# MinghanLi/MDQE_CVPR2023

Measured on AMD Instinct MI355X. Metric: frames/sec (eval-only) R50 OVIS 360p 4-frame clip, higher is better.
Workload: dtype f32; 1 GPU; R50_ovis_360 eval-only, H2D included: 120 synthetic 360x640 u8 frames/GPU/step from pinned host memory, 4-frame clips stride 1, 30-frame windows, one model(inputs) call per video; random-init weights, calibrated class logits (DESIGN.md §5); frames_per_gpu=120, instances_out=10, tracked_instances=7, gemm=exact fp32 MFMA, hw_queues=4, ranks_seen=1, parallelism=single GPU

## Files before the change

### include/mdqe_hip.h

```cpp
#ifndef MDQE_HIP_H
#define MDQE_HIP_H
#include <stdint.h>

#ifdef __cplusplus
extern "C" {
#endif

#define MDQE_OK 0
#define MDQE_EINVAL 1
#define MDQE_ELAUNCH 2
#define MDQE_ENULL 3
#define MDQE_ESTATE 4

#define MDQE_ACT_NONE 0
#define MDQE_ACT_RELU 1
#define MDQE_ACT_GELU 2
#define MDQE_ACT_SIGMOID 3
#define MDQE_ACT_TANH 4

#define MDQE_ABI_VERSION 6
int mdqe_abi_version(void);
int mdqe_version(void);
const char* mdqe_strerror(int code);

int mdqe_msda_forward_f32(const float* value, const int64_t* shapes, const int64_t* level_start,
                          const float* loc, const float* attn,
                          int B, int S, int M, int D, int L, int Q, int P,
                          float* out, void* stream);

int mdqe_msda_backward_f32(const float* value, const int64_t* shapes, const int64_t* level_start, const float* loc,
                           const float* attn, const float* grad_out, int B, int S, int M, int D, int L, int Q, int P,
                           float* grad_value, float* grad_loc, float* grad_attn, void* stream);

int mdqe_msda_forward_f64(const double* value, const int64_t* shapes, const int64_t* level_start, const double* loc,
                          const double* attn, int B, int S, int M, int D, int L, int Q, int P, double* out, void* stream);
int mdqe_msda_backward_f64(const double* value, const int64_t* shapes, const int64_t* level_start, const double* loc,
                           const double* attn, const double* grad_out, int B, int S, int M, int D, int L, int Q, int P,
                           double* grad_value, double* grad_loc, double* grad_attn, void* stream);

int mdqe_msda_forward_grouped_f32(const float* value, const int64_t* shapes, const int64_t* level_start,
                                  const float* loc, const float* attn,
                                  int B, int S, int M, int D, int G, int L, int Q, int P,
                                  float scale, float* out, void* stream);

int mdqe_msda_fused_f32(const float* value, long ldv, long v_brows, const int* vidx, const float* offs, long ldo,
                        const float* logits, long ldl, const float* ref, long ref_bstride, int ref_dim,
                        int mode, const float* grid, const int* lvH_host, const int* lvW_host,
                        const int* lvStart_host, int B, int M, int D, int G, int L, int Q, int P, float scale,
                        float* out, long ldout, long value_rows, void* stream);

int mdqe_gemm_nt_f32(const float* A, long lda, const float* W, const float* bias, float* C, long ldc,
                     int M, int N, int K, int act, int act_cols, const float* residual, long ldr, int res_mod,
                     int res_first, const unsigned char* rowmask, int mask_cols, int tile, int ksplit,
                     float* splitk_ws, const void* w_split, void* stream);

int mdqe_gemm_nt_cat2_f32(const float* A1, long lda1, int K1, const float* A2, long lda2, int K2, int NI, int OH, int OW,
                          int H2, int W2, int stride, const float* W, const float* bias, float* C, long ldc, int N, int act,
                          void* stream);

int mdqe_gemm_nt_pix_f32(const float* A, long lda, int K, int NI, int H, int W, int OH, int OW, int stride, const float* Wt,
                         const float* bias, float* C, long ldc, int N, int act, void* stream);

int mdqe_gemm_ln_f32(const float* A, long lda, const float* W, const float* bias, float* C, long ldc, int M, int N, int K,
                     const float* residual, long ldr, const float* gamma, const float* beta, float eps, void* stream);
int mdqe_gemm_ln2_f32(const float* A, long lda, const float* W, const float* bias, float* C, long ldc, int M, int N, int K,
                      const float* residual, long ldr, const float* gamma, const float* beta, const float* gamma2, const float* beta2,
                      float* C2, long ldc2, float eps, void* stream);

int mdqe_gemm_nt_side_f32(const float* A, long lda, const float* W, const float* bias, float* C, long ldc, int M, int N, int K,
                          const float* side, const float* side_w, int side_cols, const void* w_split, void* stream);

int mdqe_set_gemm_precision(int mode);
int mdqe_get_gemm_precision(void);
int mdqe_set_gemm_precision_thread(int mode);

int mdqe_f16x3_split_f32(const float* w, long n, void* planes, void* stream);

int mdqe_debug_gemm_stamps(void* buf);
int mdqe_debug_gemm_variant(int v);
int mdqe_debug_gemm_tile_rule(int v);
int mdqe_debug_gemm_rows_dot(int v);
int mdqe_debug_gemm_fast_epilogue(int v);
int mdqe_debug_gemm_stagger(int v);
int mdqe_debug_gemm_stages(int v);
int mdqe_debug_msda_dec_stage_kb(int kb);
int mdqe_debug_trk_fast(int on);
int mdqe_debug_trk_spin_us(int us);
int mdqe_debug_trk_times(double* out5, int on);
int mdqe_debug_trk_siou_blocks(int blocks);
int mdqe_debug_gemm_lds_pad(int bytes);
int mdqe_debug_window_attn_variant(int v);
int mdqe_debug_msda_xcd_order(int v);
int mdqe_debug_msda_dec_staged(int v);
int mdqe_debug_msda_dec_wpe8(int v);
int mdqe_debug_msda_patch(int v);
int mdqe_debug_msda_stage_kb(int v);
int mdqe_debug_msda_tp_staged(int v);
int mdqe_debug_msda_op_staged(int v);
int mdqe_debug_msda_variant(int v);
int mdqe_debug_mha_variant(int v);

int mdqe_conv2d_nhwc_f32(const float* X, long x_img_stride, const float* Wt, const float* bias, float* Y, long ldy,
                         int NI, int H, int W, int Cin, int Cout, int KH, int KW, int stride, int pad,
                         int act, const float* residual, long ldr, int res_first, int tile, const void* w_split,
                         int ksplit, float* splitk_ws, void* stream);

int mdqe_winograd_weight_f32(const float* Wt, int Cout, int Cin, float* U, void* stream);
long mdqe_winograd_workspace_bytes(int NI, int H, int W, int Cin, int Cout);
int mdqe_conv3x3_winograd_f32(const float* X, long x_img_stride, const float* U, const float* bias, float* Y, long ldy,
                              int NI, int H, int W, int Cin, int Cout, int act, void* workspace, long ws_bytes, void* stream);
int mdqe_debug_winograd_tile(int tile);

int mdqe_resize_pil_bilinear_u8(const unsigned char* in, long in_img_stride, int NI, int C, int H, int W, int oh, int ow,
                                const int* xmin, const int* xcnt, const int* xk, int kxs, const int* ymin, const int* ycnt,
                                const int* yk, int kys, unsigned char* out, void* stream);

#define MDQE_YUV_COEFFS { \
  {16, 128, 76309, 104597, -25675, -53279, 132201},  \
  {0, 128, 65536, 91881, -22553, -46802, 116130},    \
  {16, 128, 76309, 117489, -13975, -34925, 138438},  \
  {0, 128, 65536, 103206, -12276, -30679, 121609},   \
  {64, 512, 19077, 26149, -6419, -13320, 33050},     \
  {0, 512, 16336, 22903, -5622, -11666, 28947},      \
  {64, 512, 19077, 29372, -3494, -8731, 34610},      \
  {0, 512, 16336, 25726, -3060, -7647, 30313}        }
int mdqe_yuv420sp_to_rgb_u8(const void* y, long y_pitch, long y_stride, const void* uv, long uv_pitch, long uv_stride,
                            int NI, int H, int W, int fmt , int matrix , int full_range,
                            int bgr, unsigned char* out , void* stream);

int mdqe_layernorm_f32(const float* x, const float* res, const float* gamma, const float* beta, float* y,
                       long rows, int C, float eps, void* stream);

long mdqe_groupnorm_workspace_bytes(int NI, int G);
int mdqe_groupnorm_nhwc_f32(const float* x, long ldx, long x_img_stride, float* y, long ldy, long y_img_stride,
                            int NI, int HW, int C, int G,
                            const float* gamma, const float* beta, float eps, int act, void* workspace, void* stream);

int mdqe_stem_im2col_f32(const void* frames, int is_u8, long frame_stride, int NI, int h, int w, int Hp, int Wp,
                         const float* mean3_host, const float* std3_host, float* out, void* stream);

int mdqe_stem_conv_f32(const void* frames, int is_u8, long frame_stride, int NI, int h, int w, int Hp, int Wp,
                       const float* mean3_host, const float* std3_host, const float* wk, const float* bias, float* out,
                       void* stream);

int mdqe_maxpool3x3s2_nhwc_f32(const float* x, float* y, int NI, int H, int W, int C, void* stream);

int mdqe_upsample_nearest_add_nhwc_f32(const float* a, const float* b, float* y, int NI, int H, int W, int Hb, int Wb,
                                       int C, void* stream);

int mdqe_dwconv5x5_nhwc_f32(const float* x, const float* wt, const float* bias, float* y, int NI, int H, int W, int C,
                            int up2, const float* tw, const float* tb, void* stream);

int mdqe_dwconv5x5_c256_f32(const float* x, const float* wt, const float* bias, float* y, int NI, int H, int W, void* stream);
int mdqe_dwconv5x5_up2_c256_f32(const float* x, const float* wt, const float* bias, const float* tw, const float* tb, float* y,
                                int NI, int Hs, int Ws, void* stream);

int mdqe_dwconv5x5_up2_pw_c256_f32(const float* x, const float* wt, const float* bias, const float* tw, const float* tb,
                                   const float* pw, const float* pb, float* out, long ldo, int NI, int Hs, int Ws, void* stream);

int mdqe_trk_siou_f32(const float* saved, long saved_stride, int n_saved, const float* inp, long inp_stride,
                      int n_in, long n, float* out3, void* stream);
int mdqe_trk_accumulate_f32(float* sum, long sum_stride, float* cnt, long cnt_stride, const float* src,
                            long src_stride, long n, int nf, const int* r_host, const int* c_host, int count,
                            void* stream);
int mdqe_trk_siou_host_f32(const float* saved, long saved_stride, int n_saved, const float* inp, long inp_stride,
                           int n_in, long n, float* acc, unsigned* ticket, unsigned long long* out_host,
                           unsigned seq, void* stream);
int mdqe_trk_wait_counts(const unsigned long long* out_host, int n_out, unsigned seq, int spin_us, float* counts, void* stream);

int mdqe_trk_window_mean_f32(const float* sum, const float* cnt, long hw, int mem_len, int n, int nf, long f0,
                             float* out, void* stream);
int mdqe_trk_carry_f32(float* sum, float* cnt, long hw, int mem_len, int n, int k, long src0, float* carry, void* stream);

int mdqe_lsap_f64(const double* cost, int nr, int nc, int maximize, int* rows_out, int* cols_out, int* n_out);
int mdqe_tracker_create(int max_inst, int T, int win, int stride, int K, int E, float thr, void** handle);
int mdqe_tracker_destroy(void* handle);
int mdqe_tracker_state(void* handle, int* num_inst, int* num_clip, int* start_frame);
int mdqe_tracker_overlap(void* handle, int f0, int n_frames, int* ni, int* s0, int* a, int* nf);
int mdqe_tracker_decide(void* handle, int f0, int n_frames, int n_in, const float* scores, const float* cls_probs,
                        const float* embeds, const float* counts3, int* r_idx, int* c_idx, int* n_pairs,
                        int* s0, int* a, int* nf);
int mdqe_tracker_result(void* handle, int is_last, float* out_cls, int* n, int* ln, unsigned char* carry_valid);
int mdqe_tracker_update(void* handle, float* bank_sum, float* bank_cnt, long hw, int f0, int n_frames, int n_in,
                        const float* scores, const float* cls_probs, const float* embeds, const float* masks,
                        long inst_stride, float* counts_dev, float* counts_host, void* stream);
int mdqe_tracker_update_many(void* handle, float* bank_sum, float* bank_cnt, long hw, int n_clips, const int* f0,
                             const int* n_frames, const int* n_in, const int* row0, const float* scores,
                             const float* cls_probs, const float* embeds, const float* const* masks,
                             const long* inst_stride, float* counts_dev, float* counts_host, void* stream);
int mdqe_tracker_get_result(void* handle, int is_last, float* bank_sum, float* bank_cnt, long hw, float* out_masks,
                            float* carry, float* out_cls, int* n, int* ln, void* stream);

int mdqe_clip_assoc_f32(const float* emb, int Q, int E, const int* fidx, int Bc, int T, int ct, float wdw, int nb,
                        int* idx_out, void* stream);
int mdqe_clip_gather_init_f32(const float* content, const float* coords, const int* fidx, const int* idx, int Bc, int T,
                              int Q, int C, int ct, float* x, float* ref, float* xinst, void* stream);
int mdqe_box_refine_f32(const float* delta, const float* prev, int Bc, int T, int Q, int t0, int t1, float* boxes,
                        float* ibox, void* stream);
int mdqe_add_rows_f32(const float* a, long lda, const float* b, long ldb, float* out, long ldo, long rows, int C, void* stream);
int mdqe_time_fuse_f32(const float* w, const float* x, int Bc, int T, int Q, int C, float* out, const float* pos,
                       float* out_plus_pos, void* stream);
int mdqe_box_head_refine_f32(const float* h, long ldh, const float* W, const float* bias, const float* prev, int Bc, int T, int Q, int K,
                             int t0, int t1, float* boxes, float* ibox, void* stream);
int mdqe_time_fuse_dot_f32(const float* xw, const float* wt, const float* bt, const float* src, int Bc, int T, int Q, int C, float* out,
                           void* stream);

int mdqe_clip_select_f32(const float* cls, const float* emb, int B, int Q, int K, int C, float thr, int max_keep,
                         int* order_ws, int* n_thr_ws, float* inv_norm_ws, float* sim_ws, int* kept, int* n_keep, void* stream);
long mdqe_dyn_mask_workspace_floats(int n_rows, int T, int H, int W);
int mdqe_dyn_mask_nms_f32(const float* coef, const int* kept, const float* feats, int B, int Q, int M, int T, int H, int W,
                          const int* row0_host, const int* n_host, const int* f0_host, float* logits, float* soft_h,
                          float* hard_h, float* part, float* gram, float* stats, float* mi, void* stream);
long mdqe_nms_workspace_floats(int n_max);
int mdqe_clip_finalize_f32(const float* cls, const float* emb, const int* kept, const float* stats, const float* mi, int B,
                           int Q, int K, int C, float thr, const int* row0_host, const int* n_host, int* sel, int* n_sel,
                           float* out, void* stream);
int mdqe_rows_gather_f32(const float* src, const int* idx_dev, int n, long len, float* out, void* stream);

int mdqe_mask_row_stats_f32(const float* logits, int n, int T, int H, int W, int t_step, float* stats5,
                            float* soft_h, float* hard_h, void* stream);

int mdqe_mha_small_f32(const float* qk, long ldqk, const float* v, long ldv, float* o, long ldo, int B, int Q,
                       int C, int nh, void* stream);

int mdqe_query_select_f32(const float* conf, int NI, int H, int W, int K, int nb, float* score_ws, float* coords,
                          void* stream);

int mdqe_sample_levels_mean_f32(const float* tokens, int NI, long N, int C, const float* coords, int Qn,
                                const int* lvH_host, const int* lvW_host, const int* lvStart_host, int n_levels,
                                float* out, void* stream);

int mdqe_final_masks_u8(const float* logits, int n_sel, const int* inst_idx_dev, int Fw, int Hm, int Wm, int factor,
                        int h, int w, int Ho, int Wo, unsigned char* out, long out_inst_stride, int f_off,
                        void* stream);

int mdqe_final_masks_rle(const float* logits, int n_sel, const int* inst_idx_dev, int Fw, int Hm, int Wm, int factor,
                         int h, int w, int Ho, int Wo, int cap, int* pos, int* n_pos, void* stream);

int mdqe_final_masks_u8_geom(const float* logits, int n_sel, const int* inst_idx_dev, int Fw, int Hm, int Wm, int factor,
                             int h, int w, int Ho, int Wo, unsigned char* out, long out_inst_stride, int f_off,
                             int* geom, void* stream);
int mdqe_final_masks_rle_geom(const float* logits, int n_sel, const int* inst_idx_dev, int Fw, int Hm, int Wm, int factor,
                              int h, int w, int Ho, int Wo, int cap, int* pos, int* n_pos, int* geom, void* stream);

int mdqe_final_label_map_u8(const float* logits, int n_sel, const int* inst_idx_dev, int Fw, int Hm, int Wm, int factor,
                            int h, int w, int Ho, int Wo, unsigned char* out, int f_off, int* geom, void* stream);

int mdqe_final_matte_u8(const float* logits, int n_sel, const int* inst_idx_dev, int Fw, int Hm, int Wm, int factor,
                        int h, int w, int Ho, int Wo, const unsigned char* take, float gain, unsigned char* out, int f_off,
                        void* stream);

int mdqe_final_masks_overlap(const float* logits, int n_sel, const int* inst_idx_dev, int Fw, int Hm, int Wm, int factor,
                             int h, int w, int Ho, int Wo,
                             const uint32_t* gt_bits, int G, int f_off,
                             unsigned long long* inter, long inter_row_stride, int* area, void* stream);

int mdqe_render_overlay_u8(const void* frames, int is_u8, long frame_stride, int h0, int w0,
                           const unsigned char* labels, int F, int Ho, int Wo,
                           const unsigned char* palette, int a256, int contour,
                           unsigned char* out, int f_off, void* stream);

int mdqe_render_overlay_yuv420sp(const void* y, long y_pitch, long y_stride, const void* uv, long uv_pitch, long uv_stride,
                                 int F, int H, int W, int fmt , const unsigned char* labels,
                                 const unsigned short* palette_yuv, int a256, int contour,
                                 void* out_y, long out_y_pitch, long out_y_stride,
                                 void* out_uv, long out_uv_pitch, long out_uv_stride, int f_off, void* stream);

int mdqe_render_mosaic_u8(const void* frames, int is_u8, long frame_stride, int h0, int w0,
                          const unsigned char* labels, int F, int Ho, int Wo,
                          const unsigned char* palette, const unsigned char* action, int a256, int contour, int cell,
                          unsigned char* out, int f_off, void* stream);
int mdqe_render_mosaic_yuv420sp(const void* y, long y_pitch, long y_stride, const void* uv, long uv_pitch, long uv_stride,
                                int F, int H, int W, int fmt , const unsigned char* labels,
                                const unsigned short* palette_yuv, const unsigned char* action, int a256, int contour, int cell,
                                void* out_y, long out_y_pitch, long out_y_stride,
                                void* out_uv, long out_uv_pitch, long out_uv_stride, int f_off, void* stream);

int mdqe_render_blur_u8(const void* frames, int is_u8, long frame_stride, int h0, int w0,
                        const unsigned char* labels, int F, int Ho, int Wo,
                        const unsigned char* palette, const unsigned char* action, int a256, int contour,
                        const unsigned short* taps, int radius, unsigned char* out, int f_off, void* stream);
int mdqe_render_blur_yuv420sp(const void* y, long y_pitch, long y_stride, const void* uv, long uv_pitch, long uv_stride,
                              int F, int H, int W, int fmt , const unsigned char* labels,
                              const unsigned short* palette_yuv, const unsigned char* action, int a256, int contour,
                              const unsigned short* taps, int radius, const unsigned short* taps_c, int radius_c,
                              void* out_y, long out_y_pitch, long out_y_stride,
                              void* out_uv, long out_uv_pitch, long out_uv_stride, int f_off, void* stream);

int mdqe_render_replace_u8(const void* frames, int is_u8, long frame_stride, int h0, int w0,
                           const unsigned char* labels, int F, int Ho, int Wo,
                           const unsigned char* palette, const unsigned char* action, int a256, int contour,
                           const unsigned char* matte, const unsigned char* backdrop, int backdrop_picture, int mode,
                           unsigned char* out, int f_off, void* stream);
int mdqe_render_replace_yuv420sp(const void* y, long y_pitch, long y_stride, const void* uv, long uv_pitch, long uv_stride,
                                 int F, int H, int W, int fmt , const unsigned char* labels,
                                 const unsigned short* palette_yuv, const unsigned char* action, int a256, int contour,
                                 const unsigned char* matte, const unsigned short* backdrop_yuv,
                                 const void* by, long by_pitch, const void* buv, long buv_pitch, int mode,
                                 void* out_y, long out_y_pitch, long out_y_stride,
                                 void* out_uv, long out_uv_pitch, long out_uv_stride, int f_off, void* stream);

int mdqe_annotate_u8(unsigned char* pic , int F, int Ho, int Wo, int f_off,
                     const int* geom , int n,
                     const unsigned char* palette , const unsigned char* ink ,
                     const unsigned char* captions , int cap_len,
                     const unsigned char* font , int box, int scale, int min_area, void* stream);
int mdqe_annotate_yuv420sp(void* y, long y_pitch, long y_stride, void* uv, long uv_pitch, long uv_stride,
                           int F, int H, int W, int fmt , int f_off, const int* geom, int n,
                           const unsigned short* palette_yuv, const unsigned short* ink_yuv,
                           const unsigned char* captions, int cap_len, const unsigned char* font,
                           int box, int scale, int min_area, void* stream);

int mdqe_track_crops_u8(const void* frames, int is_u8, long frame_stride, int h0, int w0,
                        const unsigned char* labels, int F, int Ho, int Wo, const int* geom, int n,
                        int f_first, int f_step, int Sh, int Sw, int pad256, int min_area, int cutout, int fill,
                        unsigned char* out, long out_row_stride, int c_off, int* rects, long rect_row_stride, void* stream);
int mdqe_track_crops_yuv420sp(const void* y, long y_pitch, long y_stride, const void* uv, long uv_pitch, long uv_stride,
                              int H, int W, int fmt , int matrix , int full_range, int bgr,
                              const unsigned char* labels, int F, int Ho, int Wo, const int* geom, int n,
                              int f_first, int f_step, int Sh, int Sw, int pad256, int min_area, int cutout, int fill,
                              unsigned char* out, long out_row_stride, int c_off, int* rects, long rect_row_stride, void* stream);

int mdqe_label_centroids_u8(const unsigned char* labels, int F, int Ho, int Wo, int n, int min_area, long long* mom ,
                            int* pts , long pts_row_stride, int p_off, void* stream);
int mdqe_render_trails_u8(unsigned char* pic , int F, int Ho, int Wo, int f_off,
                          const int* pts, long pts_row_stride, int p_off, int n, int trail, int width,
                          const unsigned char* palette , void* stream);
int mdqe_render_trails_yuv420sp(void* y, long y_pitch, long y_stride, void* uv, long uv_pitch, long uv_stride,
                                int F, int H, int W, int fmt , int f_off,
                                const int* pts, long pts_row_stride, int p_off, int n, int trail, int width,
                                const unsigned short* palette_yuv, void* stream);

int mdqe_label_polygons_u8(const unsigned char* labels, int F, int Ho, int Wo, int n, int min_area,
                           int cap_vertices, int cap_rings,
                           int* xy,
                           int* rings,
                           int* totals,
                           void* workspace, long workspace_bytes, void* stream);
long mdqe_label_polygons_workspace(int F, int Ho, int Wo, int cap_vertices);

int mdqe_grow_labels_u8(const unsigned char* labels, int F, int Ho, int Wo,
                        const unsigned char* grow , int radius,
                        unsigned char* out , void* stream);

int mdqe_image_mask_stats_f32(const float* logits, int n, int Hm, int Wm, int factor, int h, int w, float* stats, void* stream);
int mdqe_image_final_masks_u8(const float* logits, int n_sel, const int* idx_dev, int Hm, int Wm, int factor, int h, int w,
                              int Ho, int Wo, unsigned char* out, void* stream);

int mdqe_layernorm_post_f32(const float* x, const float* gamma, const float* beta, const float* post, float* y,
                            long rows, int C, float eps, void* stream);
int mdqe_gemm_nt_swin_f32(const float* X, long lda, const float* W, const float* bias, float* C, long ldc, int B, int H, int Wd,
                          int ws, int shift, int N, int K, void* stream);
int mdqe_layernorm_swin_scatter_f32(const float* rows, const float* gamma, const float* beta, const float* shortcut, float* out,
                                    int B, int H, int W, int C, int ws, int shift, float eps, void* stream);
int mdqe_patch4_im2col_f32(const void* frames, int is_u8, long frame_stride, int NI, int h, int w, int Hp, int Wp,
                           const float* mean3_host, const float* std3_host, float* out, void* stream);
int mdqe_swin_window_f32(const float* src, const float* shortcut, float* dst, int B, int H, int W, int C, int ws,
                         int shift, int mode, void* stream);
int mdqe_window_attn_f32(const float* qkv, long ld, float* o, long ldo, int n_windows, int N, int C, int nh,
                         const float* scale, const float* bias, const float* mask, int nW, void* stream);
int mdqe_patch_merge_gather_f32(const float* x, float* out, int B, int H, int W, int C, void* stream);

#ifdef __cplusplus
}
#endif
#endif
```

### mdqe_cvpr2023_amd/_lib.py

```python
import ctypes
import os
from ctypes import c_char_p, c_float, c_int, c_void_p

_HERE = os.path.dirname(os.path.abspath(__file__))
LIB_PATH = os.environ.get("MDQE_HIP_LIB") or os.path.join(_HERE, "csrc", "libmdqe_hip.so")

from ctypes import c_long
i, f, p, l = c_int, c_float, c_void_p, c_long

SIGNATURES = {
    "mdqe_msda_forward_f32": [p, p, p, p, p, i, i, i, i, i, i, i, p, p],
    "mdqe_msda_backward_f32": [p, p, p, p, p, p, i, i, i, i, i, i, i, p, p, p, p],
    "mdqe_msda_forward_f64": [p, p, p, p, p, i, i, i, i, i, i, i, p, p],
    "mdqe_msda_backward_f64": [p, p, p, p, p, p, i, i, i, i, i, i, i, p, p, p, p],
    "mdqe_msda_forward_grouped_f32": [p, p, p, p, p, i, i, i, i, i, i, i, i, f, p, p],
    "mdqe_msda_fused_f32": [p, l, l, p, p, l, p, l, p, l, i, i, p, p, p, p, i, i, i, i, i, i, i, f, p, l, l, p],
    "mdqe_trk_siou_f32": [p, l, i, p, l, i, l, p, p],
    "mdqe_trk_accumulate_f32": [p, l, p, l, p, l, l, i, p, p, i, p],
    "mdqe_trk_window_mean_f32": [p, p, l, i, i, i, l, p, p],
    "mdqe_trk_carry_f32": [p, p, l, i, i, i, l, p, p],
    "mdqe_lsap_f64": [p, i, i, i, p, p, p],
    "mdqe_tracker_create": [i, i, i, i, i, i, f, p],
    "mdqe_tracker_destroy": [p],
    "mdqe_tracker_state": [p, p, p, p],
    "mdqe_tracker_overlap": [p, i, i, p, p, p, p],
    "mdqe_tracker_decide": [p, i, i, i, p, p, p, p, p, p, p, p, p, p],
    "mdqe_tracker_result": [p, i, p, p, p, p],
    "mdqe_tracker_update": [p, p, p, l, i, i, i, p, p, p, p, l, p, p, p],
    "mdqe_tracker_update_many": [p, p, p, l, i, p, p, p, p, p, p, p, p, p, p, p, p],
    "mdqe_tracker_get_result": [p, i, p, p, l, p, p, p, p, p, p],
    "mdqe_clip_assoc_f32": [p, i, i, p, i, i, i, f, i, p, p],
    "mdqe_clip_gather_init_f32": [p, p, p, p, i, i, i, i, i, p, p, p, p],
    "mdqe_box_refine_f32": [p, p, i, i, i, i, i, p, p, p],
    "mdqe_add_rows_f32": [p, l, p, l, p, l, l, i, p],
    "mdqe_time_fuse_f32": [p, p, i, i, i, i, p, p, p, p],
    "mdqe_box_head_refine_f32": [p, l, p, p, p, i, i, i, i, i, i, p, p, p],
    "mdqe_time_fuse_dot_f32": [p, p, p, p, i, i, i, i, p, p],
    "mdqe_clip_select_f32": [p, p, i, i, i, i, f, i, p, p, p, p, p, p, p],
    "mdqe_dyn_mask_nms_f32": [p, p, p, i, i, i, i, i, i, p, p, p, p, p, p, p, p, p, p, p],
    "mdqe_clip_finalize_f32": [p, p, p, p, p, i, i, i, i, f, p, p, p, p, p, p],
    "mdqe_rows_gather_f32": [p, p, i, l, p, p],
    "mdqe_mha_small_f32": [p, l, p, l, p, l, i, i, i, i, p],
    "mdqe_query_select_f32": [p, i, i, i, i, i, p, p, p],
    "mdqe_sample_levels_mean_f32": [p, i, l, i, p, i, p, p, p, i, p, p],
    "mdqe_image_mask_stats_f32": [p, i, i, i, i, i, i, p, p],
    "mdqe_image_final_masks_u8": [p, i, p, i, i, i, i, i, i, i, p, p],
    "mdqe_final_masks_rle": [p, i, p, i, i, i, i, i, i, i, i, i, p, p, p],
    "mdqe_final_masks_u8": [p, i, p, i, i, i, i, i, i, i, i, p, l, i, p],
    "mdqe_final_masks_rle_geom": [p, i, p, i, i, i, i, i, i, i, i, i, p, p, p, p],
    "mdqe_final_masks_u8_geom": [p, i, p, i, i, i, i, i, i, i, i, p, l, i, p, p],
    "mdqe_final_label_map_u8": [p, i, p, i, i, i, i, i, i, i, i, p, i, p, p],
    "mdqe_final_matte_u8": [p, i, p, i, i, i, i, i, i, i, i, p, f, p, i, p],
    "mdqe_render_replace_u8": [p, i, l, i, i, p, i, i, i, p, p, i, i, p, p, i, i, p, i, p],
    "mdqe_render_replace_yuv420sp": [p, l, l, p, l, l, i, i, i, i, p, p, p, i, i, p, p, p, l, p, l, i, p, l, l, p, l, l, i, p],
    "mdqe_render_overlay_u8": [p, i, l, i, i, p, i, i, i, p, i, i, p, i, p],
    "mdqe_render_overlay_yuv420sp": [p, l, l, p, l, l, i, i, i, i, p, p, i, i, p, l, l, p, l, l, i, p],
    "mdqe_render_mosaic_u8": [p, i, l, i, i, p, i, i, i, p, p, i, i, i, p, i, p],
    "mdqe_render_mosaic_yuv420sp": [p, l, l, p, l, l, i, i, i, i, p, p, p, i, i, i, p, l, l, p, l, l, i, p],
    "mdqe_render_blur_u8": [p, i, l, i, i, p, i, i, i, p, p, i, i, p, i, p, i, p],
    "mdqe_render_blur_yuv420sp": [p, l, l, p, l, l, i, i, i, i, p, p, p, i, i, p, i, p, i, p, l, l, p, l, l, i, p],
    "mdqe_annotate_u8": [p, i, i, i, i, p, i, p, p, p, i, p, i, i, i, p],
    "mdqe_annotate_yuv420sp": [p, l, l, p, l, l, i, i, i, i, i, p, i, p, p, p, i, p, i, i, i, p],
    "mdqe_track_crops_u8": [p, i, l, i, i, p, i, i, i, p, i, i, i, i, i, i, i, i, i, p, l, i, p, l, p],
    "mdqe_track_crops_yuv420sp": [p, l, l, p, l, l, i, i, i, i, i, i, p, i, i, i, p, i, i, i, i, i, i, i, i, i, p, l, i, p, l, p],
    "mdqe_label_centroids_u8": [p, i, i, i, i, i, p, p, l, i, p],
    "mdqe_label_polygons_u8": [p, i, i, i, i, i, i, i, p, p, p, p, l, p],
    "mdqe_grow_labels_u8": [p, i, i, i, p, i, p, p],
    "mdqe_render_trails_u8": [p, i, i, i, i, p, l, i, i, i, i, p, p],
    "mdqe_render_trails_yuv420sp": [p, l, l, p, l, l, i, i, i, i, i, p, l, i, i, i, i, p, p],
    "mdqe_final_masks_overlap": [p, i, p, i, i, i, i, i, i, i, i, p, i, i, p, l, p, p],
    "mdqe_set_gemm_precision": [i],
    "mdqe_set_gemm_precision_thread": [i],
    "mdqe_layernorm_post_f32": [p, p, p, p, p, l, i, f, p],
    "mdqe_gemm_nt_swin_f32": [p, l, p, p, p, l, i, i, i, i, i, i, i, p],
    "mdqe_layernorm_swin_scatter_f32": [p, p, p, p, p, i, i, i, i, i, i, f, p],
    "mdqe_patch4_im2col_f32": [p, i, l, i, i, i, i, i, p, p, p, p],
    "mdqe_swin_window_f32": [p, p, p, i, i, i, i, i, i, i, p],
    "mdqe_window_attn_f32": [p, l, p, l, i, i, i, i, p, p, p, i, p],
    "mdqe_patch_merge_gather_f32": [p, p, i, i, i, i, p],
    "mdqe_gemm_nt_f32": [p, l, p, p, p, l, i, i, i, i, i, p, l, i, i, p, i, i, i, p, p, p],
    "mdqe_f16x3_split_f32": [p, l, p, p],
    "mdqe_debug_gemm_stamps": [p],
    "mdqe_debug_gemm_variant": [i],
    "mdqe_debug_gemm_tile_rule": [i],
    "mdqe_debug_gemm_rows_dot": [i],
    "mdqe_debug_gemm_stagger": [i],
    "mdqe_debug_gemm_fast_epilogue": [i],
    "mdqe_debug_gemm_stages": [i],
    "mdqe_debug_gemm_lds_pad": [i],
    "mdqe_debug_trk_siou_blocks": [i],
    "mdqe_trk_siou_host_f32": [p, l, i, p, l, i, l, p, p, p, i, p],
    "mdqe_trk_wait_counts": [p, i, i, i, p, p],
    "mdqe_debug_trk_times": [p, i],
    "mdqe_debug_trk_fast": [i],
    "mdqe_debug_trk_spin_us": [i],
    "mdqe_debug_msda_dec_stage_kb": [i],
    "mdqe_debug_window_attn_variant": [i],
    "mdqe_debug_mha_variant": [i],
    "mdqe_debug_msda_xcd_order": [i],
    "mdqe_debug_msda_dec_staged": [i],
    "mdqe_debug_msda_patch": [i],
    "mdqe_debug_msda_dec_wpe8": [i],
    "mdqe_debug_msda_op_staged": [i],
    "mdqe_debug_msda_tp_staged": [i],
    "mdqe_debug_msda_stage_kb": [i],
    "mdqe_debug_msda_variant": [i],
    "mdqe_mask_row_stats_f32": [p, i, i, i, i, i, p, p, p, p],
    "mdqe_conv2d_nhwc_f32": [p, l, p, p, p, l, i, i, i, i, i, i, i, i, i, i, p, l, i, i, p, i, p, p],
    "mdqe_winograd_weight_f32": [p, i, i, p, p],
    "mdqe_conv3x3_winograd_f32": [p, l, p, p, p, l, i, i, i, i, i, i, p, l, p],
    "mdqe_debug_winograd_tile": [i],
    "mdqe_layernorm_f32": [p, p, p, p, p, l, i, f, p],
    "mdqe_gemm_ln_f32": [p, l, p, p, p, l, i, i, i, p, l, p, p, f, p],
    "mdqe_gemm_ln2_f32": [p, l, p, p, p, l, i, i, i, p, l, p, p, p, p, p, l, f, p],
    "mdqe_gemm_nt_side_f32": [p, l, p, p, p, l, i, i, i, p, p, i, p, p],
    "mdqe_gemm_nt_cat2_f32": [p, l, i, p, l, i, i, i, i, i, i, i, p, p, p, l, i, i, p],
    "mdqe_gemm_nt_pix_f32": [p, l, i, i, i, i, i, i, i, p, p, p, l, i, i, p],
    "mdqe_groupnorm_nhwc_f32": [p, l, l, p, l, l, i, i, i, i, p, p, f, i, p, p],
    "mdqe_resize_pil_bilinear_u8": [p, l, i, i, i, i, i, i, p, p, p, i, p, p, p, i, p, p],
    "mdqe_yuv420sp_to_rgb_u8": [p, l, l, p, l, l, i, i, i, i, i, i, i, p, p],
    "mdqe_stem_im2col_f32": [p, i, l, i, i, i, i, i, p, p, p, p],
    "mdqe_stem_conv_f32": [p, i, l, i, i, i, i, i, p, p, p, p, p, p],
    "mdqe_maxpool3x3s2_nhwc_f32": [p, p, i, i, i, i, p],
    "mdqe_upsample_nearest_add_nhwc_f32": [p, p, p, i, i, i, i, i, i, p],
    "mdqe_dwconv5x5_nhwc_f32": [p, p, p, p, i, i, i, i, i, p, p, p],
    "mdqe_dwconv5x5_c256_f32": [p, p, p, p, i, i, i, p],
    "mdqe_dwconv5x5_up2_c256_f32": [p, p, p, p, p, p, i, i, i, p],
    "mdqe_dwconv5x5_up2_pw_c256_f32": [p, p, p, p, p, p, p, p, l, i, i, i, p],
}


ABI_VERSION = 6


class LibraryMissing(RuntimeError):
    pass


class MdqeError(RuntimeError):
    pass


_lib = None


def load_library(path=None):
    global _lib
    if _lib is not None and path is None:
        return _lib
    path = path or LIB_PATH
    if not os.path.exists(path):
        raise LibraryMissing(
            f"{path} not found: build it with `make -C mdqe_cvpr2023_amd/csrc` (or "
            f"`python -c 'import __graft_entry__ as g; g.build()'`).  There is no CPU/PyTorch fallback.")
    import torch
    h = ctypes.CDLL(path)
    h.mdqe_version.restype = c_int
    h.mdqe_abi_version.restype = c_int
    h.mdqe_abi_version.argtypes = []
    if h.mdqe_abi_version() != ABI_VERSION:
        raise MdqeError(f"{path} implements ABI {h.mdqe_abi_version()}, this binding was written against ABI {ABI_VERSION} "
                        f"(include/mdqe_hip.h MDQE_ABI_VERSION): rebuild with `make -C mdqe_cvpr2023_amd/csrc`")
    h.mdqe_strerror.restype = c_char_p
    h.mdqe_strerror.argtypes = [c_int]
    h.mdqe_get_gemm_precision.restype = c_int
    h.mdqe_get_gemm_precision.argtypes = []
    h.mdqe_nms_workspace_floats.restype = c_long
    h.mdqe_nms_workspace_floats.argtypes = [c_int]
    h.mdqe_dyn_mask_workspace_floats.restype = c_long
    h.mdqe_dyn_mask_workspace_floats.argtypes = [c_int, c_int, c_int, c_int]
    h.mdqe_groupnorm_workspace_bytes.restype = c_long
    h.mdqe_groupnorm_workspace_bytes.argtypes = [c_int, c_int]
    h.mdqe_winograd_workspace_bytes.restype = c_long
    h.mdqe_winograd_workspace_bytes.argtypes = [c_int, c_int, c_int, c_int, c_int]
    h.mdqe_label_polygons_workspace.restype = c_long
    h.mdqe_label_polygons_workspace.argtypes = [c_int, c_int, c_int, c_int]
    for name, args in SIGNATURES.items():
        fn = getattr(h, name)
        fn.argtypes = args
        fn.restype = c_int
    if path == LIB_PATH:
        _lib = h
    return h


class _Lazy:
    def __getattr__(self, name):
        return getattr(load_library(), name)


lib = _Lazy()


def check(code, what=""):
    if code != 0:
        raise MdqeError(f"{what}: {load_library().mdqe_strerror(code).decode()} (code {code})")


def ptr(t):
    return None if t is None else t.data_ptr()


def raw_stream(device=None):
    import torch
    if device is None:
        idx = torch._C._cuda_getDevice()
    else:
        idx = device if isinstance(device, int) else torch.device(device).index
        if idx is None:
            idx = torch._C._cuda_getDevice()
    return torch._C._cuda_getCurrentRawStream(idx)


def cur_stream(device=None):
    return raw_stream(device)
```

### mdqe_cvpr2023_amd/csrc/common.h

```cpp
#pragma once
#include <hip/hip_runtime.h>
#include <stdint.h>
#include "../../include/mdqe_hip.h"

#define MDQE_CHECK_PTR(p) do { if ((p) == nullptr) return MDQE_ENULL; } while (0)
#define MDQE_REQUIRE(c) do { if (!(c)) return MDQE_EINVAL; } while (0)

static inline void mdqe_clear_error() { (void)hipGetLastError(); }
static inline int mdqe_launch_status() {
  return hipGetLastError() == hipSuccess ? MDQE_OK : MDQE_ELAUNCH;
}

#include <mutex>
static inline hipError_t mdqe_allow_lds(const void* kern, int bytes) {
  static std::mutex mu;
  static const void* fn[64];
  static int cap[64];
  static int n = 0;
  std::lock_guard<std::mutex> g(mu);
  int i = 0;
  for (; i < n; ++i) if (fn[i] == kern) break;
  if (i < n && cap[i] >= bytes) return hipSuccess;
  const hipError_t e = hipFuncSetAttribute(kern, hipFuncAttributeMaxDynamicSharedMemorySize, bytes);
  if (e == hipSuccess && i < 64) { fn[i] = kern; cap[i] = bytes; if (i == n) ++n; }
  return e;
}

typedef float f32x4 __attribute__((ext_vector_type(4)));
typedef float f32x2 __attribute__((ext_vector_type(2)));
typedef float f32x16 __attribute__((ext_vector_type(16)));

__device__ __forceinline__ float mdqe_gelu(float x) {
#pragma clang fp contract(off)
  const float z = __builtin_fabsf(x) * 0.70710678118654752440f;
  const float t = __builtin_amdgcn_rcpf(__builtin_fmaf(0.3275911f, z, 1.0f));
  float q = __builtin_fmaf(t, 0.5307027145f, -0.7265760135f);
  q = __builtin_fmaf(t, q, 0.7107068705f);
  q = __builtin_fmaf(t, q, -0.142248368f);
  q = __builtin_fmaf(t, q, 0.127414796f);
  const float h = q * t * __builtin_amdgcn_exp2f(z * z * -1.4426950408889634f);
  const float xh = x * h;
  return x >= 0.f ? x - xh : xh;
}

__device__ __forceinline__ float mdqe_act(float x, int act) {
  switch (act) {
    case MDQE_ACT_RELU: return x > 0.f ? x : 0.f;
    case MDQE_ACT_GELU: return mdqe_gelu(x);
    case MDQE_ACT_SIGMOID: return 1.0f / (1.0f + __expf(-x));
    case MDQE_ACT_TANH: return tanhf(x);
    default: return x;
  }
}

template <typename V4, typename ColOk>
__device__ __forceinline__ void mdqe_act4(V4& v, int act, ColOk col_ok) {
  if (act == MDQE_ACT_RELU) {
#pragma unroll
    for (int e = 0; e < 4; ++e)
      if (col_ok(e)) v[e] = v[e] > 0.f ? v[e] : 0.f;
  } else if (act == MDQE_ACT_GELU) {
#pragma unroll
    for (int e = 0; e < 4; ++e)
      if (col_ok(e)) v[e] = mdqe_gelu(v[e]);
  } else if (act != MDQE_ACT_NONE) {
#pragma unroll 1
    for (int e = 0; e < 4; ++e) {
      float x = v[0];
      if (col_ok(e)) x = mdqe_act(x, act);
      v = V4{v[1], v[2], v[3], x};
    }
  }
}
```

### mdqe_cvpr2023_amd/csrc/dwconv.hip

```cpp
#include "common.h"

namespace {
__device__ __forceinline__ f32x4 ld4(const float* p) { return *reinterpret_cast<const f32x4*>(p); }
}

__global__ void __launch_bounds__(256, 2)
dw5_c256_kernel(const float* __restrict__ x, const float* __restrict__ wt, const float* __restrict__ bias, float* __restrict__ y,
                int NI, int H, int W) {
  constexpr int C = 256;
  const int lane = threadIdx.x & 63;
  const long wid = (long)blockIdx.x * 4 + (threadIdx.x >> 6), nw = (long)gridDim.x * 4;
  f32x4 w[25];
#pragma unroll
  for (int t = 0; t < 25; ++t) w[t] = ld4(wt + t * C + lane * 4);
  const f32x4 bv = ld4(bias + lane * 4);
  const int Wp = (W + 1) / 2;
  const long total = (long)NI * H * Wp;
  for (long i = wid; i < total; i += nw) {
    const int pw_ = (int)(i % Wp); const long t = i / Wp;
    const int hh = (int)(t % H), img = (int)(t / H);
    const int w0 = pw_ * 2;
    f32x4 a0 = bv, a1 = bv;
#pragma unroll
    for (int kh = 0; kh < 5; ++kh) {
      const int ih = hh - 2 + kh;
      if (ih < 0 || ih >= H) continue;
      const float* row = x + (((long)img * H + ih) * W) * C + lane * 4;
      f32x4 X[6];
#pragma unroll
      for (int c = 0; c < 6; ++c) {
        const int iw = w0 - 2 + c;
        X[c] = (iw >= 0 && iw < W) ? ld4(row + (long)iw * C) : f32x4{0.f, 0.f, 0.f, 0.f};
      }
#pragma unroll
      for (int kw = 0; kw < 5; ++kw) { a0 += X[kw] * w[kh * 5 + kw]; a1 += X[kw + 1] * w[kh * 5 + kw]; }
    }
    float* o = y + (((long)img * H + hh) * W + w0) * C + lane * 4;
    *reinterpret_cast<f32x4*>(o) = a0;
    if (w0 + 1 < W) *reinterpret_cast<f32x4*>(o + C) = a1;
  }
}

__global__ void __launch_bounds__(256, 2)
dw5_up2_c256_kernel(const float* __restrict__ x, const float* __restrict__ wt, const float* __restrict__ bias,
                    const float* __restrict__ tw, const float* __restrict__ tb, float* __restrict__ y, int NI, int Hs, int Ws) {
  constexpr int C = 256;
  const int lane = threadIdx.x & 63;
  const long wid = (long)blockIdx.x * 4 + (threadIdx.x >> 6), nw = (long)gridDim.x * 4;
  const int H = 2 * Hs, W = 2 * Ws;
  f32x4 w[25];
#pragma unroll
  for (int t = 0; t < 25; ++t) w[t] = ld4(wt + t * C + lane * 4);
  const f32x4 bv = ld4(bias + lane * 4), twv = ld4(tw + lane * 4), tbv = ld4(tb + lane * 4);
  f32x4 wall = {0.f, 0.f, 0.f, 0.f};
#pragma unroll
  for (int t = 0; t < 25; ++t) wall += w[t];
  const f32x4 cin = bv + tbv * wall;

  const long total = (long)NI * Hs * Ws;
  for (long i = wid; i < total; i += nw) {
    const int b = (int)(i % Ws); const long t = i / Ws;
    const int a = (int)(t % Hs), img = (int)(t / Hs);
    f32x4 o00 = {0.f, 0.f, 0.f, 0.f}, o01 = o00, o10 = o00, o11 = o00;
#pragma unroll
    for (int r = 0; r < 3; ++r) {
      const int ia = a - 1 + r;
      if (ia < 0 || ia >= Hs) continue;
      const float* row = x + (((long)img * Hs + ia) * Ws) * C + lane * 4;
      f32x4 X[3];
#pragma unroll
      for (int c = 0; c < 3; ++c) {
        const int ib = b - 1 + c;
        X[c] = (ib >= 0 && ib < Ws) ? ld4(row + (long)ib * C) : f32x4{0.f, 0.f, 0.f, 0.f};
      }
#pragma unroll
      for (int c = 0; c < 3; ++c) o00 += X[c] * w[(2 * r) * 5 + 2 * c];
#pragma unroll
      for (int c = 1; c < 3; ++c) o01 += X[c] * w[(2 * r) * 5 + 2 * c - 1];
      if (r >= 1) {
#pragma unroll
        for (int c = 0; c < 3; ++c) o10 += X[c] * w[(2 * r - 1) * 5 + 2 * c];
#pragma unroll
        for (int c = 1; c < 3; ++c) o11 += X[c] * w[(2 * r - 1) * 5 + 2 * c - 1];
      }
    }
    f32x4 c00 = cin, c01 = cin, c10 = cin, c11 = cin;
    if (a == 0 || a == Hs - 1 || b == 0 || b == Ws - 1) {
      auto cst = [&](int hh, int ww) {
        f32x4 s = {0.f, 0.f, 0.f, 0.f};
#pragma unroll
        for (int kh = 0; kh < 5; ++kh) {
          const int ih = hh - 2 + kh;
          if (ih < 0 || ih >= H) continue;
#pragma unroll
          for (int kw = 0; kw < 5; ++kw) {
            const int iw = ww - 2 + kw;
            if (iw >= 0 && iw < W) s += w[kh * 5 + kw];
          }
        }
        return bv + tbv * s;
      };
      c00 = cst(2 * a, 2 * b); c01 = cst(2 * a, 2 * b + 1); c10 = cst(2 * a + 1, 2 * b); c11 = cst(2 * a + 1, 2 * b + 1);
    }
    float* o = y + (((long)img * H + 2 * a) * W + 2 * b) * C + lane * 4;
    *reinterpret_cast<f32x4*>(o) = c00 + twv * o00;
    *reinterpret_cast<f32x4*>(o + C) = c01 + twv * o01;
    *reinterpret_cast<f32x4*>(o + (long)W * C) = c10 + twv * o10;
    *reinterpret_cast<f32x4*>(o + (long)W * C + C) = c11 + twv * o11;
  }
}

__global__ void __launch_bounds__(256, 1)
dw5_up2_pw_c256_kernel(const float* __restrict__ x, const float* __restrict__ wt, const float* __restrict__ bias,
                       const float* __restrict__ tw, const float* __restrict__ tb, const float* __restrict__ pw,
                       const float* __restrict__ pb, float* __restrict__ out, long ldo, int NI, int Hs, int Ws) {
  constexpr int C = 256, QT = 8;
  extern __shared__ __attribute__((aligned(16))) float dwpw_lds[];
  const int lane = threadIdx.x & 63;
  const int wave = __builtin_amdgcn_readfirstlane(threadIdx.x >> 6);
  float* const tile = dwpw_lds + wave * (32 * C);
  const long wid = (long)blockIdx.x * 4 + wave, nw = (long)gridDim.x * 4;
  const int H = 2 * Hs, W = 2 * Ws;
  const int lr = lane & 31, lh = lane >> 5;
  f32x4 w[25];
#pragma unroll
  for (int t = 0; t < 25; ++t) w[t] = ld4(wt + t * C + lane * 4);
  const f32x4 bv = ld4(bias + lane * 4), twv = ld4(tw + lane * 4), tbv = ld4(tb + lane * 4);
  f32x4 wall = {0.f, 0.f, 0.f, 0.f};
#pragma unroll
  for (int t = 0; t < 25; ++t) wall += w[t];
  const f32x4 cin = bv + tbv * wall;
  f32x4 B0[16], B1[16];
#pragma unroll
  for (int kt = 0; kt < 16; ++kt) {
    B0[kt] = ld4(pw + lr * C + kt * 16 + lh * 4);
    B1[kt] = ld4(pw + lr * C + kt * 16 + 8 + lh * 4);
  }
  const f32x4 pbv = ld4(pb + (lane & 7) * 4);

  const int Wt = (Ws + QT - 1) / QT;
  const long total = (long)NI * Hs * Wt;
  f32x4 X[3][QT + 2];
  auto load_strip = [&](long i) __attribute__((always_inline)) {
    const int b0 = (int)(i % Wt) * QT; const long t = i / Wt;
    const int a = (int)(t % Hs), img = (int)(t / Hs);
#pragma unroll
    for (int r = 0; r < 3; ++r) {
      const int ia = a - 1 + r;
      const bool rok = ia >= 0 && ia < Hs;
      const float* row = x + (((long)img * Hs + (rok ? ia : a)) * Ws) * C + lane * 4;
#pragma unroll
      for (int c = 0; c < QT + 2; ++c) {
        const int ib = b0 - 1 + c;
        X[r][c] = (rok && ib >= 0 && ib < Ws) ? ld4(row + (long)ib * C) : f32x4{0.f, 0.f, 0.f, 0.f};
      }
    }
  };
  long i = wid;
  if (i < total) load_strip(i);
  while (i < total) {
    const int b0 = (int)(i % Wt) * QT; const long ti = i / Wt;
    const int a = (int)(ti % Hs), img = (int)(ti / Hs);
    const int nq = min(QT, Ws - b0);
#pragma unroll
    for (int q = 0; q < QT; ++q) {
      if (q >= nq) continue;
      const int b = b0 + q;
      f32x4 o00 = {0.f, 0.f, 0.f, 0.f}, o01 = o00, o10 = o00, o11 = o00;
#pragma unroll
      for (int r = 0; r < 3; ++r) {
        const int ia = a - 1 + r;
        if (ia < 0 || ia >= Hs) continue;
#pragma unroll
        for (int c = 0; c < 3; ++c) o00 += X[r][q + c] * w[(2 * r) * 5 + 2 * c];
#pragma unroll
        for (int c = 1; c < 3; ++c) o01 += X[r][q + c] * w[(2 * r) * 5 + 2 * c - 1];
        if (r >= 1) {
#pragma unroll
          for (int c = 0; c < 3; ++c) o10 += X[r][q + c] * w[(2 * r - 1) * 5 + 2 * c];
#pragma unroll
          for (int c = 1; c < 3; ++c) o11 += X[r][q + c] * w[(2 * r - 1) * 5 + 2 * c - 1];
        }
      }
      f32x4 c00 = cin, c01 = cin, c10 = cin, c11 = cin;
      if (a == 0 || a == Hs - 1 || b == 0 || b == Ws - 1) {
        auto cst = [&](int hh, int ww) {
          f32x4 s = {0.f, 0.f, 0.f, 0.f};
#pragma unroll
          for (int kh = 0; kh < 5; ++kh) {
            const int ih = hh - 2 + kh;
            if (ih < 0 || ih >= H) continue;
#pragma unroll
            for (int kw = 0; kw < 5; ++kw) {
              const int iw = ww - 2 + kw;
              if (iw >= 0 && iw < W) s += w[kh * 5 + kw];
            }
          }
          return bv + tbv * s;
        };
        c00 = cst(2 * a, 2 * b); c01 = cst(2 * a, 2 * b + 1); c10 = cst(2 * a + 1, 2 * b); c11 = cst(2 * a + 1, 2 * b + 1);
      }
      *reinterpret_cast<f32x4*>(tile + (4 * q + 0) * C + ((lane ^ ((4 * q + 0) & 15)) << 2)) = c00 + twv * o00;
      *reinterpret_cast<f32x4*>(tile + (4 * q + 1) * C + ((lane ^ ((4 * q + 1) & 15)) << 2)) = c01 + twv * o01;
      *reinterpret_cast<f32x4*>(tile + (4 * q + 2) * C + ((lane ^ ((4 * q + 2) & 15)) << 2)) = c10 + twv * o10;
      *reinterpret_cast<f32x4*>(tile + (4 * q + 3) * C + ((lane ^ ((4 * q + 3) & 15)) << 2)) = c11 + twv * o11;
    }
    asm volatile("s_waitcnt lgkmcnt(0)" ::: "memory");
    __builtin_amdgcn_wave_barrier();
    const long inext = i + nw;
    if (inext < total) load_strip(inext);

    f32x16 acc;
#pragma unroll
    for (int r = 0; r < 16; ++r) acc[r] = 0.f;
    const float* const arow = tile + lr * C;
#pragma unroll
    for (int kt = 0; kt < 16; ++kt) {
      const f32x4 a0 = *reinterpret_cast<const f32x4*>(arow + (((4 * kt + lh) ^ (lr & 15)) << 2));
      const f32x4 a1 = *reinterpret_cast<const f32x4*>(arow + (((4 * kt + 2 + lh) ^ (lr & 15)) << 2));
#pragma unroll
      for (int s = 0; s < 4; ++s) acc = __builtin_amdgcn_mfma_f32_32x32x2f32(a0[s], B0[kt][s], acc, 0, 0, 0);
#pragma unroll
      for (int s = 0; s < 4; ++s) acc = __builtin_amdgcn_mfma_f32_32x32x2f32(a1[s], B1[kt][s], acc, 0, 0, 0);
    }
    asm volatile("s_waitcnt lgkmcnt(0)" ::: "memory");
    __builtin_amdgcn_wave_barrier();
#pragma unroll
    for (int r = 0; r < 16; ++r) tile[((r & 3) + 8 * (r >> 2) + 4 * lh) * 32 + lr] = acc[r];
    asm volatile("s_waitcnt lgkmcnt(0)" ::: "memory");
    __builtin_amdgcn_wave_barrier();
#pragma unroll
    for (int it = 0; it < 4; ++it) {
      const int row = it * 8 + (lane >> 3), c4 = lane & 7;
      const int q = row >> 2, dy = (row >> 1) & 1, dx = row & 1;
      const f32x4 v = *reinterpret_cast<const f32x4*>(tile + row * 32 + c4 * 4) + pbv;
      if (q < nq) {
        const long pix = ((long)img * H + 2 * a + dy) * W + 2 * (b0 + q) + dx;
        *reinterpret_cast<f32x4*>(out + pix * ldo + c4 * 4) = v;
      }
    }
    asm volatile("s_waitcnt lgkmcnt(0)" ::: "memory");
    __builtin_amdgcn_wave_barrier();
    i = inext;
  }
}

extern "C" int mdqe_dwconv5x5_c256_f32(const float* x, const float* wt, const float* bias, float* y, int NI, int H, int W,
                                       void* stream) {
  MDQE_REQUIRE(NI >= 0 && H > 0 && W > 0);
  if (NI == 0) return MDQE_OK;
  MDQE_CHECK_PTR(x); MDQE_CHECK_PTR(wt); MDQE_CHECK_PTR(bias); MDQE_CHECK_PTR(y);
  mdqe_clear_error();
  const long total = (long)NI * H * ((W + 1) / 2);
  long nb = (total + 3) / 4; if (nb > 256 * 8) nb = 256 * 8;
  hipLaunchKernelGGL(dw5_c256_kernel, dim3((unsigned)nb), dim3(256), 0, (hipStream_t)stream, x, wt, bias, y, NI, H, W);
  return mdqe_launch_status();
}

extern "C" int mdqe_dwconv5x5_up2_c256_f32(const float* x, const float* wt, const float* bias, const float* tw, const float* tb,
                                           float* y, int NI, int Hs, int Ws, void* stream) {
  MDQE_REQUIRE(NI >= 0 && Hs > 0 && Ws > 0);
  if (NI == 0) return MDQE_OK;
  MDQE_CHECK_PTR(x); MDQE_CHECK_PTR(wt); MDQE_CHECK_PTR(bias); MDQE_CHECK_PTR(tw); MDQE_CHECK_PTR(tb); MDQE_CHECK_PTR(y);
  mdqe_clear_error();
  const long total = (long)NI * Hs * Ws;
  long nb = (total + 3) / 4; if (nb > 256 * 8) nb = 256 * 8;
  hipLaunchKernelGGL(dw5_up2_c256_kernel, dim3((unsigned)nb), dim3(256), 0, (hipStream_t)stream, x, wt, bias, tw, tb, y, NI, Hs, Ws);
  return mdqe_launch_status();
}

extern "C" int mdqe_dwconv5x5_up2_pw_c256_f32(const float* x, const float* wt, const float* bias, const float* tw, const float* tb,
                                              const float* pw, const float* pb, float* out, long ldo, int NI, int Hs, int Ws,
                                              void* stream) {
  MDQE_REQUIRE(NI >= 0 && Hs > 0 && Ws > 0 && ldo >= 32 && ldo % 4 == 0);
  if (NI == 0) return MDQE_OK;
  MDQE_CHECK_PTR(x); MDQE_CHECK_PTR(wt); MDQE_CHECK_PTR(bias); MDQE_CHECK_PTR(tw); MDQE_CHECK_PTR(tb);
  MDQE_CHECK_PTR(pw); MDQE_CHECK_PTR(pb); MDQE_CHECK_PTR(out);
  MDQE_REQUIRE((((uintptr_t)x | (uintptr_t)wt | (uintptr_t)bias | (uintptr_t)tw | (uintptr_t)tb | (uintptr_t)pw | (uintptr_t)pb |
                 (uintptr_t)out) & 15) == 0);
  mdqe_clear_error();
  static int num_cus = 0;
  if (num_cus == 0) {
    int dev = 0, n = 0;
    (void)hipGetDevice(&dev);
    if (hipDeviceGetAttribute(&n, hipDeviceAttributeMultiprocessorCount, dev) != hipSuccess || n <= 0) n = 256;
    num_cus = n;
  }
  const int smem = 4 * 32 * 256 * (int)sizeof(float);
  if (mdqe_allow_lds(reinterpret_cast<const void*>(dw5_up2_pw_c256_kernel), smem) != hipSuccess) return MDQE_ELAUNCH;
  const long total = (long)NI * Hs * ((Ws + 7) / 8);
  long nb = (total + 3) / 4; if (nb > num_cus) nb = num_cus;
  hipLaunchKernelGGL(dw5_up2_pw_c256_kernel, dim3((unsigned)nb), dim3(256), (size_t)smem, (hipStream_t)stream, x, wt, bias, tw, tb, pw,
                     pb, out, ldo, NI, Hs, Ws);
  return mdqe_launch_status();
}
```

### mdqe_cvpr2023_amd/csrc/norm.hip

```cpp
#include "common.h"

__device__ __forceinline__ float wave_sum(float v) {
#pragma unroll
  for (int o = 32; o > 0; o >>= 1) v += __shfl_xor(v, o, 64);
  return v;
}

__device__ __forceinline__ float wave_sum_c256(float v) {
  v += __shfl_xor(v, 8, 64);
  v += __shfl_xor(v, 1, 64); v += __shfl_xor(v, 2, 64); v += __shfl_xor(v, 4, 64);
  v += __shfl_xor(v, 16, 64); v += __shfl_xor(v, 32, 64);
  return v;
}

struct SwinMap { int ws, shift, H, W; };

template <int NCH>
__global__ void __launch_bounds__(256)
layernorm_kernel(const float* __restrict__ x, const float* __restrict__ res, const float* __restrict__ gamma,
                 const float* __restrict__ beta, const float* __restrict__ post, float* __restrict__ y, long rows, int C, float eps,
                 SwinMap sm) {
  const int lane = threadIdx.x & 63;
  const long wid = (long)blockIdx.x * (blockDim.x >> 6) + (threadIdx.x >> 6);
  const long nw = (long)gridDim.x * (blockDim.x >> 6);
  for (long r = wid; r < rows; r += nw) {
    long ro = r;
    if (sm.ws > 0) {
      const int ws = sm.ws, nWx = (sm.W + ws - 1) / ws, nWy = (sm.H + ws - 1) / ws;
      const int ix = (int)(r % ws); long t = r / ws;
      const int iy = (int)(t % ws); t /= ws;
      const int wx = (int)(t % nWx); t /= nWx;
      const int wy = (int)(t % nWy); const long b = t / nWy;
      const int yy = (wy * ws + iy + sm.shift) % (nWy * ws), xx = (wx * ws + ix + sm.shift) % (nWx * ws);
      if (yy >= sm.H || xx >= sm.W) continue;
      ro = (b * sm.H + yy) * sm.W + xx;
    }
    f32x4 v[NCH];
    float s = 0.f;
#pragma unroll
    for (int i = 0; i < NCH; ++i) {
      const int c = lane * 4 + i * 256;
      if (c < C) {
        v[i] = *reinterpret_cast<const f32x4*>(x + r * C + c);
        if (res != nullptr) v[i] += *reinterpret_cast<const f32x4*>(res + r * C + c);
        s += (v[i][0] + v[i][1]) + (v[i][2] + v[i][3]);
      } else {
        v[i] = f32x4{0.f, 0.f, 0.f, 0.f};
      }
    }
    const bool tree256 = NCH == 1 && C == 256;
    const float mean = (tree256 ? wave_sum_c256(s) : wave_sum(s)) / C;
    float q = 0.f;
#pragma unroll
    for (int i = 0; i < NCH; ++i) {
      const int c = lane * 4 + i * 256;
      if (c < C) {
        const f32x4 d = v[i] - mean;
        q += (d[0] * d[0] + d[1] * d[1]) + (d[2] * d[2] + d[3] * d[3]);
      }
    }
    const float rstd = rsqrtf((tree256 ? wave_sum_c256(q) : wave_sum(q)) / C + eps);
#pragma unroll
    for (int i = 0; i < NCH; ++i) {
      const int c = lane * 4 + i * 256;
      if (c < C) {
        const f32x4 g = *reinterpret_cast<const f32x4*>(gamma + c);
        const f32x4 b = *reinterpret_cast<const f32x4*>(beta + c);
        f32x4 o = (v[i] - mean) * rstd * g + b;
        if (post != nullptr) o += *reinterpret_cast<const f32x4*>(post + ro * C + c);
        *reinterpret_cast<f32x4*>(y + ro * C + c) = o;
      }
    }
  }
}

static int layernorm_impl(const float* x, const float* res, const float* gamma, const float* beta, const float* post, float* y,
                          long rows, int C, float eps, void* stream, SwinMap sm = SwinMap{0, 0, 0, 0}) {
  MDQE_REQUIRE(rows >= 0 && C > 0 && C % 4 == 0 && C <= 2048);
  if (rows == 0) return MDQE_OK;
  MDQE_CHECK_PTR(x); MDQE_CHECK_PTR(gamma); MDQE_CHECK_PTR(beta); MDQE_CHECK_PTR(y);
  mdqe_clear_error();
  long nb = (rows + 3) / 4;
  if (nb > 256 * 32) nb = 256 * 32;
  hipStream_t st = (hipStream_t)stream;
  if (C <= 256) hipLaunchKernelGGL((layernorm_kernel<1>), dim3((unsigned)nb), dim3(256), 0, st, x, res, gamma, beta, post, y, rows, C, eps, sm);
  else if (C <= 512) hipLaunchKernelGGL((layernorm_kernel<2>), dim3((unsigned)nb), dim3(256), 0, st, x, res, gamma, beta, post, y, rows, C, eps, sm);
  else if (C <= 1024) hipLaunchKernelGGL((layernorm_kernel<4>), dim3((unsigned)nb), dim3(256), 0, st, x, res, gamma, beta, post, y, rows, C, eps, sm);
  else hipLaunchKernelGGL((layernorm_kernel<8>), dim3((unsigned)nb), dim3(256), 0, st, x, res, gamma, beta, post, y, rows, C, eps, sm);
  return mdqe_launch_status();
}

extern "C" int mdqe_layernorm_f32(const float* x, const float* res, const float* gamma, const float* beta, float* y,
                                  long rows, int C, float eps, void* stream) {
  return layernorm_impl(x, res, gamma, beta, nullptr, y, rows, C, eps, stream);
}

extern "C" int mdqe_layernorm_post_f32(const float* x, const float* gamma, const float* beta, const float* post, float* y,
                                       long rows, int C, float eps, void* stream) {
  MDQE_CHECK_PTR(post);
  return layernorm_impl(x, nullptr, gamma, beta, post, y, rows, C, eps, stream);
}

extern "C" int mdqe_layernorm_swin_scatter_f32(const float* rows_, const float* gamma, const float* beta, const float* shortcut, float* out,
                                               int B, int H, int W, int C, int ws, int shift, float eps, void* stream) {
  MDQE_REQUIRE(B >= 0 && H > 0 && W > 0 && ws > 0 && shift >= 0 && shift < ws);
  MDQE_CHECK_PTR(shortcut);
  const long Hp = (H + ws - 1) / ws * ws, Wp = (W + ws - 1) / ws * ws;
  return layernorm_impl(rows_, nullptr, gamma, beta, shortcut, out, (long)B * Hp * Wp, C, eps, stream, SwinMap{ws, shift, H, W});
}

#define GN_MAX_CHUNKS 64

__global__ void __launch_bounds__(256)
gn_partial_kernel(const float* __restrict__ x, long ldx, long xis, int HW, int C, int G, int nchunks, double* __restrict__ part) {
  __shared__ float sh_s[1024], sh_q[1024];
  __shared__ double ch_s[1024], ch_q[1024];
  const int img = blockIdx.y, chunk = blockIdx.x;
  const int c4n = C / 4;
  const int tpr = 256 / c4n;
  const int col = threadIdx.x % c4n, rsub = threadIdx.x / c4n;
  const int per = (HW + nchunks - 1) / nchunks;
  const int p0 = chunk * per, p1 = min(HW, p0 + per);
  float s[4] = {0, 0, 0, 0}, q[4] = {0, 0, 0, 0};
  if (rsub < tpr) {
    const float* base = x + (long)img * xis + col * 4;
    for (int p = p0 + rsub; p < p1; p += tpr) {
      const f32x4 v = *reinterpret_cast<const f32x4*>(base + (long)p * ldx);
#pragma unroll
      for (int k = 0; k < 4; ++k) { s[k] += v[k]; q[k] += v[k] * v[k]; }
    }
#pragma unroll
    for (int k = 0; k < 4; ++k) { sh_s[rsub * C + col * 4 + k] = s[k]; sh_q[rsub * C + col * 4 + k] = q[k]; }
  }
  __syncthreads();
  for (int c = threadIdx.x; c < C; c += 256) {
    double a = 0.0, b = 0.0;
    for (int r = 0; r < tpr; ++r) { a += (double)sh_s[r * C + c]; b += (double)sh_q[r * C + c]; }
    ch_s[c] = a; ch_q[c] = b;
  }
  __syncthreads();
  const int cpg = C / G;
  if (threadIdx.x < G) {
    double a = 0.0, b = 0.0;
    for (int c = threadIdx.x * cpg; c < (threadIdx.x + 1) * cpg; ++c) { a += ch_s[c]; b += ch_q[c]; }
    double* o = part + (((long)img * nchunks + chunk) * G + threadIdx.x) * 2;
    o[0] = a; o[1] = b;
  }
}

__global__ void __launch_bounds__(256)
gn_apply_kernel(const float* __restrict__ x, long ldx, long xis, float* __restrict__ y, long ldy, long yis, int HW, int C, int G, int nchunks,
                const double* __restrict__ part, const float* __restrict__ gamma, const float* __restrict__ beta,
                float eps, int act) {
  __shared__ float s_mean[64], s_rstd[64];
  const int img = blockIdx.y;
  if (threadIdx.x < G) {
    double s = 0.0, q = 0.0;
    for (int c = 0; c < nchunks; ++c) {
      const double* o = part + (((long)img * nchunks + c) * G + threadIdx.x) * 2;
      s += o[0]; q += o[1];
    }
    const double n = (double)HW * (C / G);
    const double mean = s / n;
    double var = q / n - mean * mean;
    if (var < 0) var = 0;
    s_mean[threadIdx.x] = (float)mean;
    s_rstd[threadIdx.x] = (float)(1.0 / sqrt(var + (double)eps));
  }
  __syncthreads();
  const int c4n = C / 4, cpg = C / G;
  const long total = (long)HW * c4n;
  for (long i = (long)blockIdx.x * blockDim.x + threadIdx.x; i < total; i += (long)gridDim.x * blockDim.x) {
    const int col = (int)(i % c4n);
    const long p = i / c4n;
    const f32x4 v = *reinterpret_cast<const f32x4*>(x + (long)img * xis + p * ldx + col * 4);
    const f32x4 g = *reinterpret_cast<const f32x4*>(gamma + col * 4);
    const f32x4 b = *reinterpret_cast<const f32x4*>(beta + col * 4);
    f32x4 o;
#pragma unroll
    for (int k = 0; k < 4; ++k) {
      const int gi = (col * 4 + k) / cpg;
      o[k] = mdqe_act((v[k] - s_mean[gi]) * s_rstd[gi] * g[k] + b[k], act);
    }
    *reinterpret_cast<f32x4*>(y + (long)img * yis + p * ldy + col * 4) = o;
  }
}

extern "C" long mdqe_groupnorm_workspace_bytes(int NI, int G) { return (long)NI * GN_MAX_CHUNKS * G * 2 * sizeof(double); }

extern "C" int mdqe_groupnorm_nhwc_f32(const float* x, long ldx, long x_img_stride, float* y, long ldy, long y_img_stride,
                                       int NI, int HW, int C, int G,
                                       const float* gamma, const float* beta, float eps, int act, void* workspace,
                                       void* stream) {
  MDQE_REQUIRE(NI >= 0 && HW > 0 && C > 0 && G > 0 && G <= 64 && C % G == 0 && C % 4 == 0 && C <= 1024);
  MDQE_REQUIRE(ldx >= C && ldy >= C && ldx % 4 == 0 && ldy % 4 == 0);
  if (x_img_stride <= 0) x_img_stride = (long)HW * ldx;
  if (y_img_stride <= 0) y_img_stride = (long)HW * ldy;
  MDQE_REQUIRE(x_img_stride % 4 == 0 && y_img_stride % 4 == 0);
  if (NI == 0) return MDQE_OK;
  MDQE_CHECK_PTR(x); MDQE_CHECK_PTR(y); MDQE_CHECK_PTR(gamma); MDQE_CHECK_PTR(beta); MDQE_CHECK_PTR(workspace);
  mdqe_clear_error();
  hipStream_t st = (hipStream_t)stream;
  int nchunks = (HW + 255) / 256;
  if (nchunks > GN_MAX_CHUNKS) nchunks = GN_MAX_CHUNKS;
  if (nchunks < 1) nchunks = 1;
  hipLaunchKernelGGL(gn_partial_kernel, dim3(nchunks, NI), dim3(256), 0, st, x, ldx, x_img_stride, HW, C, G, nchunks, (double*)workspace);
  int rc = mdqe_launch_status();
  if (rc) return rc;
  long blocks = ((long)HW * (C / 4) + 255) / 256;
  if (blocks > 512) blocks = 512;
  hipLaunchKernelGGL(gn_apply_kernel, dim3((unsigned)blocks, NI), dim3(256), 0, st, x, ldx, x_img_stride, y, ldy, y_img_stride, HW, C, G, nchunks,
                     (const double*)workspace, gamma, beta, eps, act);
  return mdqe_launch_status();
}
```

### mdqe_cvpr2023_amd/csrc/spatial.hip

```cpp
#include "common.h"

template <typename T>
__global__ void __launch_bounds__(256)
stem_im2col_kernel(const T* __restrict__ frames, long frame_stride, int NI, int h, int w, int Hp, int Wp,
                   float m0, float m1, float m2, float s0, float s1, float s2, float* __restrict__ out, int OH, int OW) {
  const long total = (long)NI * OH * OW * 40;
  for (long i = (long)blockIdx.x * blockDim.x + threadIdx.x; i < total; i += (long)gridDim.x * blockDim.x) {
    const int q4 = (int)(i % 40);
    const long m = i / 40;
    const int ow = (int)(m % OW); const long t = m / OW; const int oh = (int)(t % OH); const int img = (int)(t / OH);
    f32x4 v;
#pragma unroll
    for (int e = 0; e < 4; ++e) {
      const int k = q4 * 4 + e;
      float val = 0.f;
      if (k < 147) {
        const int c = k % 3, tap = k / 3, kw = tap % 7, kh = tap / 7;
        const int ih = oh * 2 - 3 + kh, iw = ow * 2 - 3 + kw;
        if (ih >= 0 && ih < h && iw >= 0 && iw < w) {
          const float raw = (float)frames[(long)img * frame_stride + ((long)c * h + ih) * w + iw];
          const float mean = c == 0 ? m0 : (c == 1 ? m1 : m2);
          const float sd = c == 0 ? s0 : (c == 1 ? s1 : s2);
          val = (raw - mean) / sd;
        }
      }
      v[e] = val;
    }
    *reinterpret_cast<f32x4*>(out + m * 160 + q4 * 4) = v;
  }
}

extern "C" int mdqe_stem_im2col_f32(const void* frames, int is_u8, long frame_stride, int NI, int h, int w, int Hp, int Wp,
                                    const float* mean3_host, const float* std3_host, float* out, void* stream) {
  MDQE_REQUIRE(NI >= 0 && h > 0 && w > 0 && Hp >= h && Wp >= w && Hp % 2 == 0 && Wp % 2 == 0);
  if (NI == 0) return MDQE_OK;
  MDQE_CHECK_PTR(frames); MDQE_CHECK_PTR(out); MDQE_CHECK_PTR(mean3_host); MDQE_CHECK_PTR(std3_host);
  mdqe_clear_error();
  const int OH = Hp / 2, OW = Wp / 2;
  const long total = (long)NI * OH * OW * 40;
  long nb = (total + 255) / 256; if (nb > 256 * 16) nb = 256 * 16;
  hipStream_t st = (hipStream_t)stream;
  if (is_u8)
    hipLaunchKernelGGL((stem_im2col_kernel<unsigned char>), dim3((unsigned)nb), dim3(256), 0, st, (const unsigned char*)frames,
                       frame_stride, NI, h, w, Hp, Wp, mean3_host[0], mean3_host[1], mean3_host[2], std3_host[0], std3_host[1],
                       std3_host[2], out, OH, OW);
  else
    hipLaunchKernelGGL((stem_im2col_kernel<float>), dim3((unsigned)nb), dim3(256), 0, st, (const float*)frames, frame_stride, NI,
                       h, w, Hp, Wp, mean3_host[0], mean3_host[1], mean3_host[2], std3_host[0], std3_host[1], std3_host[2], out,
                       OH, OW);
  return mdqe_launch_status();
}

__global__ void __launch_bounds__(256)
maxpool3x3s2_kernel(const float* __restrict__ x, float* __restrict__ y, int NI, int H, int W, int C, int OH, int OW) {
  const int c4n = C / 4;
  const long total = (long)NI * OH * OW * c4n;
  for (long i = (long)blockIdx.x * blockDim.x + threadIdx.x; i < total; i += (long)gridDim.x * blockDim.x) {
    const int c4 = (int)(i % c4n); long t = i / c4n;
    const int ow = (int)(t % OW); t /= OW; const int oh = (int)(t % OH); const int img = (int)(t / OH);
    f32x4 m = {-INFINITY, -INFINITY, -INFINITY, -INFINITY};
#pragma unroll
    for (int kh = 0; kh < 3; ++kh) {
      const int ih = oh * 2 - 1 + kh;
      if (ih < 0 || ih >= H) continue;
#pragma unroll
      for (int kw = 0; kw < 3; ++kw) {
        const int iw = ow * 2 - 1 + kw;
        if (iw < 0 || iw >= W) continue;
        const f32x4 v = *reinterpret_cast<const f32x4*>(x + (((long)img * H + ih) * W + iw) * C + c4 * 4);
#pragma unroll
        for (int e = 0; e < 4; ++e) m[e] = fmaxf(m[e], v[e]);
      }
    }
    *reinterpret_cast<f32x4*>(y + (((long)img * OH + oh) * OW + ow) * C + c4 * 4) = m;
  }
}

extern "C" int mdqe_maxpool3x3s2_nhwc_f32(const float* x, float* y, int NI, int H, int W, int C, void* stream) {
  MDQE_REQUIRE(NI >= 0 && H > 0 && W > 0 && C > 0 && C % 4 == 0);
  if (NI == 0) return MDQE_OK;
  MDQE_CHECK_PTR(x); MDQE_CHECK_PTR(y);
  mdqe_clear_error();
  const int OH = (H + 2 - 3) / 2 + 1, OW = (W + 2 - 3) / 2 + 1;
  const long total = (long)NI * OH * OW * (C / 4);
  long nb = (total + 255) / 256; if (nb > 256 * 16) nb = 256 * 16;
  hipLaunchKernelGGL(maxpool3x3s2_kernel, dim3((unsigned)nb), dim3(256), 0, (hipStream_t)stream, x, y, NI, H, W, C, OH, OW);
  return mdqe_launch_status();
}

__global__ void __launch_bounds__(256)
upsample_add_kernel(const float* __restrict__ a, const float* __restrict__ b, float* __restrict__ y, int NI, int H, int W,
                    int Hb, int Wb, int C) {
  const int c4n = C / 4;
  const float sh = (float)Hb / (float)H, sw = (float)Wb / (float)W;
  const long total = (long)NI * H * W * c4n;
  for (long i = (long)blockIdx.x * blockDim.x + threadIdx.x; i < total; i += (long)gridDim.x * blockDim.x) {
    const int c4 = (int)(i % c4n); long t = i / c4n;
    const int ww = (int)(t % W); t /= W; const int hh = (int)(t % H); const int img = (int)(t / H);
    const int hb = min((int)floorf(hh * sh), Hb - 1), wb = min((int)floorf(ww * sw), Wb - 1);
    const f32x4 va = *reinterpret_cast<const f32x4*>(a + (((long)img * H + hh) * W + ww) * C + c4 * 4);
    const f32x4 vb = *reinterpret_cast<const f32x4*>(b + (((long)img * Hb + hb) * Wb + wb) * C + c4 * 4);
    *reinterpret_cast<f32x4*>(y + (((long)img * H + hh) * W + ww) * C + c4 * 4) = va + vb;
  }
}

extern "C" int mdqe_upsample_nearest_add_nhwc_f32(const float* a, const float* b, float* y, int NI, int H, int W, int Hb,
                                                  int Wb, int C, void* stream) {
  MDQE_REQUIRE(NI >= 0 && H > 0 && W > 0 && Hb > 0 && Wb > 0 && C > 0 && C % 4 == 0);
  if (NI == 0) return MDQE_OK;
  MDQE_CHECK_PTR(a); MDQE_CHECK_PTR(b); MDQE_CHECK_PTR(y);
  mdqe_clear_error();
  const long total = (long)NI * H * W * (C / 4);
  long nb = (total + 255) / 256; if (nb > 256 * 16) nb = 256 * 16;
  hipLaunchKernelGGL(upsample_add_kernel, dim3((unsigned)nb), dim3(256), 0, (hipStream_t)stream, a, b, y, NI, H, W, Hb, Wb, C);
  return mdqe_launch_status();
}

template <int K>
__global__ void __launch_bounds__(256)
dwconv_kernel(const float* __restrict__ x, const float* __restrict__ wt, const float* __restrict__ bias, float* __restrict__ y,
              int NI, int H, int W, int C, int up2, const float* __restrict__ tw, const float* __restrict__ tb) {
  const int c4n = C / 4;
  const long total = (long)NI * H * W * c4n;
  const int Hs = up2 ? H / 2 : H, Ws = up2 ? W / 2 : W;
  for (long i = (long)blockIdx.x * blockDim.x + threadIdx.x; i < total; i += (long)gridDim.x * blockDim.x) {
    const int c4 = (int)(i % c4n); long t = i / c4n;
    const int ww = (int)(t % W); t /= W; const int hh = (int)(t % H); const int img = (int)(t / H);
    f32x4 acc = *reinterpret_cast<const f32x4*>(bias + c4 * 4);
    f32x4 twv = {0, 0, 0, 0}, tbv = {0, 0, 0, 0};
    if (up2) { twv = *reinterpret_cast<const f32x4*>(tw + c4 * 4); tbv = *reinterpret_cast<const f32x4*>(tb + c4 * 4); }
#pragma unroll
    for (int kh = 0; kh < K; ++kh) {
      const int ih = hh - K / 2 + kh;
      if (ih < 0 || ih >= H) continue;
#pragma unroll
      for (int kw = 0; kw < K; ++kw) {
        const int iw = ww - K / 2 + kw;
        if (iw < 0 || iw >= W) continue;
        const f32x4 wv = *reinterpret_cast<const f32x4*>(wt + (long)(kh * K + kw) * C + c4 * 4);
        f32x4 v;
        if (up2) {
          if (((ih | iw) & 1) == 0)
            v = *reinterpret_cast<const f32x4*>(x + (((long)img * Hs + (ih >> 1)) * Ws + (iw >> 1)) * C + c4 * 4) * twv + tbv;
          else
            v = tbv;
        } else {
          v = *reinterpret_cast<const f32x4*>(x + (((long)img * Hs + ih) * Ws + iw) * C + c4 * 4);
        }
        acc += v * wv;
      }
    }
    *reinterpret_cast<f32x4*>(y + (((long)img * H + hh) * W + ww) * C + c4 * 4) = acc;
  }
}

extern "C" int mdqe_dwconv5x5_nhwc_f32(const float* x, const float* wt, const float* bias, float* y, int NI, int H, int W,
                                       int C, int up2, const float* tw, const float* tb, void* stream) {
  MDQE_REQUIRE(NI >= 0 && H > 0 && W > 0 && C > 0 && C % 4 == 0);
  MDQE_REQUIRE(!up2 || (H % 2 == 0 && W % 2 == 0));
  if (NI == 0) return MDQE_OK;
  MDQE_CHECK_PTR(x); MDQE_CHECK_PTR(wt); MDQE_CHECK_PTR(bias); MDQE_CHECK_PTR(y);
  if (up2) { MDQE_CHECK_PTR(tw); MDQE_CHECK_PTR(tb); }
  mdqe_clear_error();
  const long total = (long)NI * H * W * (C / 4);
  long nb = (total + 255) / 256; if (nb > 256 * 32) nb = 256 * 32;
  hipLaunchKernelGGL((dwconv_kernel<5>), dim3((unsigned)nb), dim3(256), 0, (hipStream_t)stream, x, wt, bias, y, NI, H, W, C, up2,
                     tw, tb);
  return mdqe_launch_status();
}

__global__ void __launch_bounds__(256)
resize_pil_bilinear_kernel(const unsigned char* __restrict__ in, long in_img_stride, int C, int H, int W, int oh, int ow,
                           const int* __restrict__ xmin, const int* __restrict__ xcnt, const int* __restrict__ xk, int kxs,
                           const int* __restrict__ ymin, const int* __restrict__ ycnt, const int* __restrict__ yk, int kys,
                           unsigned char* __restrict__ out, long total) {
  for (long i = (long)blockIdx.x * blockDim.x + threadIdx.x; i < total; i += (long)gridDim.x * blockDim.x) {
    const int X = (int)(i % ow); long t = i / ow;
    const int Y = (int)(t % oh); t /= oh;
    const int c = (int)(t % C); const long img = t / C;
    const unsigned char* src = in + img * in_img_stride + (long)c * H * W;
    const int x0 = xmin[X], nx = xcnt[X], y0 = ymin[Y], ny = ycnt[Y];
    const int* kx = xk + (long)X * kxs;
    const int* ky = yk + (long)Y * kys;
    int acc = 1 << 21;
    for (int ty = 0; ty < ny; ++ty) {
      const unsigned char* row = src + (long)(y0 + ty) * W + x0;
      int hv;
      if (ow == W) {
        hv = row[X - x0];
      } else {
        int hs = 1 << 21;
        for (int tx = 0; tx < nx; ++tx) hs += (int)row[tx] * kx[tx];
        hv = min(max(hs >> 22, 0), 255);
      }
      if (oh == H) { acc = hv; break; }
      acc += hv * ky[ty];
    }
    out[i] = (unsigned char)(oh == H ? acc : min(max(acc >> 22, 0), 255));
  }
}

extern "C" int mdqe_resize_pil_bilinear_u8(const unsigned char* in, long in_img_stride, int NI, int C, int H, int W, int oh, int ow,
                                           const int* xmin, const int* xcnt, const int* xk, int kxs, const int* ymin,
                                           const int* ycnt, const int* yk, int kys, unsigned char* out, void* stream) {
  MDQE_REQUIRE(NI >= 0 && C > 0 && H > 0 && W > 0 && oh > 0 && ow > 0 && kxs > 0 && kys > 0);
  if (NI == 0) return MDQE_OK;
  MDQE_CHECK_PTR(in); MDQE_CHECK_PTR(out); MDQE_CHECK_PTR(xmin); MDQE_CHECK_PTR(xcnt); MDQE_CHECK_PTR(xk);
  MDQE_CHECK_PTR(ymin); MDQE_CHECK_PTR(ycnt); MDQE_CHECK_PTR(yk);
  mdqe_clear_error();
  const long total = (long)NI * C * oh * ow;
  long nb = (total + 255) / 256; if (nb > 256 * 64) nb = 256 * 64;
  hipLaunchKernelGGL(resize_pil_bilinear_kernel, dim3((unsigned)nb), dim3(256), 0, (hipStream_t)stream, in, in_img_stride, C, H, W, oh,
                     ow, xmin, xcnt, xk, kxs, ymin, ycnt, yk, kys, out, total);
  return mdqe_launch_status();
}
```

### mdqe_cvpr2023_amd/engine.py

```python
import contextlib
import math
import os
from types import SimpleNamespace as NS

import numpy as np
import torch
import torch.nn.functional as F

from . import ops
from .config import MDQEConfig
from .params import ALIASES, RESNET_BLOCKS, msda_dir_grid


def _fold_bn(sd, p, eps=1e-5):
    scale = sd[p + ".norm.weight"] * (sd[p + ".norm.running_var"] + eps).rsqrt()
    shift = sd[p + ".norm.bias"] - sd[p + ".norm.running_mean"] * scale
    return sd[p + ".weight"] * scale.view(-1, 1, 1, 1), shift


GEO_CACHE = max(1, int(os.environ.get("MDQE_GEO_CACHE", "16")))
STEM_FUSED = os.environ.get("MDQE_STEM_FUSED", "1") != "0"
SWIN_FUSED = os.environ.get("MDQE_SWIN_FUSED", "1") != "0"
RESNET_CAT = os.environ.get("MDQE_RESNET_CAT", "1") != "0"

# ... 173 lines not shown
                Wi, bi = sd[f"{q}.{mod}.in_proj_weight"], sd[f"{q}.{mod}.in_proj_bias"]
                setattr(L, tag, NS(wqk=up(Wi[:2 * C]), bqk=up(bi[:2 * C]), wv=up(Wi[2 * C:]), bv=up(bi[2 * C:]),
                                   wo=up(sd[f"{q}.{mod}.out_proj.weight"]), bo=up(sd[f"{q}.{mod}.out_proj.bias"])))
            for tag, mod in (("ca", "cross_attn"), ("ta", "temp_attn_inst")):
                if not (q + f".{mod}.value_proj.weight") in sd:
                    setattr(L, tag, None)
                    continue
                wq = torch.cat([sd[f"{q}.{mod}.sampling_grid_offsets.weight"], sd[f"{q}.{mod}.attention_weights.weight"]], 0)
                bq = torch.cat([sd[f"{q}.{mod}.sampling_grid_offsets.bias"], sd[f"{q}.{mod}.attention_weights.bias"]])
                setattr(L, tag, NS(wq=up(wq), bq=up(bq), n_off=sd[f"{q}.{mod}.sampling_grid_offsets.weight"].shape[0],
                                   wo=up(sd[f"{q}.{mod}.output_proj.weight"]), bo=up(sd[f"{q}.{mod}.output_proj.bias"])))
                vw.append(sd[f"{q}.{mod}.value_proj.weight"])
                vb.append(sd[f"{q}.{mod}.value_proj.bias"])
            P64, bp64 = w.double().cpu(), sd[d + ".point2pos_proj.bias"].double().cpu()
            for tag, mod in (("sa", "self_attn"), ("sai", "self_attn_inst")):
                m = getattr(L, tag)
                Wi, bi = sd[f"{q}.{mod}.in_proj_weight"].double().cpu(), sd[f"{q}.{mod}.in_proj_bias"].double().cpu()
                sw = torch.zeros(3 * C, 4, dtype=torch.float64)
                sw[:2 * C] = Wi[:2 * C] @ P64
                bb = bi.clone()
                bb[:2 * C] += Wi[:2 * C] @ bp64
                m.wqkv, m.bqkv_pos, m.side_w = up(Wi.float()), up(bb.float()), up(sw.float())
            for tag in ("ca", "ta"):
                m = getattr(L, tag)
                if m is None:
                    continue
                m.side_w = up((m.wq.double().cpu() @ P64).float())
                m.bq_pos = up((m.bq.double().cpu() + m.wq.double().cpu() @ bp64).float())
            for nm in ("norm1", "norm2", "norm3", "norm1_inst", "norm2_inst", "norm3_inst"):
                setattr(L, nm, (up(sd[f"{q}.{nm}.weight"]), up(sd[f"{q}.{nm}.bias"])))
            for nm in ("linear1", "linear2", "linear1_inst", "linear2_inst", "time_weights"):
                setattr(L, nm, (up(sd[f"{q}.{nm}.weight"]), up(sd[f"{q}.{nm}.bias"])))
            self.dec.append(L)
        self.dec_vw, self.dec_vb = up(torch.cat(vw, 0)), up(torch.cat(vb))
        self.n_val = len(vw)
        self.grid_sp = up(msda_dir_grid(nh, cfg.n_levels, cfg.dec_points))
        self.grid_tp = up(msda_dir_grid(nh, cfg.n_frames, cfg.dec_points))
        nb = cfg.n_bins
        ii, jj = torch.meshgrid(torch.arange(nb), torch.arange(nb), indexing="ij")
        ind = torch.stack([jj, ii], -1).view(-1, 2)
        self.relpos = (ind[:, None] - ind[None]).abs().to(dev)


def _pos_sine(mask, npf, temperature=10000.0):
    nm = ~mask[None]
    y = nm.cumsum(1, dtype=torch.float32)
    x = nm.cumsum(2, dtype=torch.float32)
    y = y / (y[:, -1:, :] + 1e-6) * (2 * math.pi)
    x = x / (x[:, :, -1:] + 1e-6) * (2 * math.pi)
    d = torch.arange(npf, dtype=torch.float32)
    d = temperature ** (2 * torch.div(d, 2, rounding_mode="trunc") / npf)
    px, py = x[..., None] / d, y[..., None] / d
    px = torch.stack((px[..., 0::2].sin(), px[..., 1::2].cos()), 4).flatten(3)
    py = torch.stack((py[..., 0::2].sin(), py[..., 1::2].cos()), 4).flatten(3)
    return torch.cat((py, px), 3)[0].reshape(-1, 2 * npf)


class Geometry:

    def __init__(self, P: Packed, h, w):
        cfg, dev = P.cfg, P.dev
        d = cfg.size_divisibility
        self.h, self.w = h, w
        self.Hp, self.Wp = (h + d - 1) // d * d, (w + d - 1) // d * d
        shapes, masks = [], []
        for s in cfg.backbone_strides:
            H, W = self.Hp // s, self.Wp // s
            m = torch.ones(H, W, dtype=torch.bool)
            m[: int(np.ceil(float(h) / s)), : int(np.ceil(float(w) / s))] = False
            shapes.append((H, W))
            masks.append(m)
        for l in range(len(shapes), cfg.n_levels):
            H, W = (shapes[-1][0] + 2 - 3) // 2 + 1, (shapes[-1][1] + 2 - 3) // 2 + 1
            m = F.interpolate(masks[len(cfg.backbone_strides) - 1][None, None].float(), size=(H, W)).to(torch.bool)[0, 0]
            shapes.append((H, W))
            masks.append(m)
        self.shapes = shapes
        self.hw = [a * b for a, b in shapes]
        self.starts = [0] + list(np.cumsum(self.hw)[:-1])
        self.N = int(sum(self.hw))
        self.mask_flat = torch.cat([m.flatten() for m in masks]).to(dev)
        self.any_pad = bool(self.mask_flat.any())
        npf = cfg.hidden_dim // 2
        self.pos_tables = []
        if P.level_embed is not None:
            pos = torch.cat([_pos_sine(m, npf) + P.level_embed[l].view(1, -1) for l, m in enumerate(masks)], 0)
            ref = torch.cat([self._ref_points(H, W) for H, W in shapes], 0)
            self.ref = ref.contiguous().to(dev)
            pos_d = pos.contiguous().to(dev)
            nq = P.enc[0].wq.shape[0] if P.enc else 0
            C = cfg.hidden_dim
            for lyr in P.enc:
                t = torch.zeros(self.N, C + nq, device=dev)
                ops.linear(pos_d, lyr.wq, None, out=t[:, C:], ldc=C + nq)
                self.pos_tables.append(t)
        self._masks_rep = {}
        self.swin_masks = None
        if P.swin is not None:
            H, W = self.Hp // 4, self.Wp // 4
            self.swin_masks = []
            for stg in P.swin.stages:
                self.swin_masks.append((H, W, _swin_shift_mask(H, W, stg.ws).to(dev)))
                H, W = (H + 1) // 2, (W + 1) // 2

    @staticmethod
    def _ref_points(H, W):
        ry, rx = torch.meshgrid(torch.linspace(0.5, H - 0.5, H), torch.linspace(0.5, W - 0.5, W), indexing="ij")
        return torch.stack((rx.reshape(-1) / max(W, 1), ry.reshape(-1) / max(H, 1)), -1)

    def rowmask(self, n):
        if not self.any_pad:
            return None
        if n not in self._masks_rep:
            m = self.mask_flat.view(torch.uint8).repeat(n).contiguous()
            if m.is_cuda:
                torch.cuda.current_stream(m.device).synchronize()
            self._masks_rep[n] = m
        return self._masks_rep[n]


def inverse_sigmoid(x, eps=1e-5):
    x = x.clamp(0, 1)
    return torch.log(x.clamp(min=eps) / (1 - x).clamp(min=eps))


def box_cxcywh_to_xyxy(b):
    cx, cy, w, h = b.unbind(-1)
    return torch.stack([cx - 0.5 * w, cy - 0.5 * h, cx + 0.5 * w, cy + 0.5 * h], -1)


def box_xyxy_to_cxcywh(b):
    x0, y0, x1, y1 = b.unbind(-1)
    return torch.stack([(x0 + x1) / 2, (y0 + y1) / 2, x1 - x0, y1 - y0], -1)


INST_STREAMS = {}
DEC_TWO_STREAMS = os.environ.get("MDQE_DEC_TWO_STREAMS", "1") != "0"
DEC_FUSED = os.environ.get("MDQE_DEC_FUSED", "1") != "0"


class Engine:
    def __init__(self, cfg: MDQEConfig, state_dict, device="cuda", backbone_fn=None, only_backbone=False):
        self.cfg = cfg
        self.P = Packed(state_dict, cfg, device, only_backbone=only_backbone)
        self.dev = self.P.dev
        self.backbone_fn = backbone_fn
        self._geo = {}
        self.precision_map = os.environ.get("MDQE_PRECISION_MAP", "")
        if self.precision_map not in ("", "reference", "autocast_f16"):
            raise ValueError("MDQE_PRECISION_MAP: '' (exact fp32 everywhere), 'reference' or 'autocast_f16', not %r" % self.precision_map)

    def amp(self):
        if self.precision_map == "reference" and self.dev.type == "cuda":
            return ops.gemm_precision("f16x3")
        if self.precision_map == "autocast_f16" and self.dev.type == "cuda":
            return ops.gemm_precision("f16")
        return contextlib.nullcontext()

    def geometry(self, h, w) -> Geometry:
        k = (h, w)
        g = self._geo.pop(k, None)
        if g is None:
            g = Geometry(self.P, h, w)
            while len(self._geo) >= GEO_CACHE:
                self._geo.pop(next(iter(self._geo)))
        self._geo[k] = g
        return g

    def backbone(self, frames, geo):
        if self.backbone_fn is not None:
            return self.backbone_fn(frames, geo)
        with self.amp():
            return self.backbone_swin(frames, geo) if self.P.swin is not None else self._backbone_r50(frames, geo)

    def _backbone_r50(self, frames, geo):
        bb, cfg = self.P.bb, self.cfg
        NI = frames.shape[0]
        if STEM_FUSED:
            x = ops.stem_conv(frames, geo.Hp, geo.Wp, cfg.pixel_mean, cfg.pixel_std, bb.stem_wk, bb.stem_b)
        else:
            col = ops.stem_im2col(frames, geo.Hp, geo.Wp, cfg.pixel_mean, cfg.pixel_std)
            x = ops.linear(col, bb.stem_w, bb.stem_b, act="relu").view(NI, geo.Hp // 2, geo.Wp // 2, 64)
            del col
        x = ops.maxpool3x3s2(x)
        outs = []
        for si, blocks in enumerate(bb.stages):
            for blk in blocks:
                s, s1, s3 = blk.stride, blk.s1, blk.s3
                if blk.cat is not None and RESNET_CAT and ops.get_gemm_precision() == "f32" and x.is_contiguous():
                    if s1 == 1:
                        y = self._conv(x, blk.conv1, 1, 1, 0, "relu")
                    else:
                        y = ops.linear_pix(x, s1, blk.conv1[0].view(blk.conv1[0].shape[0], -1), blk.conv1[1], act="relu")
                    y = self._conv(y, blk.conv2, 3, s3, 1, "relu")
                    x = ops.linear_cat2(y, x, s, *blk.cat, act="relu")
                    continue
                sc = x if blk.shortcut is None else self._conv(x, blk.shortcut, 1, s, 0, None)
                y = self._conv(x, blk.conv1, 1, s1, 0, "relu")
                y = self._conv(y, blk.conv2, 3, s3, 1, "relu")
                x = self._conv(y, blk.conv3, 1, 1, 0, "relu", residual=sc)
            if si >= 1:
                outs.append(x)
        return outs

    def backbone_swin(self, frames, geo):
        sw, cfg = self.P.swin, self.cfg
        NI = frames.shape[0]
        col = ops.patch4_im2col(frames, geo.Hp, geo.Wp, cfg.pixel_mean, cfg.pixel_std)
        x = ops.layernorm(ops.linear(col, sw.pe_w, sw.pe_b), *sw.pe_n)
        del col
        outs = []
        for si, stg in enumerate(sw.stages):
            H, W, mask = geo.swin_masks[si]
            C, ws, nh = stg.dim, stg.ws, stg.nh
            N = ws * ws
            nWy, nWx = (H + ws - 1) // ws, (W + ws - 1) // ws
            x4 = x.view(NI, H, W, C)
            fuse = SWIN_FUSED and ops.get_gemm_precision() == "f32" and x4.is_contiguous()
            own = False
            for blk in stg.blocks:
                if fuse:
                    qkv = ops.linear_swin(x4, blk.wqkv, blk.bqkv, ws, blk.shift)
                else:
                    qkv = ops.linear(ops.swin_window_gather(x4, ws, blk.shift), blk.wqkv, blk.bqkv)
                a = ops.window_attn(qkv, NI * nWy * nWx, N, C, nh, blk.scale, blk.bias, mask if blk.shift > 0 else None, nWy * nWx)
                if fuse:
                    x4 = ops.layernorm_swin_scatter(ops.linear(a, blk.wproj, blk.bproj), *blk.n1, x4, ws, blk.shift,
                                                    out=x4 if own else torch.empty_like(x4))
                else:
                    pr = ops.layernorm(ops.linear(a, blk.wproj, blk.bproj), *blk.n1)
                    x4 = ops.swin_window_scatter_add(pr, x4, ws, blk.shift)
                own = True
                x2 = x4.view(-1, C)
                h = ops.linear(x2, *blk.fc1, act="gelu")
                x4 = ops.layernorm_post(ops.linear(h, *blk.fc2), *blk.n2, post=x2).view(NI, H, W, C)
            if stg.out_norm is not None:
                outs.append(ops.layernorm(x4, *stg.out_norm).view(NI, H, W, C))
            if stg.down is not None:
                g = ops.patch_merge_gather(x4)
                x = ops.layernorm(ops.linear(g, stg.down.w, None), *stg.down.n)
        return outs

    @staticmethod
    def _conv(x, wb, k, stride, pad, act, residual=None):
        w, b = wb
        if k == 1 and stride == 1 and x.is_contiguous():
            NI, H, W, Cin = x.shape
            r = residual.view(-1, residual.shape[-1]) if residual is not None else None
            return ops.linear(x.view(-1, Cin), w.view(w.shape[0], Cin), b, act=act, residual=r, res_first=True).view(NI, H, W, -1)
        return ops.conv2d_nhwc(x, w, b, stride, pad, act=act, residual=residual, res_first=True)

    def encode(self, feats, geo):
        P, cfg = self.P, self.cfg
        NI, C, N = feats[0].shape[0], cfg.hidden_dim, geo.N
        x = torch.empty(NI, N, C, device=self.dev)
        src = None
        for l in range(cfg.n_levels):
            ip = P.inproj[l]
            with self.amp():
                if l < len(feats):
                    f = feats[l]
                    y = ops.linear(f.reshape(-1, f.shape[-1]), ip.w.view(C, -1), ip.b)
                else:
                    src = feats[-1] if l == len(feats) else src
                    y = ops.conv2d_nhwc(src, ip.w, ip.b, 2, 1)
                    src = None
            s0, hw = geo.starts[l], geo.hw[l]
            ops.groupnorm_nhwc(y.view(NI, hw, C), 32, ip.g, ip.beta, out=x[:, s0:s0 + hw])
        M, nh = NI * N, cfg.nheads
        D = C // nh
        LP = cfg.n_levels * cfg.enc_points
        levels = ([s[0] for s in geo.shapes], [s[1] for s in geo.shapes], geo.starts)
        rowmask = geo.rowmask(NI)
        x2 = x.view(M, C)
        nq = 3 * nh * LP
        proj = torch.empty(M, C + nq, device=self.dev)
        attn = torch.empty(M, C, device=self.dev)
        hid = torch.empty(M, cfg.d_ffn, device=self.dev)
        y = torch.empty(M, C, device=self.dev)
        for li, lyr in enumerate(P.enc):
            ops.linear(x2, lyr.wcat, lyr.bcat, residual=geo.pos_tables[li], res_mod=N, rowmask=rowmask, mask_cols=C, out=proj)
            ops.msda_fused(proj[:, :C], proj[:, C:C + 2 * nh * LP], proj[:, C + 2 * nh * LP:], geo.ref, levels, NI, N, nh, D,
                           cfg.n_levels, cfg.enc_points, mode=0, v_brows=N, out=attn)
            ops.linear_ln(attn, lyr.wo, lyr.bo, x2, *lyr.n1, out=x2, scratch=y)
            ops.linear(x2, lyr.w1, lyr.b1, act="gelu", out=hid)
            if li == len(P.enc) - 1:
                _, out = ops.linear_ln(hid, lyr.w2, lyr.b2, x2, *lyr.n2, out=x2, scratch=y, second=P.enc_norm)
                return out.view(NI, N, C)
            ops.linear_ln(hid, lyr.w2, lyr.b2, x2, *lyr.n2, out=x2, scratch=y)
        return ops.layernorm(x2, *P.enc_norm).view(NI, N, C)

    def mask_features(self, enc, geo, out=None):
        with self.amp():
            return self._mask_features(enc, geo, out)

    def mask_feature_shape(self, geo):
        H, W = geo.shapes[0]
        return 2 * H, 2 * W, int(self.P.mh.out_lay2.pw.shape[0])

    def _mask_features(self, enc, geo, out=None):
        mh, cfg = self.P.mh, self.cfg
        NI, N, C = enc.shape
        lv = [enc[:, geo.starts[l]:geo.starts[l] + geo.hw[l]].view(NI, geo.shapes[l][0], geo.shapes[l][1], C) for l in range(3)]
        x = ops.conv2d_nhwc(lv[2], *mh.lay1, 1, 1)
        x = ops.groupnorm_nhwc(x, 8, *mh.gn1, act="gelu", out=x).view(x.shape)
        for i, f in ((2, lv[1]), (3, lv[0])):
            cur = ops.conv2d_nhwc(f, *getattr(mh, f"ad{i - 1}"), 1, 0)
            x = ops.upsample_nearest_add(cur, x, out=cur)
            x = ops.conv2d_nhwc(x, *getattr(mh, f"lay{i}"), 1, 1)
            x = ops.groupnorm_nhwc(x, 8, *getattr(mh, f"gn{i}"), act="gelu", out=x).view(x.shape)
        o1, o2 = mh.out_lay1, mh.out_lay2
        y = ops.dwconv5x5(x, o1.dw, o1.db)
        y = ops.linear(y.view(-1, C), o1.pw, o1.pb).view(x.shape)
        y = ops.groupnorm_nhwc(y, 32, o1.g, o1.beta, act="relu", out=y).view(x.shape)
        Md = o2.pw.shape[0]
        Hm, Wm = 2 * y.shape[1], 2 * y.shape[2]
        if out is not None and (tuple(out.shape) != (NI, Hm, Wm, Md) or not out.is_contiguous()):
            raise RuntimeError("mask_features: out must be a contiguous [NI, Hm, Wm, M] tensor")
        z2 = ops.dwconv5x5_up2_pw(y, o2.dw, o2.db, mh.tw, mh.tb, o2.pw, o2.pb, out=None if out is None else out.view(-1, Md)).view(NI, Hm, Wm, Md)
        return ops.groupnorm_nhwc(z2, 32 if Md % 32 == 0 else 24, o2.g, o2.beta, act="relu", out=z2).view(z2.shape)

    def _mlp(self, x, layers, last_act=None, out=None):
        n = len(layers)
        for i, (w, b) in enumerate(layers):
            x = ops.linear(x, w, b, act="gelu" if i < n - 1 else last_act, out=out if i == n - 1 else None)
        return x

    def frame_queries(self, enc, geo, out=None):
        cfg = self.cfg
        NI, N, C = enc.shape
        H, W = geo.shapes[0]
        nb = cfg.n_bins
        o_coords, o_content, o_emb = out if out is not None else (None, None, None)
        with self.amp():
            conf = self._mlp(enc[:, :H * W].reshape(-1, C), self.P.rpn_cls).view(NI, H, W, -1)
        coords = ops.query_select(conf, nb, out=o_coords)
        content = ops.sample_levels_mean(enc, coords, geo.shapes, geo.starts, out=o_content)
        with self.amp():
            emb = self._mlp(content.view(-1, C), self.P.track_embed, out=None if o_emb is None else o_emb.view(NI * nb * nb, -1)).view(NI, nb * nb, -1)
        return coords, content, emb

    def cache_shapes(self, geo, keep_enc=False):
        cfg, P = self.cfg, self.P
        C, Q = cfg.hidden_dim, cfg.n_bins * cfg.n_bins
        sh = {"vals": (geo.N, int(P.dec_vw.shape[0])), "coords": (Q, 2), "content": (Q, C), "emb": (Q, int(P.track_embed[-1][0].shape[0])),
              "mf": self.mask_feature_shape(geo)}
        if keep_enc:
            sh["enc"] = (geo.N, C)
        return sh

    def dec_values(self, enc, geo, out=None):
        NI, N, C = enc.shape
        if out is not None:
            out = out.view(NI * N, -1)
        return ops.linear(enc.view(-1, C), self.P.dec_vw, self.P.dec_vb, rowmask=geo.rowmask(NI),
                          mask_cols=self.P.dec_vw.shape[0], out=out).view(NI, N, -1)

    def _to_dev_i32(self, arr):
        h = torch.from_numpy(np.ascontiguousarray(arr, dtype=np.int32))
        if self.dev.type != "cuda":
            return h.to(self.dev)
        return h.pin_memory().to(self.dev, non_blocking=True)

    def decode_clip(self, coords, content, emb, values, geo):
        T = content.shape[0]
        out = self.decode_clips({"coords": coords, "content": content, "emb": emb, "vals": values}, [0], T, geo)
        return {k: v[0] for k, v in out.items()}

    def decode_clips(self, cache, starts, T, geo, two_streams=True):
        P, cfg = self.P, self.cfg
        Bc = len(starts)
        fidx_h = np.asarray([[a + t for t in range(T)] for a in starts], dtype=np.int32).reshape(Bc, T)
        lo, hi = int(fidx_h.min()), int(fidx_h.max()) + 1
        if lo > 0 or hi < cache["content"].shape[0]:
            cache = {k: v[lo:hi] for k, v in cache.items() if k in ("coords", "content", "emb", "vals")}
            fidx_h = fidx_h - lo
        fidx = self._to_dev_i32(fidx_h)
        content, vals = cache["content"], cache["vals"]
        Q, C = content.shape[1], content.shape[2]
        nh, N = cfg.nheads, geo.N
        D, Tc = C // nh, cfg.n_frames
        ct = int((T - 1) / 2)
        idx = ops.clip_assoc(cache["emb"], fidx, ct, cfg.window_inter_frame_asso / 2, cfg.n_bins) if T > 1 else None
        x, ref, x_inst = ops.clip_gather_init(content, cache["coords"], fidx, idx, ct)
        BT = Bc * T
        fused = DEC_FUSED
        small = fused and C == 256

        def refine(z, prev, zn=None):
            z = ops.layernorm(z, *P.dec_norm) if zn is None else zn
            if small:
                h = ops.linear(ops.linear(z, *P.bbox_embed[0], act="gelu"), *P.bbox_embed[1], act="gelu")
                return ops.box_head_refine(h, *P.bbox_embed[2], prev, Bc, T, Q, t0, t1)
            return ops.box_refine(self._mlp(z, P.bbox_embed), prev, Bc, T, Q, t0, t1)

        def qkv(sa, z, box, B_):
            if fused:
                o = ops.linear_side(z, sa.wqkv, sa.bqkv_pos, box, sa.side_w, 2 * C)
                return ops.mha_small(o[:, :2 * C], o[:, 2 * C:], B_, Q, C, nh)
            zp = ops.add_rows(z, ops.linear(box, *P.p2p))
            return ops.mha_small(ops.linear(zp, sa.wqk, sa.bqk), ops.linear(z, sa.wv, sa.bv), B_, Q, C, nh)

        def qproj(m, z, box):
            if fused:
                return ops.linear_side(z, m.wq, m.bq_pos, box, m.side_w, m.wq.shape[0])
            return ops.linear(ops.add_rows(z, ops.linear(box, *P.p2p)), m.wq, m.bq)

        t0, t1 = max(ct - int((Tc - 1) / 2), 0), ct + Tc
        boxes, ibox = refine(x, ref)
        itv = max(int(T / Tc), 1)
        ts = max(ct - int((Tc - 1) / 2) * itv, 0)
        tca = list(range(ts, T, itv))[:Tc]
        tca = tca + [tca[-1]] * (Tc - len(tca))
        lv_sp = ([s[0] for s in geo.shapes], [s[1] for s in geo.shapes], geo.starts)
        lv_tp = ([s[0] for s in geo.shapes for _ in range(Tc)], [s[1] for s in geo.shapes for _ in range(Tc)],
                 [f * N + geo.starts[g] for g in range(len(geo.shapes)) for f in tca])
        LP = cfg.n_levels * cfg.dec_points
        TP = Tc * cfg.dec_points
        vals2 = vals.view(-1, vals.shape[-1])
        vidx_sp = fidx.view(-1)
        vidx_tp = self._to_dev_i32(fidx_h[:, 0])
        vi = 0
        main = torch.cuda.current_stream(self.dev) if self.dev.type == "cuda" else None
        two = DEC_TWO_STREAMS and two_streams and main is not None and len(P.dec) > 1
        if two:
            pool = INST_STREAMS
            side = pool.get(main.cuda_stream)
            if side is None:
                side = pool[main.cuda_stream] = torch.cuda.Stream(self.dev, priority=-1)
            side.wait_stream(main)
            hold = [x_inst]

        def inst_level(L, x, sx, x_inst, ibox, vi):
            if small:
                fq = ops.time_fuse_dot(x, *L.time_weights, sx, Bc, T, Q)
            else:
                fq = ops.time_fuse(ops.linear(x, *L.time_weights), sx, Bc, T, Q)
            if L.ta is not None:
                pr = qproj(L.ta, fq, ibox)
                a = ops.msda_fused(vals2[:, vi * C:(vi + 1) * C], pr[:, :2 * nh * TP], pr[:, 2 * nh * TP:], ibox.view(Bc, Q, 4), lv_tp,
                                   Bc, Q, nh, D, Tc, cfg.dec_points, mode=1, grid=P.grid_tp, groups=len(geo.shapes),
                                   scale=1.0 / len(geo.shapes), v_brows=N, vidx=vidx_tp)
                x_inst = ops.linear_ln(a, L.ta.wo, L.ta.bo, x_inst, *L.norm2_inst)
            else:
                x_inst = ops.layernorm(x_inst, *L.norm2_inst, res=fq)
            x_inst = ops.linear_ln(qkv(L.sai, x_inst, ibox, Bc), L.sai.wo, L.sai.bo, x_inst, *L.norm1_inst)
            hdn = ops.linear(x_inst, *L.linear1_inst, act="gelu")
            return ops.linear_ln(hdn, *L.linear2_inst, x_inst, *L.norm3_inst)

        for L in P.dec:
            pr = qproj(L.ca, x, boxes)
            a = ops.msda_fused(vals2[:, vi * C:(vi + 1) * C], pr[:, :2 * nh * LP], pr[:, 2 * nh * LP:], boxes.view(BT, Q, 4), lv_sp,
                               BT, Q, nh, D, cfg.n_levels, cfg.dec_points, mode=1, grid=P.grid_sp, v_brows=N, vidx=vidx_sp)
            vi += 1
            x = ops.linear_ln(a, L.ca.wo, L.ca.bo, x, *L.norm2)
            sx = x
            x = ops.linear_ln(qkv(L.sa, x, boxes, BT), L.sa.wo, L.sa.bo, x, *L.norm1)
            hdn = ops.linear(x, *L.linear1, act="gelu")
            xn = None
            if L is not P.dec[-1]:
                x, xn = ops.linear_ln(hdn, *L.linear2, x, *L.norm3, second=P.dec_norm)
            else:
                x = ops.linear_ln(hdn, *L.linear2, x, *L.norm3)
            vi_inst = vi
            if L.ta is not None:
                vi += 1
            if two:
                ev = torch.cuda.Event()
                ev.record(main)
                with torch.cuda.stream(side):
                    side.wait_event(ev)
                    x_inst = inst_level(L, x, sx, x_inst, ibox, vi_inst)
                hold += [x, sx, ibox]
            else:
                x_inst = inst_level(L, x, sx, x_inst, ibox, vi_inst)
            if L is not P.dec[-1]:
                boxes, ibox = refine(x, boxes, xn)
        if two:
            main.wait_stream(side)
            del hold
        n = ops.layernorm(x_inst, *P.dec_norm)
        with self.amp():
            return {"cls": self._mlp(n, P.cls_embed, "sigmoid").view(Bc, Q, -1),
                    "mask_coeff": self._mlp(n, P.mask_embed, "tanh").view(Bc, Q, -1),
                    "query_embed": x_inst.view(Bc, Q, C)}

    def inference_clip(self, out, mask_feats):
        return self.inference_clips({k: v[None] for k, v in out.items()}, [mask_feats])[0]

    def inference_clips(self, outs, mask_feats, f0=None, T=None):
        cfg = self.cfg
        cls, coef, emb = outs["cls"].contiguous(), outs["mask_coeff"].contiguous(), outs["query_embed"].contiguous()
        B, Q, K = cls.shape
        C = emb.shape[-1]
        thr = cfg.apply_cls_thres
        if isinstance(mask_feats, (list, tuple)):
            T = int(mask_feats[0].shape[0])
            Hm, Wm, Md = (int(v) for v in mask_feats[0].shape[1:])
            fbytes = Hm * Wm * Md * 4
            p0 = min(m.data_ptr() for m in mask_feats)
            st0 = mask_feats[0].untyped_storage().data_ptr()
            if any((not m.is_contiguous()) or tuple(m.shape) != (T, Hm, Wm, Md) or (m.data_ptr() - p0) % fbytes
                   or m.untyped_storage().data_ptr() != st0 for m in mask_feats):
                raise RuntimeError("inference_clips: mask_feats must be contiguous [T,Hm,Wm,M] views of one channels-last buffer")
            f0 = np.asarray([(m.data_ptr() - p0) // fbytes for m in mask_feats], dtype=np.int32)
            nfr = int(f0.max()) + T
            lo = min(mask_feats, key=lambda m: m.data_ptr())
            feats = torch.as_strided(lo, (nfr, Hm, Wm, Md), (Hm * Wm * Md, Wm * Md, Md, 1))
        else:
            feats = mask_feats
            f0 = np.asarray(f0, dtype=np.int32)
            Hm, Wm, Md = (int(v) for v in feats.shape[1:])
        kept, n_keep = ops.clip_select(cls, emb, thr, 10 * cfg.detections_per_image)
        n = n_keep.cpu().numpy().astype(np.int32)
        row0 = np.zeros(B, dtype=np.int32)
        row0[1:] = np.cumsum(n)[:-1]
        n_tot = int(n.sum())
        mp, stats, mi = ops.dyn_mask_nms(coef, kept, feats, row0, n, f0, T)
        sel, n_sel, small = ops.clip_finalize(cls, emb, kept, stats, mi, thr, row0, n)
        if self.dev.type == "cuda":
            hs = torch.empty(small.shape, pin_memory=True)
            hk = torch.empty(B, dtype=torch.int32, pin_memory=True)
            hsel = torch.empty(sel.shape, dtype=torch.int32, pin_memory=True)
            hs.copy_(small, non_blocking=True); hk.copy_(n_sel, non_blocking=True); hsel.copy_(sel, non_blocking=True)
            torch.cuda.current_stream(self.dev).synchronize()
        else:
            hs, hk, hsel = small, n_sel, sel
        hs, hk, hsel = hs.numpy(), hk.numpy(), hsel.numpy()
        rows = [hsel[row0[b]:row0[b] + hk[b]] for b in range(B)]
        n_out = int(hk.sum())
        pm = torch.empty(n_out, T, Hm, Wm, device=self.dev)
        if n_out:
            ops.rows_gather(mp, self._to_dev_i32(np.concatenate(rows)), out=pm)
        labels = small[:, 1].long()
        results, o = [], 0
        for b in range(B):
            k, r0 = int(hk[b]), int(row0[b])
            h = hs[r0:r0 + k]
            d = small[r0:r0 + k]
            results.append({"scores": d[:, 0], "pred_classes": labels[r0:r0 + k], "cls_probs": d[:, 2:2 + K], "pred_masks": pm[o:o + k],
                            "query_embeds": d[:, 2 + K:], "rows": d,
                            "host": {"scores": h[:, 0], "cls_probs": h[:, 2:2 + K], "query_embeds": h[:, 2 + K:]}})
            o += k
        return results
```

### mdqe_cvpr2023_amd/ops.py

```python
import contextlib
import os
import threading

import torch

from ._lib import check, cur_stream, lib, ptr, raw_stream

ACT = {"none": 0, None: 0, "relu": 1, "gelu": 2, "sigmoid": 3, "tanh": 4}

if os.environ.get("MDQE_MSDA_VARIANT"):
    check(lib.mdqe_debug_msda_variant(int(os.environ["MDQE_MSDA_VARIANT"])), "msda_variant")

if os.environ.get("MDQE_MSDA_DEC_STAGED"):
    check(lib.mdqe_debug_msda_dec_staged(int(os.environ["MDQE_MSDA_DEC_STAGED"])), "msda_dec_staged")

if os.environ.get("MDQE_GEMM_TILE_RULE"):
    check(lib.mdqe_debug_gemm_tile_rule(int(os.environ["MDQE_GEMM_TILE_RULE"])), "gemm_tile_rule")
if os.environ.get("MDQE_GEMM_STAGGER"):
    check(lib.mdqe_debug_gemm_stagger(int(os.environ["MDQE_GEMM_STAGGER"])), "gemm_stagger")

if os.environ.get("MDQE_MSDA_DEC_STAGE_KB"):
    check(lib.mdqe_debug_msda_dec_stage_kb(int(os.environ["MDQE_MSDA_DEC_STAGE_KB"])), "msda_dec_stage_kb")
if os.environ.get("MDQE_MSDA_TP_STAGED"):
    check(lib.mdqe_debug_msda_tp_staged(int(os.environ["MDQE_MSDA_TP_STAGED"])), "msda_tp_staged")
if os.environ.get("MDQE_GEMM_LDS_PAD"):
    check(lib.mdqe_debug_gemm_lds_pad(int(os.environ["MDQE_GEMM_LDS_PAD"])), "gemm_lds_pad")
if os.environ.get("MDQE_WINOGRAD_TILE"):
    check(lib.mdqe_debug_winograd_tile(int(os.environ["MDQE_WINOGRAD_TILE"])), "winograd_tile")

_ws = {}


GEMM_MODES = {"f32": 0, "f16x3": 1, "f16": 2}


def set_gemm_precision(mode):
    check(lib.mdqe_set_gemm_precision(GEMM_MODES[mode]), "set_gemm_precision")


def get_gemm_precision():
    return {v: k for k, v in GEMM_MODES.items()}[lib.mdqe_get_gemm_precision()]


_tl_prec = threading.local()


@contextlib.contextmanager
def gemm_precision(mode):
    prev = getattr(_tl_prec, "v", -1)
    cur = GEMM_MODES[mode]
    check(lib.mdqe_set_gemm_precision_thread(cur), "set_gemm_precision_thread")
    _tl_prec.v = cur
    try:
        yield
    finally:
        check(lib.mdqe_set_gemm_precision_thread(prev), "set_gemm_precision_thread")
        _tl_prec.v = prev


_split = {}


def const_weight(w):
    import weakref
    if not (torch.is_tensor(w) and w.is_cuda and w.dtype == torch.float32 and w.dim() >= 2 and w.is_contiguous()):
        return w
    N = w.shape[0]
    K = w.numel() // max(N, 1)
    if N < 128 or K % 32 != 0 or float(w.abs().max()) >= 32752.0:
        return w
    planes = torch.empty(3 * w.numel(), dtype=torch.float16, device=w.device)
    check(lib.mdqe_f16x3_split_f32(ptr(w), w.numel(), ptr(planes), cur_stream()), "f16x3_split")
    key = w.data_ptr()
    _split[key] = (weakref.ref(w), w._version, planes)
    weakref.finalize(w, _drop_split, key)
    return w


def _drop_split(key):
    ent = _split.get(key)
    if ent is not None and ent[0]() is None:
        del _split[key]


def _wsplit(w):
    ent = _split.get(w.data_ptr())
    if ent is None:
        return None
    ref, ver, planes = ent
    base = ref()
    if base is None or base._version != ver:
        del _split[w.data_ptr()]
        return None
    if w.numel() != base.numel() or w._version != ver or not w.is_contiguous():
        return None
    return planes


WINOGRAD = os.environ.get("MDQE_WINOGRAD", "1") != "0"
_wino = {}


def winograd_weight(w):
    import weakref
    if not (torch.is_tensor(w) and w.is_cuda and w.dtype == torch.float32 and w.dim() == 4 and w.is_contiguous()):
        return w
    Cout, KH, KW, Cin = w.shape
    if KH != 3 or KW != 3 or Cin < 128 or Cin % 32 != 0 or Cout % 4 != 0 or Cout > 1024:
        return w
    U = torch.empty((16, Cout, Cin), dtype=torch.float32, device=w.device)
    check(lib.mdqe_winograd_weight_f32(ptr(w), Cout, Cin, ptr(U), cur_stream()), "winograd_weight_f32")
    key = w.data_ptr()
    _wino[key] = (weakref.ref(w), w._version, U)
    weakref.finalize(w, _drop_wino, key)
    return w


def _drop_wino(key):
    ent = _wino.get(key)
    if ent is not None and ent[0]() is None:
        del _wino[key]


def _wino_u(w):
    ent = _wino.get(w.data_ptr())
    if ent is None:
        return None
    ref, ver, U = ent
    base = ref()
    if base is None or base._version != ver:
        del _wino[w.data_ptr()]
        return None
    if w.shape != base.shape or w._version != ver or not w.is_contiguous():
        return None
    return U


def _workspace(nbytes, device):
    dev = device.index if device.index is not None else torch.cuda.current_device()
    key = (dev, raw_stream(dev))
    t = _ws.get(key)
    if t is None or t.numel() < nbytes:
        t = torch.empty(max(nbytes, 1 << 20), dtype=torch.uint8, device=device)
        _ws[key] = t
    return t


def _chk(t, name, dtype=torch.float32):
    if t is None:
        return
    if not t.is_cuda or t.dtype != dtype or not t.is_contiguous():
        raise RuntimeError(f"{name}: expected contiguous CUDA {dtype} tensor, got {t.dtype} {t.device} "
                           f"contiguous={t.is_contiguous()}")


def linear(x, weight, bias=None, act=None, residual=None, res_mod=0, rowmask=None, mask_cols=0, act_cols=0,
           out=None, ldc=None, tile=0, res_first=False, ksplit=0):
    K = x.shape[-1]
    N = weight.shape[0]
    if x.dim() != 2:
        x2 = x.reshape(-1, K)
    else:
        x2 = x
    if x2.stride(-1) != 1:
        raise RuntimeError("linear: last dim of x must be contiguous")
    M = x2.shape[0]
    lda = x2.stride(0) if M > 1 else K
    _chk(weight, "weight"); _chk(bias, "bias")
    if rowmask is not None and rowmask.dtype == torch.bool:
        rowmask = rowmask.view(torch.uint8)
    if out is None:
        out = torch.empty((M, N), dtype=torch.float32, device=x.device)
        ldc_ = N
    else:
        ldc_ = ldc if ldc is not None else out.stride(0) if out.dim() == 2 else N
    ldr = 0
    if residual is not None:
        ldr = residual.stride(0) if residual.dim() == 2 else residual.shape[-1]
    ws = None
    if ksplit > 1:
        ws = _workspace(ksplit * M * N * 4 + 64, x.device)
    check(lib.mdqe_gemm_nt_f32(ptr(x2), lda, ptr(weight), ptr(bias), ptr(out), ldc_, M, N, K, ACT[act], act_cols,
                               ptr(residual), ldr, res_mod, int(res_first), ptr(rowmask), mask_cols, tile, ksplit, ptr(ws),
                               ptr(_wsplit(weight)), cur_stream()), "gemm_nt_f32")
    if x.dim() != 2 and ldc is None and out.dim() == 2 and out.shape == (M, N):
        return out.view(*x.shape[:-1], N)
    return out


def conv2d_nhwc(x, w_packed, bias=None, stride=1, pad=0, act=None, residual=None, out=None, tile=0, res_first=False, ksplit=0):
    _chk(w_packed, "w"); _chk(bias, "bias"); _chk(residual, "residual")
    NI, H, W, Cin = x.shape
    if not (x.is_cuda and x.dtype == torch.float32 and x.stride(3) == 1 and x.stride(2) == Cin and x.stride(1) == W * Cin):
        raise RuntimeError("conv2d_nhwc: x must be CUDA fp32 NHWC with dense pixels")
    xis = x.stride(0) if NI > 1 else 0
    Cout, KH, KW, _ = w_packed.shape
    OH = (H + 2 * pad - KH) // stride + 1
    OW = (W + 2 * pad - KW) // stride + 1
    if out is None:
        out = torch.empty((NI, OH, OW, Cout), dtype=torch.float32, device=x.device)
    ldy = out.stride(-2)
    ldr = residual.stride(-2) if residual is not None else 0
    M, K = NI * OH * OW, KH * KW * Cin
    if (WINOGRAD and KH == 3 and KW == 3 and stride == 1 and pad == 1 and residual is None and tile == 0 and ksplit == 0
            and Cin >= 128 and Cin % 32 == 0 and lib.mdqe_get_gemm_precision() == 0):
        U = _wino_u(w_packed)
        aligned = ((x.data_ptr() | out.data_ptr() | (bias.data_ptr() if bias is not None else 0)) & 15) == 0 and ldy % 4 == 0 and xis % 4 == 0
        if U is not None and aligned:
            nb = lib.mdqe_winograd_workspace_bytes(NI, H, W, Cin, Cout)
            ws = _workspace(nb, x.device)
            check(lib.mdqe_conv3x3_winograd_f32(ptr(x), xis, ptr(U), ptr(bias), ptr(out), ldy, NI, H, W, Cin, Cout, ACT[act],
                                                ptr(ws), ws.numel(), cur_stream()), "conv3x3_winograd_f32")
            return out
    ws = None
    if ksplit == 0 and K >= 4096 and ((OH * OW + 63) // 64) * ((Cout + 63) // 64) <= 16:
        ksplit = min(16, K // 1024)
    if ksplit > 1:
        ws = _workspace(ksplit * M * Cout * 4 + 64, x.device)
    check(lib.mdqe_conv2d_nhwc_f32(ptr(x), xis, ptr(w_packed), ptr(bias), ptr(out), ldy, NI, H, W, Cin, Cout, KH, KW, stride,
                                   pad, ACT[act], ptr(residual), ldr, int(res_first), tile, ptr(_wsplit(w_packed)), ksplit, ptr(ws),
                                   cur_stream()),
          "conv2d_nhwc_f32")
    return out


LINEAR_LN_FUSED = os.environ.get("MDQE_LINEAR_LN_FUSED", "1") != "0"
LINEAR_LN_MIN_ROWS = 16384


def linear_ln(x, weight, bias, residual, gamma, beta, eps=1e-5, out=None, scratch=None, second=None):
    M, K = x.shape
    N = weight.shape[0]
    if out is None:
        out = torch.empty((M, N), dtype=torch.float32, device=x.device)
    nb = (M + 63) // 64
    full = nb >= 1024 or nb / (256.0 * ((nb + 255) // 256)) >= 0.8
    small = M * max(out.stride(0), residual.stride(0) if residual is not None else 0) * 4 < 0xFFFF0000
    if LINEAR_LN_FUSED and N == 256 and M >= LINEAR_LN_MIN_ROWS and full and small and get_gemm_precision() == "f32" and x.stride(1) == 1:
        _chk(weight, "weight"); _chk(bias, "bias"); _chk(gamma, "gamma"); _chk(beta, "beta"); _chk(residual, "residual"); _chk(out, "out")
        if second is not None and LINEAR_LN2_FUSED:
            _chk(second[0], "gamma2"); _chk(second[1], "beta2")
            out2 = torch.empty((M, N), dtype=torch.float32, device=x.device)
            check(lib.mdqe_gemm_ln2_f32(ptr(x), x.stride(0) if M > 1 else K, ptr(weight), ptr(bias), ptr(out), out.stride(0), M, N, K,
                                        ptr(residual), residual.stride(0) if residual is not None else 0, ptr(gamma), ptr(beta),
                                        ptr(second[0]), ptr(second[1]), ptr(out2), out2.stride(0), eps, cur_stream()), "gemm_ln2_f32")
            return out, out2
        check(lib.mdqe_gemm_ln_f32(ptr(x), x.stride(0) if M > 1 else K, ptr(weight), ptr(bias), ptr(out), out.stride(0), M, N, K,
                                   ptr(residual), residual.stride(0) if residual is not None else 0, ptr(gamma), ptr(beta), eps,
                                   cur_stream()), "gemm_ln_f32")
        return out if second is None else (out, layernorm(out, second[0], second[1], eps=eps))
    y = linear(x, weight, bias, residual=residual, out=scratch)
    out = layernorm(y, gamma, beta, eps=eps, out=out)
    return out if second is None else (out, layernorm(out, second[0], second[1], eps=eps))


LINEAR_LN2_FUSED = os.environ.get("MDQE_LINEAR_LN2_FUSED", "1") != "0"


def linear_side(x, weight, bias, side, side_w, side_cols, out=None):
    M, K = x.shape
    N = weight.shape[0]
    _chk(weight, "weight"); _chk(bias, "bias"); _chk(side, "side"); _chk(side_w, "side_w")
    if x.stride(1) != 1 or side.shape != (M, 4) or side_w.shape != (N, 4):
        raise RuntimeError("linear_side: x rows contiguous, side [M,4], side_w [N,4] required")
    if out is None:
        out = torch.empty((M, N), dtype=torch.float32, device=x.device)
    check(lib.mdqe_gemm_nt_side_f32(ptr(x), x.stride(0) if M > 1 else K, ptr(weight), ptr(bias), ptr(out), out.stride(0), M, N, K,
                                    ptr(side), ptr(side_w), side_cols, ptr(_wsplit(weight)), cur_stream()), "gemm_nt_side_f32")
    return out


def linear_cat2(y, x_nhwc, stride, weight, bias, act=None, out=None):
    _chk(y, "y"); _chk(x_nhwc, "x"); _chk(weight, "weight"); _chk(bias, "bias")
    NI, OH, OW, K1 = y.shape
    _, H2, W2, K2 = x_nhwc.shape
    N = weight.shape[0]
    if not (y.is_contiguous() and x_nhwc.is_contiguous() and weight.is_contiguous() and weight.shape[1] == K1 + K2):
        raise RuntimeError("linear_cat2: contiguous operands and a [N, K1 + K2] weight required")
    if out is None:
        out = torch.empty((NI, OH, OW, N), dtype=torch.float32, device=y.device)
    check(lib.mdqe_gemm_nt_cat2_f32(ptr(y), K1, K1, ptr(x_nhwc), K2, K2, NI, OH, OW, H2, W2, stride, ptr(weight), ptr(bias), ptr(out), N, N,
                                    ACT[act], cur_stream()), "gemm_nt_cat2")
    return out


def linear_pix(x_nhwc, stride, weight, bias, act=None, out=None):
    _chk(x_nhwc, "x"); _chk(weight, "weight"); _chk(bias, "bias")
    NI, H, W, K = x_nhwc.shape
    N = weight.shape[0]
    if weight.dim() != 2 or weight.shape[1] != K:
        raise RuntimeError("linear_pix: a [N, K] weight required")
    OH, OW = (H - 1) // stride + 1, (W - 1) // stride + 1
    if out is None:
        out = torch.empty((NI, OH, OW, N), dtype=torch.float32, device=x_nhwc.device)
    check(lib.mdqe_gemm_nt_pix_f32(ptr(x_nhwc), K, K, NI, H, W, OH, OW, stride, ptr(weight), ptr(bias), ptr(out), N, N, ACT[act],
                                   cur_stream()), "gemm_nt_pix")
    return out


def layernorm(x, gamma, beta, res=None, eps=1e-5, out=None):
    _chk(x, "x"); _chk(res, "res"); _chk(gamma, "gamma"); _chk(beta, "beta")
    C = x.shape[-1]
    rows = x.numel() // C
    if out is None:
        out = torch.empty_like(x)
    check(lib.mdqe_layernorm_f32(ptr(x), ptr(res), ptr(gamma), ptr(beta), ptr(out), rows, C, eps, cur_stream()), "layernorm")
    return out


def groupnorm_nhwc(x, groups, gamma, beta, act=None, eps=1e-5, out=None):
    if x.dim() == 4:
        x = x.view(x.shape[0], -1, x.shape[-1])
    NI, HW, C = x.shape
    if out is None:
        out = torch.empty((NI, HW, C), dtype=torch.float32, device=x.device)
    elif out.dim() == 4:
        out = out.view(NI, HW, C)
    ws = _workspace(lib.mdqe_groupnorm_workspace_bytes(NI, groups), x.device)
    check(lib.mdqe_groupnorm_nhwc_f32(ptr(x), x.stride(1), x.stride(0) if NI > 1 else 0, ptr(out), out.stride(1),
                                      out.stride(0) if NI > 1 else 0, NI, HW, C, groups, ptr(gamma),
                                      ptr(beta), eps, ACT[act], ptr(ws), cur_stream()), "groupnorm_nhwc")
    return out


def stem_im2col(frames, Hp, Wp, mean, std):
    import ctypes
    if not frames.is_cuda or not frames.is_contiguous() or frames.dtype not in (torch.uint8, torch.float32):
        raise RuntimeError("stem_im2col: frames must be contiguous CUDA uint8/float32 [NI,3,h,w]")
    NI, _, h, w = frames.shape
    out = torch.empty((NI * (Hp // 2) * (Wp // 2), 160), dtype=torch.float32, device=frames.device)
    m = (ctypes.c_float * 3)(*[float(v) for v in mean])
    s = (ctypes.c_float * 3)(*[float(v) for v in std])
    check(lib.mdqe_stem_im2col_f32(ptr(frames), int(frames.dtype == torch.uint8), 3 * h * w, NI, h, w, Hp, Wp, m, s, ptr(out),
                                   cur_stream()), "stem_im2col")
    return out


def stem_weight_kmajor(w_krsc):
    wk = torch.zeros(7, 22, 64, dtype=torch.float32)
    wk[:, :21] = w_krsc.reshape(64, 7, 21).permute(1, 2, 0)
    return wk.reshape(154, 64).contiguous()


def stem_conv(frames, Hp, Wp, mean, std, wk, bias):
    import ctypes
    if not frames.is_cuda or not frames.is_contiguous() or frames.dtype not in (torch.uint8, torch.float32):
        raise RuntimeError("stem_conv: frames must be contiguous CUDA uint8/float32 [NI,3,h,w]")
    _chk(wk, "wk"); _chk(bias, "bias")
    if tuple(wk.shape) != (154, 64) or bias.numel() != 64:
        raise RuntimeError("stem_conv: wk must be [154,64] (stem_weight_kmajor) and bias [64]")
    NI, _, h, w = frames.shape
    out = torch.empty((NI, Hp // 2, Wp // 2, 64), dtype=torch.float32, device=frames.device)
    m = (ctypes.c_float * 3)(*[float(v) for v in mean])
    s = (ctypes.c_float * 3)(*[float(v) for v in std])
    check(lib.mdqe_stem_conv_f32(ptr(frames), int(frames.dtype == torch.uint8), 3 * h * w, NI, h, w, Hp, Wp, m, s, ptr(wk),
                                 ptr(bias), ptr(out), cur_stream()), "stem_conv")
    return out


def maxpool3x3s2(x):
    _chk(x, "x")
    NI, H, W, C = x.shape
    out = torch.empty((NI, (H - 1) // 2 + 1, (W - 1) // 2 + 1, C), dtype=torch.float32, device=x.device)
    check(lib.mdqe_maxpool3x3s2_nhwc_f32(ptr(x), ptr(out), NI, H, W, C, cur_stream()), "maxpool")
    return out


def upsample_nearest_add(a, b, out=None):
    _chk(a, "a"); _chk(b, "b")
    NI, H, W, C = a.shape
    if out is None:
        out = torch.empty_like(a)
    check(lib.mdqe_upsample_nearest_add_nhwc_f32(ptr(a), ptr(b), ptr(out), NI, H, W, b.shape[1], b.shape[2], C, cur_stream()),
          "upsample_nearest_add")
    return out


def dwconv5x5(x, wt, bias, up2=False, tw=None, tb=None):
    _chk(x, "x"); _chk(wt, "wt"); _chk(bias, "bias")
    NI, H, W, C = x.shape
    OH, OW = (2 * H, 2 * W) if up2 else (H, W)
    out = torch.empty((NI, OH, OW, C), dtype=torch.float32, device=x.device)
    if C == 256 and DW_FAST:
        if up2:
            _chk(tw, "tw"); _chk(tb, "tb")
            check(lib.mdqe_dwconv5x5_up2_c256_f32(ptr(x), ptr(wt), ptr(bias), ptr(tw), ptr(tb), ptr(out), NI, H, W, cur_stream()),
                  "dwconv5x5_up2_c256")
        else:
            check(lib.mdqe_dwconv5x5_c256_f32(ptr(x), ptr(wt), ptr(bias), ptr(out), NI, H, W, cur_stream()), "dwconv5x5_c256")
        return out
    check(lib.mdqe_dwconv5x5_nhwc_f32(ptr(x), ptr(wt), ptr(bias), ptr(out), NI, OH, OW, C, int(up2), ptr(tw), ptr(tb),
                                      cur_stream()), "dwconv5x5")
    return out


DW_FAST = os.environ.get("MDQE_DW_FAST", "1") != "0"
MASK_HEAD_FUSED = os.environ.get("MDQE_MASK_HEAD_FUSED", "1") != "0"


def dwconv5x5_up2_pw(x, wt, bias, tw, tb, pw, pb, out=None):
    _chk(x, "x"); _chk(wt, "wt"); _chk(bias, "bias"); _chk(tw, "tw"); _chk(tb, "tb"); _chk(pw, "pw"); _chk(pb, "pb")
    NI, Hs, Ws, C = x.shape
    N = pw.shape[0]
    rows = NI * 4 * Hs * Ws
    if out is not None and (out.dim() != 2 or tuple(out.shape) != (rows, N) or out.stride(1) != 1 or not out.is_cuda or out.dtype != torch.float32):
        raise RuntimeError("dwconv5x5_up2_pw: out must be a CUDA fp32 [NI*2Hs*2Ws, N] view with contiguous rows")
    ldo = N if out is None or rows <= 1 else out.stride(0)
    ptrs = [t.data_ptr() for t in (x, wt, bias, tw, tb, pw, pb)] + ([out.data_ptr()] if out is not None else [])
    fused = (MASK_HEAD_FUSED and DW_FAST and C == 256 and N == 32 and pw.shape[1] == C and lib.mdqe_get_gemm_precision() == 0
             and all(a % 16 == 0 for a in ptrs) and ldo % 4 == 0 and ldo >= N)
    if not fused:
        z = dwconv5x5(x, wt, bias, up2=True, tw=tw, tb=tb)
        return linear(z.view(-1, C), pw, pb, out=out)
    if out is None:
        out = torch.empty((rows, N), dtype=torch.float32, device=x.device)
    check(lib.mdqe_dwconv5x5_up2_pw_c256_f32(ptr(x), ptr(wt), ptr(bias), ptr(tw), ptr(tb), ptr(pw), ptr(pb), ptr(out), ldo, NI, Hs, Ws,
                                             cur_stream()), "dwconv5x5_up2_pw_c256")
    return out


def msda(value, shapes_dev, starts_dev, loc, attn, groups=1, scale=1.0, out=None):
    B, S, M, D = value.shape
    Q, L, P = loc.shape[1], loc.shape[3], loc.shape[4]
    if out is None:
        out = torch.empty((B, Q, M * D), dtype=torch.float32, device=value.device)
    check(lib.mdqe_msda_forward_grouped_f32(ptr(value), ptr(shapes_dev), ptr(starts_dev), ptr(loc), ptr(attn), B, S, M, D,
                                            groups, L, Q, P, scale, ptr(out), cur_stream()), "msda")
    return out


def msda_fused(value, offs, logits, ref, levels, B, Q, M, D, L, P, mode=0, grid=None, groups=1, scale=1.0,
               v_brows=None, out=None, vidx=None):
    import ctypes
    Hs, Ws, Ss = levels
    n = groups * L
    assert len(Hs) == n and len(Ws) == n and len(Ss) == n
    if ref.dim() == 2:
        ref_b, ref_dim = 0, ref.shape[-1]
    else:
        ref_b, ref_dim = ref.stride(0), ref.shape[-1]
    _chk(ref, "ref")
    if out is None:
        out = torch.empty((B * Q, M * D), dtype=torch.float32, device=value.device)
    arr = lambda v: (ctypes.c_int * n)(*[int(x) for x in v])
    if v_brows is None:
        v_brows = value.shape[0] // max(B, 1)
    if vidx is not None and (vidx.dtype != torch.int32 or not vidx.is_cuda or vidx.numel() != B):
        raise RuntimeError("msda_fused: vidx must be a CUDA int32 tensor with B entries")
    check(lib.mdqe_msda_fused_f32(ptr(value), value.stride(0), v_brows, ptr(vidx), ptr(offs), offs.stride(0), ptr(logits),
                                  logits.stride(0), ptr(ref), ref_b, ref_dim, mode, ptr(grid), arr(Hs), arr(Ws), arr(Ss),
                                  B, M, D, groups, L, Q, P, scale, ptr(out), out.stride(0), value.shape[0], cur_stream()), "msda_fused")
    return out


def mask_row_stats(logits):
    _chk(logits, "logits")
    n, T, H, W = logits.shape
    t_step = 2 if T >= 5 else 1
    Th = (T + t_step - 1) // t_step
    Ph = Th * (H // 2) * (W // 2)
    stats = torch.empty(n, 5, device=logits.device)
    soft_h = torch.empty(n, Ph, device=logits.device)
    hard_h = torch.empty(n, Ph, device=logits.device)
    check(lib.mdqe_mask_row_stats_f32(ptr(logits), n, T, H, W, t_step, ptr(stats), ptr(soft_h), ptr(hard_h), cur_stream()),
          "mask_row_stats")
    return stats, soft_h, hard_h


def mha_small(qk, v, B, Q, C, nh, out=None):
    if out is None:
        out = torch.empty((B * Q, C), dtype=torch.float32, device=v.device)
    check(lib.mdqe_mha_small_f32(ptr(qk), qk.stride(0), ptr(v), v.stride(0), ptr(out), out.stride(0), B, Q, C, nh, cur_stream()),
          "mha_small")
    return out


def query_select(conf, nb, out=None):
    _chk(conf, "conf")
    NI, H, W, K = conf.shape
    ws = torch.empty(NI * H * W, dtype=torch.float32, device=conf.device)
    if out is not None:
        _chk(out, "out")
        if tuple(out.shape) != (NI, nb * nb, 2):
            raise RuntimeError("query_select: out must be [NI, nb*nb, 2]")
    coords = out if out is not None else torch.empty(NI, nb * nb, 2, dtype=torch.float32, device=conf.device)
    check(lib.mdqe_query_select_f32(ptr(conf), NI, H, W, K, nb, ptr(ws), ptr(coords), cur_stream()), "query_select")
    return coords


def sample_levels_mean(tokens, coords, shapes, starts, out=None):
    import ctypes
    _chk(tokens, "tokens"); _chk(coords, "coords")
    NI, N, C = tokens.shape
    Qn = coords.shape[1]
    n = len(shapes)
    arr = lambda v: (ctypes.c_int * n)(*[int(x) for x in v])
    if out is None:
        out = torch.empty(NI, Qn, C, dtype=torch.float32, device=tokens.device)
    else:
        _chk(out, "out")
        if tuple(out.shape) != (NI, Qn, C):
            raise RuntimeError("sample_levels_mean: out must be [NI, Q, C]")
    check(lib.mdqe_sample_levels_mean_f32(ptr(tokens), NI, N, C, ptr(coords), Qn, arr([s[0] for s in shapes]), arr([s[1] for s in shapes]),
                                          arr(starts), n, ptr(out), cur_stream()), "sample_levels_mean")
    return out


def _final_mask_args(logits, inst_idx, check_idx, cap=None):
    _chk(logits, "logits")
    n, Fw, Hm, Wm = logits.shape
    if check_idx:
        _chk(inst_idx, "inst_idx", torch.int32)
    k = int(inst_idx.numel())
    if cap is None:
        return k, Fw, Hm, Wm
    return (k, Fw, Hm, Wm, torch.empty(k * Fw, cap, dtype=torch.int32, device=logits.device),
            torch.empty(k * Fw, dtype=torch.int32, device=logits.device))


def final_masks(logits, inst_idx, factor, h, w, Ho, Wo, out, f_off):
    k, Fw, Hm, Wm = _final_mask_args(logits, inst_idx, False)
    check(lib.mdqe_final_masks_u8(ptr(logits), k, ptr(inst_idx), Fw, Hm, Wm, factor, h, w, Ho, Wo, ptr(out),
                                  out.stride(0), f_off, cur_stream()), "final_masks")
    return out


def final_masks_geom(logits, inst_idx, factor, h, w, Ho, Wo, out, f_off, geom=None):
    k, Fw, Hm, Wm = _final_mask_args(logits, inst_idx, True)
    if (not out.is_cuda or out.dtype != torch.uint8 or out.dim() != 4 or out.shape[0] < k or (out.shape[0] and not out[0].is_contiguous())
            or tuple(out.shape[2:]) != (Ho, Wo) or f_off < 0 or f_off + Fw > out.shape[1]):
        raise RuntimeError("final_masks_geom: out must be CUDA uint8 [>= n_sel, >= f_off + Fw, Ho, Wo]")
    geom = _geom_rows(geom, k * Fw, logits.device)
    check(lib.mdqe_final_masks_u8_geom(ptr(logits), k, ptr(inst_idx), Fw, Hm, Wm, factor, h, w, Ho, Wo, ptr(out), out.stride(0), f_off,
                                       ptr(geom), cur_stream()), "final_masks_geom")
    return out, geom


def final_label_map(logits, inst_idx, factor, h, w, Ho, Wo, out, f_off, geom=None):
    if logits.dim() != 4 or int(logits.shape[0]) > 255:
        raise RuntimeError("final_label_map: logits must be [n <= 255, Fw, Hm, Wm] (uint8 labels), got %s" % (tuple(logits.shape),))
    if inst_idx.dtype != torch.int32 or inst_idx.dim() != 1:
        raise RuntimeError("final_label_map: inst_idx must be int32 [n_sel], got %s %s" % (inst_idx.dtype, tuple(inst_idx.shape)))
    Fw = int(logits.shape[1])
    if (not torch.is_tensor(out) or out.dtype != torch.uint8 or out.dim() != 3 or tuple(out.shape[1:]) != (Ho, Wo) or f_off < 0
            or f_off + Fw > out.shape[0] or not out.is_contiguous() or not out.is_cuda):
        raise RuntimeError("final_label_map: out must be contiguous CUDA uint8 [>= f_off + Fw = %d, Ho, Wo]" % (f_off + Fw))
    k, Fw, Hm, Wm = _final_mask_args(logits, inst_idx, True)
    if geom is not None:
        geom = _geom_rows(geom, k * Fw, logits.device)
    check(lib.mdqe_final_label_map_u8(ptr(logits), k, ptr(inst_idx), Fw, Hm, Wm, factor, h, w, Ho, Wo, ptr(out), f_off,
                                      ptr(geom) if geom is not None and k else None, cur_stream()), "final_label_map")
    return out, geom


def final_matte(logits, inst_idx, factor, h, w, Ho, Wo, out, f_off, take=None, gain=1.0):
    if not torch.is_tensor(logits) or logits.dim() != 4 or int(logits.shape[0]) > 255:
        raise RuntimeError("final_matte: logits must be [n <= 255, Fw, Hm, Wm], got %s" % (tuple(getattr(logits, "shape", ())),))
    if not torch.is_tensor(inst_idx) or inst_idx.dtype != torch.int32 or inst_idx.dim() != 1:
        raise RuntimeError("final_matte: inst_idx must be int32 [n_sel]")
    if isinstance(gain, bool) or not isinstance(gain, (int, float)) or not 0.0 < float(gain) <= 64.0:
        raise RuntimeError("final_matte: gain must be a finite number in (0, 64], got %r" % (gain,))
    if take is not None and (not torch.is_tensor(take) or take.dtype != torch.uint8 or tuple(take.shape) != (256,) or not take.is_contiguous()):
        raise RuntimeError("final_matte: take must be contiguous uint8 [256] (render.Style.takes) or None")
    Fw = int(logits.shape[1])
    if (not torch.is_tensor(out) or out.dtype != torch.uint8 or out.dim() != 3 or tuple(out.shape[1:]) != (Ho, Wo)
            or not isinstance(f_off, int) or f_off < 0 or f_off + Fw > out.shape[0] or not out.is_contiguous()):
        raise RuntimeError("final_matte: out must be contiguous CUDA uint8 [>= f_off + Fw = %d, Ho, Wo]" % (f_off + Fw))
    for name, t in (("out", out), ("take", take)):
        if t is not None and (not t.is_cuda or t.device != logits.device):
            raise RuntimeError("final_matte: %s must be a CUDA tensor on the logits' device, got %s" % (name, t.device))
    k, Fw, Hm, Wm = _final_mask_args(logits, inst_idx, True)
    check(lib.mdqe_final_matte_u8(ptr(logits), k, ptr(inst_idx), Fw, Hm, Wm, factor, h, w, Ho, Wo, ptr(take), float(gain), ptr(out), f_off,
                                  cur_stream()), "final_matte")
    return out


def final_masks_overlap(logits, inst_idx, factor, h, w, Ho, Wo, gt_bits, G, f_off, inter, area=None):
    if not torch.is_tensor(logits) or logits.dim() != 4:
        raise RuntimeError("final_masks_overlap: logits must be [n, Fw, Hm, Wm], got %s" % (tuple(getattr(logits, "shape", ())),))
    if not torch.is_tensor(inst_idx) or inst_idx.dtype != torch.int32 or inst_idx.dim() != 1:
        raise RuntimeError("final_masks_overlap: inst_idx must be int32 [n_sel]")
    k, Fw = int(inst_idx.numel()), int(logits.shape[1])
    if (not torch.is_tensor(gt_bits) or gt_bits.dtype != torch.uint32 or gt_bits.dim() != 3 or tuple(gt_bits.shape[1:]) != (Ho, Wo)
            or not gt_bits.is_contiguous()):
        raise RuntimeError("final_masks_overlap: gt_bits must be contiguous uint32 [frames, Ho = %d, Wo = %d]" % (Ho, Wo))
    if f_off < 0 or f_off + Fw > gt_bits.shape[0]:
        raise RuntimeError("final_masks_overlap: gt_bits holds %d frames, the window needs f_off + Fw = %d" % (gt_bits.shape[0], f_off + Fw))
    if (not torch.is_tensor(inter) or inter.dtype != torch.int64 or inter.dim() != 2 or inter.shape[0] < k or inter.shape[1] < G
            or inter.stride(1) != 1 or (inter.shape[0] > 1 and inter.stride(0) < G)):
        raise RuntimeError("final_masks_overlap: inter must be int64 [>= n_sel = %d, >= G = %d] with unit column stride" % (k, G))
    if area is not None and (not torch.is_tensor(area) or area.dtype != torch.int32 or area.numel() != k * Fw or not area.is_contiguous()):
        raise RuntimeError("final_masks_overlap: area must be contiguous int32 [n_sel * Fw = %d]" % (k * Fw))
    for name, t in (("gt_bits", gt_bits), ("inter", inter), ("area", area)):
        if t is not None and not t.is_cuda:
            raise RuntimeError("final_masks_overlap: %s must be a CUDA tensor" % name)
    k, Fw, Hm, Wm = _final_mask_args(logits, inst_idx, True)
    if area is None:
        area = torch.empty(k * Fw, dtype=torch.int32, device=logits.device)
    check(lib.mdqe_final_masks_overlap(ptr(logits), k, ptr(inst_idx), Fw, Hm, Wm, factor, h, w, Ho, Wo, ptr(gt_bits), G, f_off,
                                       ptr(inter), inter.stride(0) if inter.shape[0] > 1 else max(int(inter.shape[1]), G), ptr(area),
                                       cur_stream()), "final_masks_overlap")
    return inter, area


def _mosaic_args(name, action, cell):
    if not torch.is_tensor(action) or action.dtype != torch.uint8 or tuple(action.shape) != (256,) or not action.is_contiguous():
        raise RuntimeError("%s: action must be contiguous uint8 [256] (render.Style.actions)" % name)
    if isinstance(cell, bool) or not isinstance(cell, int) or not 2 <= cell <= 64 or cell % 2:
        raise RuntimeError("%s: cell must be an even int in 2..64, got %r" % (name, cell))


def _blur_args(name, action, taps, taps_c=None, surface=False):
    if not torch.is_tensor(action) or action.dtype != torch.uint8 or tuple(action.shape) != (256,) or not action.is_contiguous():
        raise RuntimeError("%s: action must be contiguous uint8 [256] (render.Style.actions)" % name)
    for t, what, top in ((taps, "taps", 32),) + (((taps_c, "taps_c", 16),) if surface else ()):
        if (not torch.is_tensor(t) or t.dtype not in (torch.uint16, torch.int16) or t.dim() != 1 or not 1 <= t.numel() <= top + 1
                or not t.is_contiguous()):
            raise RuntimeError("%s: %s must be contiguous uint16 [radius + 1], radius in 0..%d (render.blur_taps)" % (name, what, top))


def _replace_args(name, action, matte, backdrop, F, H, W):
    if not torch.is_tensor(action) or action.dtype != torch.uint8 or tuple(action.shape) != (256,) or not action.is_contiguous():
        raise RuntimeError("%s: action must be contiguous uint8 [256] (render.Style.actions)" % name)
    if not torch.is_tensor(matte) or matte.dtype != torch.uint8 or tuple(matte.shape) != (F, H, W) or not matte.is_contiguous():
        raise RuntimeError("%s: matte must be contiguous uint8 [F = %d, %d, %d], the labels' shape (ops.final_matte)" % (name, F, H, W))
    if (not torch.is_tensor(backdrop) or backdrop.dtype != torch.uint8 or tuple(backdrop.shape) not in ((3,), (H, W, 3))
            or not backdrop.is_contiguous()):
        raise RuntimeError("%s: backdrop must be contiguous uint8 [3] (a colour) or [%d, %d, 3] (a picture of the output's size), got %s"
                           % (name, H, W, tuple(getattr(backdrop, "shape", ()))))


def _rgb_paint_args(name, labels, frames, palette, out, f_off, a256, contour, mosaic=None, blur=None, replace=None):
    if not torch.is_tensor(labels) or labels.dtype != torch.uint8 or labels.dim() != 3 or not labels.is_contiguous():
        raise RuntimeError("%s: labels must be contiguous uint8 [F, Ho, Wo]" % name)
    F, Ho, Wo = (int(v) for v in labels.shape)
    if not isinstance(a256, int) or not isinstance(contour, int) or not 0 <= a256 <= 256 or not 0 <= contour <= 3:
        raise RuntimeError("%s: a256 must be an int in 0..256 and contour an int in 0..3, got %r, %r" % (name, a256, contour))
    if mosaic is not None:
        _mosaic_args(name, *mosaic)
    if blur is not None:
        _blur_args(name, *blur)
    if replace is not None:
        _replace_args(name, *replace, F, Ho, Wo)
    if Ho < 1 or Wo < 1 or Ho * Wo * 3 >= 2 ** 31 or F * Ho * Wo >= 2 ** 31:
        raise RuntimeError("%s: Ho, Wo must be positive with Ho*Wo*3 < 2^31 and F*Ho*Wo < 2^31, got %s" % (name, tuple(labels.shape)))
    if not torch.is_tensor(palette) or palette.dtype != torch.uint8 or tuple(palette.shape) != (256, 3) or not palette.is_contiguous():
        raise RuntimeError("%s: palette must be contiguous uint8 [256, 3]" % name)
    if (not torch.is_tensor(out) or out.dtype != torch.uint8 or out.dim() != 4 or tuple(out.shape[1:]) != (Ho, Wo, 3) or f_off < 0
            or f_off + F > out.shape[0] or not out.is_contiguous()):
        raise RuntimeError("%s: out must be contiguous CUDA uint8 [>= f_off + F = %d, Ho, Wo, 3]" % (name, f_off + F))
    h0 = w0 = stride = 0
    if frames is not None:
        if (not torch.is_tensor(frames) or frames.dtype not in (torch.uint8, torch.float32) or frames.dim() != 4
                or int(frames.shape[0]) != F or int(frames.shape[1]) != 3 or frames.shape[2] < 1 or frames.shape[3] < 1):
            raise RuntimeError("%s: frames must be uint8 or float32 [F = %d, 3, h0, w0] or None" % (name, F))
        h0, w0 = int(frames.shape[2]), int(frames.shape[3])
        stride = int(frames.stride(0)) if F > 1 else 3 * h0 * w0
        if tuple(frames.stride()[1:]) != (h0 * w0, w0, 1) or stride < 3 * h0 * w0 or h0 * Ho >= 2 ** 31 or w0 * Wo >= 2 ** 31:
            raise RuntimeError("%s: every frame must be contiguous and the frames a stride >= 3*h0*w0 apart, got strides %s"
                               % (name, tuple(frames.stride())))
    tensors = [(labels, "labels"), (palette, "palette")] + ([(mosaic[0], "action")] if mosaic is not None else [])
    tensors += [(blur[0], "action"), (blur[1], "taps")] if blur is not None else []
    tensors += [(replace[0], "action"), (replace[1], "matte"), (replace[2], "backdrop")] if replace is not None else []
    tensors += [(out, "out"), (frames, "frames")]
    for t, what in tensors:
        if t is not None and (not t.is_cuda or t.device != out.device):
            raise RuntimeError("%s: %s must be a CUDA tensor on out's device, got %s" % (name, what, t.device))
    return F, Ho, Wo, h0, w0, stride


def render_overlay(labels, frames, palette, out, f_off=0, a256=128, contour=1):
    F, Ho, Wo, h0, w0, stride = _rgb_paint_args("render_overlay", labels, frames, palette, out, f_off, a256, contour)
    check(lib.mdqe_render_overlay_u8(ptr(frames) if frames is not None else None, int(frames is not None and frames.dtype == torch.uint8),
                                     stride, h0, w0, ptr(labels), F, Ho, Wo, ptr(palette), a256, contour, ptr(out), f_off, cur_stream()),
          "render_overlay")
    return out


def render_mosaic(labels, frames, palette, action, out, f_off=0, a256=128, contour=1, cell=16):
    F, Ho, Wo, h0, w0, stride = _rgb_paint_args("render_mosaic", labels, frames, palette, out, f_off, a256, contour, (action, cell))
    check(lib.mdqe_render_mosaic_u8(ptr(frames) if frames is not None else None, int(frames is not None and frames.dtype == torch.uint8),
                                    stride, h0, w0, ptr(labels), F, Ho, Wo, ptr(palette), ptr(action), a256, contour, cell, ptr(out),
                                    f_off, cur_stream()), "render_mosaic")
    return out


REPLACE_MODES = ("background", "tracks")


def render_replace(labels, frames, palette, action, matte, backdrop, out, f_off=0, a256=128, contour=1, mode="background"):
    if mode not in REPLACE_MODES:
        raise RuntimeError("render_replace: mode must be 'background' or 'tracks', got %r" % (mode,))
    F, Ho, Wo, h0, w0, stride = _rgb_paint_args("render_replace", labels, frames, palette, out, f_off, a256, contour,
                                                replace=(action, matte, backdrop))
    check(lib.mdqe_render_replace_u8(ptr(frames) if frames is not None else None, int(frames is not None and frames.dtype == torch.uint8),
                                     stride, h0, w0, ptr(labels), F, Ho, Wo, ptr(palette), ptr(action), a256, contour, ptr(matte),
                                     ptr(backdrop), int(backdrop.dim() == 3), REPLACE_MODES.index(mode), ptr(out), f_off, cur_stream()),
          "render_replace")
    return out


def render_replace_yuv(labels, yuv, palette_yuv, action, matte, backdrop, out=None, f_off=0, a256=128, contour=1, mode="background"):
    from .preprocess import YuvFrames
    name = "render_replace_yuv"
    if mode not in REPLACE_MODES:
        raise RuntimeError("%s: mode must be 'background' or 'tracks', got %r" % (name, mode))
    if not isinstance(yuv, YuvFrames):
        raise RuntimeError("%s: yuv must be a preprocess.YuvFrames, got %s" % (name, type(yuv).__name__))
    F, H, W = len(yuv), yuv.height, yuv.width
    if not torch.is_tensor(action) or action.dtype != torch.uint8 or tuple(action.shape) != (256,) or not action.is_contiguous():
        raise RuntimeError("%s: action must be contiguous uint8 [256] (render.Style.actions)" % name)
    if not torch.is_tensor(matte) or matte.dtype != torch.uint8 or tuple(matte.shape) != (F, H, W) or not matte.is_contiguous():
        raise RuntimeError("%s: matte must be contiguous uint8 [F = %d, %d, %d], the surfaces' own size (ops.final_matte)" % (name, F, H, W))
    surf = isinstance(backdrop, YuvFrames)
    if surf:
        if len(backdrop) != 1 or (backdrop.height, backdrop.width, backdrop.fmt) != (H, W, yuv.fmt):
            raise RuntimeError("%s: a backdrop surface must be a YuvFrames of ONE surface of %d x %d %s" % (name, H, W, yuv.fmt))
    elif (not torch.is_tensor(backdrop) or backdrop.dtype not in (torch.uint16, torch.int16) or tuple(backdrop.shape) != (3,)
# ... 807 lines not shown
```

Baseline: 870.1 frames/s.

## Apply GroupNorm on load in mask-head consumers instead of separate pass

```diff
diff --git a/include/mdqe_hip.h b/include/mdqe_hip.h
--- a/include/mdqe_hip.h
+++ b/include/mdqe_hip.h
@@ -158,6 +158,22 @@
 int mdqe_dwconv5x5_up2_pw_c256_f32(const float* x, const float* wt, const float* bias, const float* tw, const float* tb,
                                    const float* pw, const float* pb, float* out, long ldo, int NI, int Hs, int Ws, void* stream);
 
+int mdqe_groupnorm_stats_f32(const float* x, long ldx, long x_img_stride, int NI, int HW, int C, int G, float eps,
+                             void* workspace, float* stats, void* stream);
+int mdqe_upsample_nearest_add_gn_nhwc_f32(const float* a, const float* b, long ldb, long b_img_stride, float* y, int NI,
+                                          int H, int W, int Hb, int Wb, int C, const float* stats, int G,
+                                          const float* gamma, const float* beta, int act, void* stream);
+int mdqe_dwconv5x5_gn_c256_f32(const float* x, long ldx, long x_img_stride, const float* wt, const float* bias, float* y,
+                               int NI, int H, int W, const float* stats, int G, const float* gamma, const float* beta,
+                               int act, int strip_rows, void* stream);
+int mdqe_dwconv5x5_up2_gn_c256_f32(const float* x, long ldx, long x_img_stride, const float* wt, const float* bias,
+                                   const float* tw, const float* tb, float* y, int NI, int Hs, int Ws, const float* stats,
+                                   int G, const float* gamma, const float* beta, int act, void* stream);
+int mdqe_dwconv5x5_up2_pw_gn_c256_f32(const float* x, long ldx, long x_img_stride, const float* wt, const float* bias,
+                                      const float* tw, const float* tb, const float* pw, const float* pb, float* out,
+                                      long ldo, int NI, int Hs, int Ws, const float* stats, int G, const float* gamma,
+                                      const float* beta, int act, void* stream);
+
 int mdqe_trk_siou_f32(const float* saved, long saved_stride, int n_saved, const float* inp, long inp_stride,
                       int n_in, long n, float* out3, void* stream);
 int mdqe_trk_accumulate_f32(float* sum, long sum_stride, float* cnt, long cnt_stride, const float* src,
diff --git a/mdqe_cvpr2023_amd/_lib.py b/mdqe_cvpr2023_amd/_lib.py
--- a/mdqe_cvpr2023_amd/_lib.py
+++ b/mdqe_cvpr2023_amd/_lib.py
@@ -127,6 +127,11 @@
     "mdqe_dwconv5x5_c256_f32": [p, p, p, p, i, i, i, p],
     "mdqe_dwconv5x5_up2_c256_f32": [p, p, p, p, p, p, i, i, i, p],
     "mdqe_dwconv5x5_up2_pw_c256_f32": [p, p, p, p, p, p, p, p, l, i, i, i, p],
+    "mdqe_groupnorm_stats_f32": [p, l, l, i, i, i, i, f, p, p, p],
+    "mdqe_upsample_nearest_add_gn_nhwc_f32": [p, p, l, l, p, i, i, i, i, i, i, p, i, p, p, i, p],
+    "mdqe_dwconv5x5_gn_c256_f32": [p, l, l, p, p, p, i, i, i, p, i, p, p, i, i, p],
+    "mdqe_dwconv5x5_up2_gn_c256_f32": [p, l, l, p, p, p, p, p, i, i, i, p, i, p, p, i, p],
+    "mdqe_dwconv5x5_up2_pw_gn_c256_f32": [p, l, l, p, p, p, p, p, p, p, l, i, i, i, p, i, p, p, i, p],
 }
 
 
diff --git a/mdqe_cvpr2023_amd/csrc/common.h b/mdqe_cvpr2023_amd/csrc/common.h
--- a/mdqe_cvpr2023_amd/csrc/common.h
+++ b/mdqe_cvpr2023_amd/csrc/common.h
@@ -53,6 +53,47 @@
   }
 }
 
+__device__ __forceinline__ void mdqe_gn_stats(const double* __restrict__ part, int img, int g, int G, int nchunks, int HW, int C,
+                                              float eps, float& mean_f, float& rstd_f) {
+#pragma clang fp contract(off)
+  double s = 0.0, q = 0.0;
+  for (int c = 0; c < nchunks; ++c) {
+    const double* o = part + (((long)img * nchunks + c) * G + g) * 2;
+    s += o[0]; q += o[1];
+  }
+  const double n = (double)HW * (C / G);
+  const double mean = s / n;
+  double var = __builtin_fma(-mean, mean, q / n);
+  if (var < 0) var = 0;
+  mean_f = (float)mean;
+  rstd_f = (float)(1.0 / sqrt(var + (double)eps));
+}
+
+__device__ __forceinline__ float mdqe_gn_elem(float v, float mean, float rstd, float gamma, float beta, int act) {
+#pragma clang fp contract(off)
+  const float t = (v - mean) * rstd;
+  return mdqe_act(__builtin_fmaf(t, gamma, beta), act);
+}
+
+struct GnLane {
+  f32x4 gamma, beta;
+  int g;
+};
+__device__ __forceinline__ GnLane mdqe_gn_lane(const float* __restrict__ gamma, const float* __restrict__ beta, int c4, int C, int G) {
+  GnLane L;
+  L.gamma = *reinterpret_cast<const f32x4*>(gamma + c4 * 4);
+  L.beta = *reinterpret_cast<const f32x4*>(beta + c4 * 4);
+  L.g = (c4 * 4) / (C / G);
+  return L;
+}
+template <int ACT>
+__device__ __forceinline__ f32x4 mdqe_gn4(f32x4 v, f32x2 mr, const GnLane& L) {
+  f32x4 o;
+#pragma unroll
+  for (int k = 0; k < 4; ++k) o[k] = mdqe_gn_elem(v[k], mr[0], mr[1], L.gamma[k], L.beta[k], ACT);
+  return o;
+}
+
 template <typename V4, typename ColOk>
 __device__ __forceinline__ void mdqe_act4(V4& v, int act, ColOk col_ok) {
   if (act == MDQE_ACT_RELU) {
diff --git a/mdqe_cvpr2023_amd/csrc/dwconv.hip b/mdqe_cvpr2023_amd/csrc/dwconv.hip
--- a/mdqe_cvpr2023_amd/csrc/dwconv.hip
+++ b/mdqe_cvpr2023_amd/csrc/dwconv.hip
@@ -41,13 +41,99 @@
   }
 }
 
+template <int ACT, int NC>
+__global__ void __launch_bounds__(256, 2)
+dw5_gn_c256_kernel(const float* __restrict__ x, long ldx, long xis, const float* __restrict__ wt, const float* __restrict__ bias,
+                   float* __restrict__ y, int NI, int H, int W, int RS, const float* __restrict__ st, int G,
+                   const float* __restrict__ gamma, const float* __restrict__ beta) {
+  constexpr int C = 256;
+  __shared__ __attribute__((aligned(16))) float sw[25 * C];
+  for (int i = threadIdx.x; i < 25 * C / 4; i += 256) reinterpret_cast<f32x4*>(sw)[i] = reinterpret_cast<const f32x4*>(wt)[i];
+  __syncthreads();
+  const int lane = threadIdx.x & 63;
+  const long wid = (long)blockIdx.x * 4 + (threadIdx.x >> 6), nw = (long)gridDim.x * 4;
+  const float* const swl = sw + lane * 4;
+  const f32x4 bv = ld4(bias + lane * 4);
+  const GnLane L = mdqe_gn_lane(gamma, beta, lane, C, G);
+  const int Wp = (W + NC - 1) / NC;
+  const int nseg = (H + RS - 1) / RS;
+  const long total = (long)NI * nseg * Wp;
+  for (long i = wid; i < total; i += nw) {
+    const int pw_ = (int)(i % Wp); const long t = i / Wp;
+    const int seg = (int)(t % nseg), img = (int)(t / nseg);
+    const int w0 = pw_ * NC, h0 = seg * RS, h1 = min(H, h0 + RS);
+    const f32x2 mr = *reinterpret_cast<const f32x2*>(st + ((long)img * G + L.g) * 2);
+    const float* xi = x + (long)img * xis + lane * 4;
+    float* yi = y + ((long)img * H * W) * C + lane * 4;
+    f32x4 R[NC + 4];
+    auto load_row = [&](int ih) __attribute__((always_inline)) {
+      const bool rok = ih >= 0 && ih < H && ih < h1 + 2;
+#pragma unroll
+      for (int c = 0; c < NC + 4; ++c) {
+        const int iw = w0 - 2 + c;
+        R[c] = (rok && iw >= 0 && iw < W) ? ld4(xi + ((long)ih * W + iw) * ldx) : f32x4{0.f, 0.f, 0.f, 0.f};
+      }
+    };
+    f32x4 A[5][NC];
+#pragma unroll
+    for (int j = 0; j < 5; ++j)
+#pragma unroll
+      for (int o = 0; o < NC; ++o) A[j][o] = bv;
+    load_row(h0 - 2);
+    for (int ih = h0 - 2; ih < h1 + 2; ++ih) {
+      if (ih >= 0 && ih < H) {
+        f32x4 X[NC + 4];
+#pragma unroll
+        for (int c = 0; c < NC + 4; ++c) {
+          const int iw = w0 - 2 + c;
+          const f32x4 n = mdqe_gn4<ACT>(R[c], mr, L);
+          X[c] = (iw >= 0 && iw < W) ? n : f32x4{0.f, 0.f, 0.f, 0.f};
+        }
+        load_row(ih + 1);
+#pragma unroll
+        for (int j = 0; j < 5; ++j) {
+          const int oh = ih - 2 + j;
+          if (oh < h0 || oh >= h1) continue;
+#pragma unroll
+          for (int kw = 0; kw < 5; ++kw) {
+            const f32x4 wv = ld4(swl + ((4 - j) * 5 + kw) * C);
+#pragma unroll
+            for (int o = 0; o < NC; ++o) A[j][o] += X[o + kw] * wv;
+          }
+        }
+      } else {
+        load_row(ih + 1);
+      }
+      const int oh = ih - 2;
+      if (oh >= h0 && oh < h1) {
+        float* o_ = yi + ((long)oh * W + w0) * C;
+#pragma unroll
+        for (int o = 0; o < NC; ++o)
+          if (w0 + o < W) *reinterpret_cast<f32x4*>(o_ + o * C) = A[0][o];
+      }
+#pragma unroll
+      for (int o = 0; o < NC; ++o) {
+#pragma unroll
+        for (int j = 0; j < 4; ++j) A[j][o] = A[j + 1][o];
+        A[4][o] = bv;
+      }
+    }
+  }
+}
+
+template <int GN>
 __global__ void __launch_bounds__(256, 2)
 dw5_up2_c256_kernel(const float* __restrict__ x, const float* __restrict__ wt, const float* __restrict__ bias,
-                    const float* __restrict__ tw, const float* __restrict__ tb, float* __restrict__ y, int NI, int Hs, int Ws) {
+                    const float* __restrict__ tw, const float* __restrict__ tb, float* __restrict__ y, int NI, int Hs, int Ws,
+                    long ldx_, long xis_, const float* __restrict__ st, int G, const float* __restrict__ gamma,
+                    const float* __restrict__ beta) {
   constexpr int C = 256;
   const int lane = threadIdx.x & 63;
   const long wid = (long)blockIdx.x * 4 + (threadIdx.x >> 6), nw = (long)gridDim.x * 4;
   const int H = 2 * Hs, W = 2 * Ws;
+  const long ldx = GN < 0 ? (long)C : ldx_, xis = GN < 0 ? (long)Hs * Ws * C : xis_;
+  GnLane L;
+  if constexpr (GN >= 0) L = mdqe_gn_lane(gamma, beta, lane, C, G);
   f32x4 w[25];
 #pragma unroll
   for (int t = 0; t < 25; ++t) w[t] = ld4(wt + t * C + lane * 4);
@@ -62,16 +148,22 @@
     const int b = (int)(i % Ws); const long t = i / Ws;
     const int a = (int)(t % Hs), img = (int)(t / Hs);
     f32x4 o00 = {0.f, 0.f, 0.f, 0.f}, o01 = o00, o10 = o00, o11 = o00;
+    f32x2 mr = {0.f, 0.f};
+    if constexpr (GN >= 0) mr = *reinterpret_cast<const f32x2*>(st + ((long)img * G + L.g) * 2);
 #pragma unroll
     for (int r = 0; r < 3; ++r) {
       const int ia = a - 1 + r;
       if (ia < 0 || ia >= Hs) continue;
-      const float* row = x + (((long)img * Hs + ia) * Ws) * C + lane * 4;
+      const float* row = x + (long)img * xis + ((long)ia * Ws) * ldx + lane * 4;
       f32x4 X[3];
 #pragma unroll
       for (int c = 0; c < 3; ++c) {
         const int ib = b - 1 + c;
-        X[c] = (ib >= 0 && ib < Ws) ? ld4(row + (long)ib * C) : f32x4{0.f, 0.f, 0.f, 0.f};
+        X[c] = (ib >= 0 && ib < Ws) ? ld4(row + (long)ib * ldx) : f32x4{0.f, 0.f, 0.f, 0.f};
+        if constexpr (GN >= 0) {
+          const f32x4 n = mdqe_gn4<GN>(X[c], mr, L);
+          X[c] = (ib >= 0 && ib < Ws) ? n : X[c];
+        }
       }
 #pragma unroll
       for (int c = 0; c < 3; ++c) o00 += X[c] * w[(2 * r) * 5 + 2 * c];
@@ -110,11 +202,15 @@
   }
 }
 
+template <int GN>
 __global__ void __launch_bounds__(256, 1)
 dw5_up2_pw_c256_kernel(const float* __restrict__ x, const float* __restrict__ wt, const float* __restrict__ bias,
                        const float* __restrict__ tw, const float* __restrict__ tb, const float* __restrict__ pw,
-                       const float* __restrict__ pb, float* __restrict__ out, long ldo, int NI, int Hs, int Ws) {
+                       const float* __restrict__ pb, float* __restrict__ out, long ldo, int NI, int Hs, int Ws,
+                       long ldx_, long xis_, const float* __restrict__ st, int G, const float* __restrict__ gamma,
+                       const float* __restrict__ beta) {
   constexpr int C = 256, QT = 8;
+  const long ldx = GN < 0 ? (long)C : ldx_, xis = GN < 0 ? (long)Hs * Ws * C : xis_;
   extern __shared__ __attribute__((aligned(16))) float dwpw_lds[];
   const int lane = threadIdx.x & 63;
   const int wave = __builtin_amdgcn_readfirstlane(threadIdx.x >> 6);
@@ -141,18 +237,22 @@
   const int Wt = (Ws + QT - 1) / QT;
   const long total = (long)NI * Hs * Wt;
   f32x4 X[3][QT + 2];
+  GnLane L;
+  f32x2 MR = {0.f, 0.f};
+  if constexpr (GN >= 0) L = mdqe_gn_lane(gamma, beta, lane, C, G);
   auto load_strip = [&](long i) __attribute__((always_inline)) {
     const int b0 = (int)(i % Wt) * QT; const long t = i / Wt;
     const int a = (int)(t % Hs), img = (int)(t / Hs);
+    if constexpr (GN >= 0) MR = *reinterpret_cast<const f32x2*>(st + ((long)img * G + L.g) * 2);
 #pragma unroll
     for (int r = 0; r < 3; ++r) {
       const int ia = a - 1 + r;
       const bool rok = ia >= 0 && ia < Hs;
-      const float* row = x + (((long)img * Hs + (rok ? ia : a)) * Ws) * C + lane * 4;
+      const float* row = x + (long)img * xis + ((long)(rok ? ia : a) * Ws) * ldx + lane * 4;
 #pragma unroll
       for (int c = 0; c < QT + 2; ++c) {
         const int ib = b0 - 1 + c;
-        X[r][c] = (rok && ib >= 0 && ib < Ws) ? ld4(row + (long)ib * C) : f32x4{0.f, 0.f, 0.f, 0.f};
+        X[r][c] = (rok && ib >= 0 && ib < Ws) ? ld4(row + (long)ib * ldx) : f32x4{0.f, 0.f, 0.f, 0.f};
       }
     }
   };
@@ -162,6 +262,19 @@
     const int b0 = (int)(i % Wt) * QT; const long ti = i / Wt;
     const int a = (int)(ti % Hs), img = (int)(ti / Hs);
     const int nq = min(QT, Ws - b0);
+    if constexpr (GN >= 0) {
+#pragma unroll
+      for (int r = 0; r < 3; ++r) {
+        const int ia = a - 1 + r;
+        if (ia < 0 || ia >= Hs) continue;
+#pragma unroll
+        for (int c = 0; c < QT + 2; ++c) {
+          const int ib = b0 - 1 + c;
+          const f32x4 n = mdqe_gn4<GN>(X[r][c], MR, L);
+          X[r][c] = (ib >= 0 && ib < Ws) ? n : X[r][c];
+        }
+      }
+    }
 #pragma unroll
     for (int q = 0; q < QT; ++q) {
       if (q >= nq) continue;
@@ -265,7 +378,8 @@
   mdqe_clear_error();
   const long total = (long)NI * Hs * Ws;
   long nb = (total + 3) / 4; if (nb > 256 * 8) nb = 256 * 8;
-  hipLaunchKernelGGL(dw5_up2_c256_kernel, dim3((unsigned)nb), dim3(256), 0, (hipStream_t)stream, x, wt, bias, tw, tb, y, NI, Hs, Ws);
+  hipLaunchKernelGGL((dw5_up2_c256_kernel<-1>), dim3((unsigned)nb), dim3(256), 0, (hipStream_t)stream, x, wt, bias, tw, tb, y, NI, Hs, Ws,
+                     0L, 0L, (const float*)nullptr, 0, (const float*)nullptr, (const float*)nullptr);
   return mdqe_launch_status();
 }
 
@@ -287,10 +401,95 @@
     num_cus = n;
   }
   const int smem = 4 * 32 * 256 * (int)sizeof(float);
-  if (mdqe_allow_lds(reinterpret_cast<const void*>(dw5_up2_pw_c256_kernel), smem) != hipSuccess) return MDQE_ELAUNCH;
+  if (mdqe_allow_lds(reinterpret_cast<const void*>(dw5_up2_pw_c256_kernel<-1>), smem) != hipSuccess) return MDQE_ELAUNCH;
   const long total = (long)NI * Hs * ((Ws + 7) / 8);
   long nb = (total + 3) / 4; if (nb > num_cus) nb = num_cus;
-  hipLaunchKernelGGL(dw5_up2_pw_c256_kernel, dim3((unsigned)nb), dim3(256), (size_t)smem, (hipStream_t)stream, x, wt, bias, tw, tb, pw,
-                     pb, out, ldo, NI, Hs, Ws);
-  return mdqe_launch_status();
-}
+  hipLaunchKernelGGL((dw5_up2_pw_c256_kernel<-1>), dim3((unsigned)nb), dim3(256), (size_t)smem, (hipStream_t)stream, x, wt, bias, tw, tb,
+                     pw, pb, out, ldo, NI, Hs, Ws, 0L, 0L, (const float*)nullptr, 0, (const float*)nullptr, (const float*)nullptr);
+  return mdqe_launch_status();
+}
+
+namespace {
+int gn_args_ok(const float* x, long ldx, long& xis, long HW, const float* stats, int G, const float* gamma, const float* beta, int act) {
+  if (!(G > 0 && 256 % G == 0 && (256 / G) % 4 == 0 && ldx >= 256 && ldx % 4 == 0)) return MDQE_EINVAL;
+  if (!(act == MDQE_ACT_NONE || act == MDQE_ACT_RELU || act == MDQE_ACT_GELU)) return MDQE_EINVAL;
+  if (xis <= 0) xis = HW * ldx;
+  if (xis % 4 != 0) return MDQE_EINVAL;
+  if (!x || !stats || !gamma || !beta) return MDQE_ENULL;
+  if ((((uintptr_t)x | (uintptr_t)gamma | (uintptr_t)beta) & 15) != 0 || ((uintptr_t)stats & 7) != 0) return MDQE_EINVAL;
+  return MDQE_OK;
+}
+}
+
+#define MDQE_GN_DISPATCH(act, LAUNCH)                  \
+  do {                                                 \
+    if ((act) == MDQE_ACT_GELU) { LAUNCH(MDQE_ACT_GELU); } \
+    else if ((act) == MDQE_ACT_RELU) { LAUNCH(MDQE_ACT_RELU); } \
+    else { LAUNCH(MDQE_ACT_NONE); }                    \
+  } while (0)
+
+extern "C" int mdqe_dwconv5x5_gn_c256_f32(const float* x, long ldx, long x_img_stride, const float* wt, const float* bias, float* y,
+                                          int NI, int H, int W, const float* stats, int G, const float* gamma, const float* beta,
+                                          int act, int strip_rows, void* stream) {
+  MDQE_REQUIRE(NI >= 0 && H > 0 && W > 0);
+  if (NI == 0) return MDQE_OK;
+  MDQE_CHECK_PTR(wt); MDQE_CHECK_PTR(bias); MDQE_CHECK_PTR(y);
+  const int ok = gn_args_ok(x, ldx, x_img_stride, (long)H * W, stats, G, gamma, beta, act);
+  if (ok != MDQE_OK) return ok;
+  MDQE_REQUIRE((((uintptr_t)wt | (uintptr_t)bias | (uintptr_t)y) & 15) == 0);
+  mdqe_clear_error();
+  const int RS = strip_rows > 0 ? strip_rows : 24;
+  constexpr int NC = 4;
+  const long total = (long)NI * ((H + RS - 1) / RS) * ((W + NC - 1) / NC);
+  long nb = (total + 3) / 4; if (nb > 256 * 8) nb = 256 * 8;
+#define MDQE_L(A) hipLaunchKernelGGL((dw5_gn_c256_kernel<A, NC>), dim3((unsigned)nb), dim3(256), 0, (hipStream_t)stream, x, ldx, \
+                                     x_img_stride, wt, bias, y, NI, H, W, RS, stats, G, gamma, beta)
+  MDQE_GN_DISPATCH(act, MDQE_L);
+#undef MDQE_L
+  return mdqe_launch_status();
+}
+
+extern "C" int mdqe_dwconv5x5_up2_gn_c256_f32(const float* x, long ldx, long x_img_stride, const float* wt, const float* bias,
+                                              const float* tw, const float* tb, float* y, int NI, int Hs, int Ws, const float* stats,
+                                              int G, const float* gamma, const float* beta, int act, void* stream) {
+  MDQE_REQUIRE(NI >= 0 && Hs > 0 && Ws > 0);
+  if (NI == 0) return MDQE_OK;
+  MDQE_CHECK_PTR(wt); MDQE_CHECK_PTR(bias); MDQE_CHECK_PTR(tw); MDQE_CHECK_PTR(tb); MDQE_CHECK_PTR(y);
+  const int ok = gn_args_ok(x, ldx, x_img_stride, (long)Hs * Ws, stats, G, gamma, beta, act);
+  if (ok != MDQE_OK) return ok;
+  mdqe_clear_error();
+  const long total = (long)NI * Hs * Ws;
+  long nb = (total + 3) / 4; if (nb > 256 * 8) nb = 256 * 8;
+#define MDQE_L(A) hipLaunchKernelGGL((dw5_up2_c256_kernel<A>), dim3((unsigned)nb), dim3(256), 0, (hipStream_t)stream, x, wt, bias, tw, \
+                                     tb, y, NI, Hs, Ws, ldx, x_img_stride, stats, G, gamma, beta)
+  MDQE_GN_DISPATCH(act, MDQE_L);
+#undef MDQE_L
+  return mdqe_launch_status();
+}
+
+extern "C" int mdqe_dwconv5x5_up2_pw_gn_c256_f32(const float* x, long ldx, long x_img_stride, const float* wt, const float* bias,
+                                                 const float* tw, const float* tb, const float* pw, const float* pb, float* out,
+                                                 long ldo, int NI, int Hs, int Ws, const float* stats, int G, const float* gamma,
+                                                 const float* beta, int act, void* stream) {
+  MDQE_REQUIRE(NI >= 0 && Hs > 0 && Ws > 0 && ldo >= 32 && ldo % 4 == 0);
+  if (NI == 0) return MDQE_OK;
+  MDQE_CHECK_PTR(wt); MDQE_CHECK_PTR(bias); MDQE_CHECK_PTR(tw); MDQE_CHECK_PTR(tb);
+  MDQE_CHECK_PTR(pw); MDQE_CHECK_PTR(pb); MDQE_CHECK_PTR(out);
+  const int ok = gn_args_ok(x, ldx, x_img_stride, (long)Hs * Ws, stats, G, gamma, beta, act);
+  if (ok != MDQE_OK) return ok;
+  MDQE_REQUIRE((((uintptr_t)wt | (uintptr_t)bias | (uintptr_t)tw | (uintptr_t)tb | (uintptr_t)pw | (uintptr_t)pb | (uintptr_t)out) & 15) == 0);
+  mdqe_clear_error();
+  int dev = 0, num_cus = 0;
+  (void)hipGetDevice(&dev);
+  if (hipDeviceGetAttribute(&num_cus, hipDeviceAttributeMultiprocessorCount, dev) != hipSuccess || num_cus <= 0) num_cus = 256;
+  const int smem = 4 * 32 * 256 * (int)sizeof(float);
+  const long total = (long)NI * Hs * ((Ws + 7) / 8);
+  long nb = (total + 3) / 4; if (nb > num_cus) nb = num_cus;
+#define MDQE_L(A)                                                                                                                    \
+  if (mdqe_allow_lds(reinterpret_cast<const void*>(dw5_up2_pw_c256_kernel<A>), smem) != hipSuccess) return MDQE_ELAUNCH;             \
+  hipLaunchKernelGGL((dw5_up2_pw_c256_kernel<A>), dim3((unsigned)nb), dim3(256), (size_t)smem, (hipStream_t)stream, x, wt, bias, tw, \
+                     tb, pw, pb, out, ldo, NI, Hs, Ws, ldx, x_img_stride, stats, G, gamma, beta)
+  MDQE_GN_DISPATCH(act, MDQE_L);
+#undef MDQE_L
+  return mdqe_launch_status();
+}
diff --git a/mdqe_cvpr2023_amd/csrc/norm.hip b/mdqe_cvpr2023_amd/csrc/norm.hip
--- a/mdqe_cvpr2023_amd/csrc/norm.hip
+++ b/mdqe_cvpr2023_amd/csrc/norm.hip
@@ -154,19 +154,7 @@
                 float eps, int act) {
   __shared__ float s_mean[64], s_rstd[64];
   const int img = blockIdx.y;
-  if (threadIdx.x < G) {
-    double s = 0.0, q = 0.0;
-    for (int c = 0; c < nchunks; ++c) {
-      const double* o = part + (((long)img * nchunks + c) * G + threadIdx.x) * 2;
-      s += o[0]; q += o[1];
-    }
-    const double n = (double)HW * (C / G);
-    const double mean = s / n;
-    double var = q / n - mean * mean;
-    if (var < 0) var = 0;
-    s_mean[threadIdx.x] = (float)mean;
-    s_rstd[threadIdx.x] = (float)(1.0 / sqrt(var + (double)eps));
-  }
+  if (threadIdx.x < G) mdqe_gn_stats(part, img, threadIdx.x, G, nchunks, HW, C, eps, s_mean[threadIdx.x], s_rstd[threadIdx.x]);
   __syncthreads();
   const int c4n = C / 4, cpg = C / G;
   const long total = (long)HW * c4n;
@@ -180,10 +168,26 @@
 #pragma unroll
     for (int k = 0; k < 4; ++k) {
       const int gi = (col * 4 + k) / cpg;
-      o[k] = mdqe_act((v[k] - s_mean[gi]) * s_rstd[gi] * g[k] + b[k], act);
+      o[k] = mdqe_gn_elem(v[k], s_mean[gi], s_rstd[gi], g[k], b[k], act);
     }
     *reinterpret_cast<f32x4*>(y + (long)img * yis + p * ldy + col * 4) = o;
   }
+}
+
+__global__ void __launch_bounds__(64)
+gn_stats_kernel(const double* __restrict__ part, int HW, int C, int G, int nchunks, float eps, float* __restrict__ st) {
+  const int img = blockIdx.x;
+  if (threadIdx.x < G) {
+    float m, r;
+    mdqe_gn_stats(part, img, threadIdx.x, G, nchunks, HW, C, eps, m, r);
+    *reinterpret_cast<f32x2*>(st + ((long)img * G + threadIdx.x) * 2) = f32x2{m, r};
+  }
+}
+
+static int gn_chunks(int HW) {
+  int nchunks = (HW + 255) / 256;
+  if (nchunks > GN_MAX_CHUNKS) nchunks = GN_MAX_CHUNKS;
+  return nchunks < 1 ? 1 : nchunks;
 }
 
 extern "C" long mdqe_groupnorm_workspace_bytes(int NI, int G) { return (long)NI * GN_MAX_CHUNKS * G * 2 * sizeof(double); }
@@ -201,9 +205,7 @@
   MDQE_CHECK_PTR(x); MDQE_CHECK_PTR(y); MDQE_CHECK_PTR(gamma); MDQE_CHECK_PTR(beta); MDQE_CHECK_PTR(workspace);
   mdqe_clear_error();
   hipStream_t st = (hipStream_t)stream;
-  int nchunks = (HW + 255) / 256;
-  if (nchunks > GN_MAX_CHUNKS) nchunks = GN_MAX_CHUNKS;
-  if (nchunks < 1) nchunks = 1;
+  const int nchunks = gn_chunks(HW);
   hipLaunchKernelGGL(gn_partial_kernel, dim3(nchunks, NI), dim3(256), 0, st, x, ldx, x_img_stride, HW, C, G, nchunks, (double*)workspace);
   int rc = mdqe_launch_status();
   if (rc) return rc;
@@ -213,3 +215,22 @@
                      (const double*)workspace, gamma, beta, eps, act);
   return mdqe_launch_status();
 }
+
+extern "C" int mdqe_groupnorm_stats_f32(const float* x, long ldx, long x_img_stride, int NI, int HW, int C, int G, float eps,
+                                        void* workspace, float* stats, void* stream) {
+  MDQE_REQUIRE(NI >= 0 && HW > 0 && C > 0 && G > 0 && G <= 64 && C % G == 0 && C % 4 == 0 && C <= 1024);
+  MDQE_REQUIRE(ldx >= C && ldx % 4 == 0);
+  if (x_img_stride <= 0) x_img_stride = (long)HW * ldx;
+  MDQE_REQUIRE(x_img_stride % 4 == 0);
+  if (NI == 0) return MDQE_OK;
+  MDQE_CHECK_PTR(x); MDQE_CHECK_PTR(workspace); MDQE_CHECK_PTR(stats);
+  MDQE_REQUIRE(((uintptr_t)stats & 7) == 0);
+  mdqe_clear_error();
+  hipStream_t st = (hipStream_t)stream;
+  const int nchunks = gn_chunks(HW);
+  hipLaunchKernelGGL(gn_partial_kernel, dim3(nchunks, NI), dim3(256), 0, st, x, ldx, x_img_stride, HW, C, G, nchunks, (double*)workspace);
+  int rc = mdqe_launch_status();
+  if (rc) return rc;
+  hipLaunchKernelGGL(gn_stats_kernel, dim3(NI), dim3(64), 0, st, (const double*)workspace, HW, C, G, nchunks, eps, stats);
+  return mdqe_launch_status();
+}
diff --git a/mdqe_cvpr2023_amd/csrc/spatial.hip b/mdqe_cvpr2023_amd/csrc/spatial.hip
--- a/mdqe_cvpr2023_amd/csrc/spatial.hip
+++ b/mdqe_cvpr2023_amd/csrc/spatial.hip
@@ -113,6 +113,51 @@
   const long total = (long)NI * H * W * (C / 4);
   long nb = (total + 255) / 256; if (nb > 256 * 16) nb = 256 * 16;
   hipLaunchKernelGGL(upsample_add_kernel, dim3((unsigned)nb), dim3(256), 0, (hipStream_t)stream, a, b, y, NI, H, W, Hb, Wb, C);
+  return mdqe_launch_status();
+}
+
+template <int ACT>
+__global__ void __launch_bounds__(256)
+upsample_add_gn_kernel(const float* __restrict__ a, const float* __restrict__ b, long ldb, long bis, float* __restrict__ y, int NI,
+                       int H, int W, int Hb, int Wb, int C, const float* __restrict__ st, int G, const float* __restrict__ gamma,
+                       const float* __restrict__ beta) {
+#pragma clang fp contract(off)
+  const int c4n = C / 4;
+  const float sh = (float)Hb / (float)H, sw = (float)Wb / (float)W;
+  const long total = (long)NI * H * W * c4n;
+  for (long i = (long)blockIdx.x * blockDim.x + threadIdx.x; i < total; i += (long)gridDim.x * blockDim.x) {
+    const int c4 = (int)(i % c4n); long t = i / c4n;
+    const int ww = (int)(t % W); t /= W; const int hh = (int)(t % H); const int img = (int)(t / H);
+    const int hb = min((int)floorf(hh * sh), Hb - 1), wb = min((int)floorf(ww * sw), Wb - 1);
+    const GnLane L = mdqe_gn_lane(gamma, beta, c4, C, G);
+    const f32x2 mr = *reinterpret_cast<const f32x2*>(st + ((long)img * G + L.g) * 2);
+    const f32x4 va = *reinterpret_cast<const f32x4*>(a + (((long)img * H + hh) * W + ww) * C + c4 * 4);
+    const f32x4 vb = *reinterpret_cast<const f32x4*>(b + (long)img * bis + ((long)hb * Wb + wb) * ldb + c4 * 4);
+    *reinterpret_cast<f32x4*>(y + (((long)img * H + hh) * W + ww) * C + c4 * 4) = va + mdqe_gn4<ACT>(vb, mr, L);
+  }
+}
+
+extern "C" int mdqe_upsample_nearest_add_gn_nhwc_f32(const float* a, const float* b, long ldb, long b_img_stride, float* y, int NI,
+                                                     int H, int W, int Hb, int Wb, int C, const float* stats, int G,
+                                                     const float* gamma, const float* beta, int act, void* stream) {
+  MDQE_REQUIRE(NI >= 0 && H > 0 && W > 0 && Hb > 0 && Wb > 0 && C > 0 && C % 4 == 0);
+  MDQE_REQUIRE(G > 0 && C % G == 0 && (C / G) % 4 == 0 && ldb >= C && ldb % 4 == 0);
+  MDQE_REQUIRE(act == MDQE_ACT_NONE || act == MDQE_ACT_RELU || act == MDQE_ACT_GELU);
+  if (b_img_stride <= 0) b_img_stride = (long)Hb * Wb * ldb;
+  MDQE_REQUIRE(b_img_stride % 4 == 0);
+  if (NI == 0) return MDQE_OK;
+  MDQE_CHECK_PTR(a); MDQE_CHECK_PTR(b); MDQE_CHECK_PTR(y); MDQE_CHECK_PTR(stats); MDQE_CHECK_PTR(gamma); MDQE_CHECK_PTR(beta);
+  MDQE_REQUIRE(((uintptr_t)stats & 7) == 0);
+  mdqe_clear_error();
+  const long total = (long)NI * H * W * (C / 4);
+  long nb = (total + 255) / 256; if (nb > 256 * 16) nb = 256 * 16;
+#define MDQE_UPS_GN(ACT_)                                                                                                          \
+  hipLaunchKernelGGL((upsample_add_gn_kernel<ACT_>), dim3((unsigned)nb), dim3(256), 0, (hipStream_t)stream, a, b, ldb, b_img_stride, \
+                     y, NI, H, W, Hb, Wb, C, stats, G, gamma, beta)
+  if (act == MDQE_ACT_GELU) MDQE_UPS_GN(MDQE_ACT_GELU);
+  else if (act == MDQE_ACT_RELU) MDQE_UPS_GN(MDQE_ACT_RELU);
+  else MDQE_UPS_GN(MDQE_ACT_NONE);
+#undef MDQE_UPS_GN
   return mdqe_launch_status();
 }
 
diff --git a/mdqe_cvpr2023_amd/engine.py b/mdqe_cvpr2023_amd/engine.py
--- a/mdqe_cvpr2023_amd/engine.py
+++ b/mdqe_cvpr2023_amd/engine.py
@@ -499,17 +499,23 @@
         mh, cfg = self.P.mh, self.cfg
         NI, N, C = enc.shape
         lv = [enc[:, geo.starts[l]:geo.starts[l] + geo.hw[l]].view(NI, geo.shapes[l][0], geo.shapes[l][1], C) for l in range(3)]
+
+        def gn(t, groups, gamma, beta, act, on_load=True):
+            if on_load and t.shape[-1] == 256 and ops.DW_FAST and ops.gn_on_load_ok(t, groups, act):
+                return ops.groupnorm_on_load(t, groups, gamma, beta, act=act)
+            return ops.groupnorm_nhwc(t, groups, gamma, beta, act=act, out=t).view(t.shape)
+
         x = ops.conv2d_nhwc(lv[2], *mh.lay1, 1, 1)
-        x = ops.groupnorm_nhwc(x, 8, *mh.gn1, act="gelu", out=x).view(x.shape)
+        x = gn(x, 8, *mh.gn1, "gelu")
         for i, f in ((2, lv[1]), (3, lv[0])):
             cur = ops.conv2d_nhwc(f, *getattr(mh, f"ad{i - 1}"), 1, 0)
             x = ops.upsample_nearest_add(cur, x, out=cur)
             x = ops.conv2d_nhwc(x, *getattr(mh, f"lay{i}"), 1, 1)
-            x = ops.groupnorm_nhwc(x, 8, *getattr(mh, f"gn{i}"), act="gelu", out=x).view(x.shape)
+            x = gn(x, 8, *getattr(mh, f"gn{i}"), "gelu")
         o1, o2 = mh.out_lay1, mh.out_lay2
         y = ops.dwconv5x5(x, o1.dw, o1.db)
         y = ops.linear(y.view(-1, C), o1.pw, o1.pb).view(x.shape)
-        y = ops.groupnorm_nhwc(y, 32, o1.g, o1.beta, act="relu", out=y).view(x.shape)
+        y = gn(y, 32, o1.g, o1.beta, "relu", on_load=ops.GN_ON_LOAD_TAIL)
         Md = o2.pw.shape[0]
         Hm, Wm = 2 * y.shape[1], 2 * y.shape[2]
         if out is not None and (tuple(out.shape) != (NI, Hm, Wm, Md) or not out.is_contiguous()):
diff --git a/mdqe_cvpr2023_amd/ops.py b/mdqe_cvpr2023_amd/ops.py
--- a/mdqe_cvpr2023_amd/ops.py
+++ b/mdqe_cvpr2023_amd/ops.py
@@ -323,6 +323,59 @@
     return out
 
 
+GN_ON_LOAD = os.environ.get("MDQE_GN_ON_LOAD", "1") != "0"
+GN_ON_LOAD_TAIL = os.environ.get("MDQE_GN_ON_LOAD", "1") == "2"
+
+
+class GnOnLoad:
+    __slots__ = ("x", "stats", "groups", "gamma", "beta", "act")
+
+    def __init__(self, x, stats, groups, gamma, beta, act):
+        self.x, self.stats, self.groups, self.gamma, self.beta, self.act = x, stats, groups, gamma, beta, act
+
+    @property
+    def shape(self):
+        return self.x.shape
+
+    def strides(self):
+        x = self.x
+        NI, H, W, C = x.shape
+        ld = x.stride(2) if H * W > 1 else C
+        if x.stride(3) != 1 or (H > 1 and x.stride(1) != W * ld) or ld % 4 or ld < C or (NI > 1 and x.stride(0) % 4):
+            return None
+        return ld, (x.stride(0) if NI > 1 else 0)
+
+    def args(self):
+        ld, ims = self.strides()
+        return ptr(self.x), ld, ims
+
+    def tail(self):
+        return ptr(self.stats), self.groups, ptr(self.gamma), ptr(self.beta), ACT[self.act]
+
+    def apply(self):
+        NI, H, W, C = self.x.shape
+        return groupnorm_nhwc(self.x, self.groups, self.gamma, self.beta, act=self.act).view(NI, H, W, C)
+
+
+def gn_on_load_ok(x, groups, act):
+    C = x.shape[-1]
+    return (GN_ON_LOAD and x.dim() == 4 and x.is_cuda and x.dtype == torch.float32 and C % groups == 0 and (C // groups) % 4 == 0
+            and act in (None, "relu", "gelu") and x.data_ptr() % 16 == 0
+            and GnOnLoad(x, None, groups, None, None, act).strides() is not None)
+
+
+def groupnorm_on_load(x, groups, gamma, beta, act=None, eps=1e-5):
+    _chk(gamma, "gamma"); _chk(beta, "beta")
+    if not gn_on_load_ok(x, groups, act):
+        raise RuntimeError("groupnorm_on_load: x must be a CUDA fp32 [NI,H,W,C] view with rows W pixels apart and C/groups % 4 == 0")
+    NI, H, W, C = x.shape
+    g = GnOnLoad(x, torch.empty((NI, groups, 2), dtype=torch.float32, device=x.device), groups, gamma, beta, act)
+    ld, ims = g.strides()
+    ws = _workspace(lib.mdqe_groupnorm_workspace_bytes(NI, groups), x.device)
+    check(lib.mdqe_groupnorm_stats_f32(ptr(x), ld, ims, NI, H * W, C, groups, eps, ptr(ws), ptr(g.stats), cur_stream()), "groupnorm_stats")
+    return g
+
+
 def stem_im2col(frames, Hp, Wp, mean, std):
     import ctypes
     if not frames.is_cuda or not frames.is_contiguous() or frames.dtype not in (torch.uint8, torch.float32):
@@ -367,19 +420,37 @@
 
 
 def upsample_nearest_add(a, b, out=None):
-    _chk(a, "a"); _chk(b, "b")
+    _chk(a, "a")
     NI, H, W, C = a.shape
     if out is None:
         out = torch.empty_like(a)
+    if isinstance(b, GnOnLoad):
+        check(lib.mdqe_upsample_nearest_add_gn_nhwc_f32(ptr(a), *b.args(), ptr(out), NI, H, W, b.shape[1], b.shape[2], C, *b.tail(),
+                                                        cur_stream()), "upsample_nearest_add_gn")
+        return out
+    _chk(b, "b")
     check(lib.mdqe_upsample_nearest_add_nhwc_f32(ptr(a), ptr(b), ptr(out), NI, H, W, b.shape[1], b.shape[2], C, cur_stream()),
           "upsample_nearest_add")
     return out
 
 
 def dwconv5x5(x, wt, bias, up2=False, tw=None, tb=None):
-    _chk(x, "x"); _chk(wt, "wt"); _chk(bias, "bias")
+    _chk(wt, "wt"); _chk(bias, "bias")
     NI, H, W, C = x.shape
     OH, OW = (2 * H, 2 * W) if up2 else (H, W)
+    if isinstance(x, GnOnLoad):
+        if not (C == 256 and DW_FAST and all(t.data_ptr() % 16 == 0 for t in (wt, bias, x.gamma, x.beta))):
+            return dwconv5x5(x.apply(), wt, bias, up2=up2, tw=tw, tb=tb)
+        out = torch.empty((NI, OH, OW, C), dtype=torch.float32, device=wt.device)
+        if up2:
+            _chk(tw, "tw"); _chk(tb, "tb")
+            check(lib.mdqe_dwconv5x5_up2_gn_c256_f32(*x.args(), ptr(wt), ptr(bias), ptr(tw), ptr(tb), ptr(out), NI, H, W, *x.tail(),
+                                                     cur_stream()), "dwconv5x5_up2_gn_c256")
+        else:
+            check(lib.mdqe_dwconv5x5_gn_c256_f32(*x.args(), ptr(wt), ptr(bias), ptr(out), NI, H, W, *x.tail(), DW_GN_STRIP_ROWS,
+                                                 cur_stream()), "dwconv5x5_gn_c256")
+        return out
+    _chk(x, "x")
     out = torch.empty((NI, OH, OW, C), dtype=torch.float32, device=x.device)
     if C == 256 and DW_FAST:
         if up2:
@@ -396,10 +467,16 @@
 
 DW_FAST = os.environ.get("MDQE_DW_FAST", "1") != "0"
 MASK_HEAD_FUSED = os.environ.get("MDQE_MASK_HEAD_FUSED", "1") != "0"
+DW_GN_STRIP_ROWS = int(os.environ.get("MDQE_DW_GN_STRIP_ROWS", "0"))
 
 
 def dwconv5x5_up2_pw(x, wt, bias, tw, tb, pw, pb, out=None):
-    _chk(x, "x"); _chk(wt, "wt"); _chk(bias, "bias"); _chk(tw, "tw"); _chk(tb, "tb"); _chk(pw, "pw"); _chk(pb, "pb")
+    gn = x if isinstance(x, GnOnLoad) else None
+    if gn is not None:
+        x = gn.x
+    else:
+        _chk(x, "x")
+    _chk(wt, "wt"); _chk(bias, "bias"); _chk(tw, "tw"); _chk(tb, "tb"); _chk(pw, "pw"); _chk(pb, "pb")
     NI, Hs, Ws, C = x.shape
     N = pw.shape[0]
     rows = NI * 4 * Hs * Ws
@@ -407,13 +484,19 @@
         raise RuntimeError("dwconv5x5_up2_pw: out must be a CUDA fp32 [NI*2Hs*2Ws, N] view with contiguous rows")
     ldo = N if out is None or rows <= 1 else out.stride(0)
     ptrs = [t.data_ptr() for t in (x, wt, bias, tw, tb, pw, pb)] + ([out.data_ptr()] if out is not None else [])
+    if gn is not None:
+        ptrs += [gn.gamma.data_ptr(), gn.beta.data_ptr()]
     fused = (MASK_HEAD_FUSED and DW_FAST and C == 256 and N == 32 and pw.shape[1] == C and lib.mdqe_get_gemm_precision() == 0
              and all(a % 16 == 0 for a in ptrs) and ldo % 4 == 0 and ldo >= N)
     if not fused:
-        z = dwconv5x5(x, wt, bias, up2=True, tw=tw, tb=tb)
+        z = dwconv5x5(x if gn is None else gn, wt, bias, up2=True, tw=tw, tb=tb)
         return linear(z.view(-1, C), pw, pb, out=out)
     if out is None:
         out = torch.empty((rows, N), dtype=torch.float32, device=x.device)
+    if gn is not None:
+        check(lib.mdqe_dwconv5x5_up2_pw_gn_c256_f32(*gn.args(), ptr(wt), ptr(bias), ptr(tw), ptr(tb), ptr(pw), ptr(pb), ptr(out), ldo, NI,
+                                                    Hs, Ws, *gn.tail(), cur_stream()), "dwconv5x5_up2_pw_gn_c256")
+        return out
     check(lib.mdqe_dwconv5x5_up2_pw_c256_f32(ptr(x), ptr(wt), ptr(bias), ptr(tw), ptr(tb), ptr(pw), ptr(pb), ptr(out), ldo, NI, Hs, Ws,
                                              cur_stream()), "dwconv5x5_up2_pw_c256")
     return out
```

Result: no change. 871.8 frames/s (median of 2 runs) (+0.2%).
